# wonheeML/mtl-ssl

Hardware: AMD Instinct MI355X
Metric: images/sec training, Faster R-CNN ResNet-101 + aux heads (higher is better)
Workload: dtype f32; 1 GPU; Faster R-CNN ResNet-101 + window/closeness/edgemask heads + refine, synthetic 1024x600 COCO-shaped (90 classes), per-GPU batch 2 (BASELINE.json configs[1]); global_batch=2, parallelism=dp1, pipeline_config=configs/frcnn_resnet101_coco_mtl.config

## Files before the change

mtl_ssl_amd/csrc/conv.hip:

```cpp
#include <stdlib.h>

#include <atomic>
#include <mutex>
#include <unordered_map>

#include "conv_mfma.h"
#include "conv_split.h"

namespace mtlssl {

__global__ void __launch_bounds__(256) k_row_group_flags(const float* __restrict__ scale, int n, uint8_t* __restrict__ flags) {
  const int i = blockIdx.x * blockDim.x + threadIdx.x;
  if (i < n) flags[i] = scale[i] != 0.f;
}
__global__ void __launch_bounds__(256) k_active_ksteps(const uint8_t* __restrict__ flags, int rpg, int P, int pps, int stride,
                                                       int* __restrict__ out) {
  const int z = blockIdx.x, pix0 = z * pps, pix1 = min(P, pix0 + pps);
  const int ksteps = (max(pix1 - pix0, 0) + BK - 1) / BK;
  const int lane = threadIdx.x & 63, w = threadIdx.x >> 6;
  int* list = out + KSTEP_HDR + (int64_t)z * stride;
  __shared__ int wave_cnt[4];
  int base = 0;
  for (int s0 = 0; s0 < ksteps; s0 += 256) {
    const int s = s0 + threadIdx.x;
    bool act = false;
    if (s < ksteps) {
      const int r0 = pix0 + s * BK, r1 = min(r0 + BK, pix1) - 1;
      for (int g = r0 / rpg; g <= r1 / rpg; ++g) act |= flags[g] != 0;
    }
    const unsigned long long m = __ballot(act);
    if (lane == 0) wave_cnt[w] = __popcll(m);
    __syncthreads();
    int off = base;
    for (int i = 0; i < w; ++i) off += wave_cnt[i];
    if (act) list[off + __popcll(m & ((1ull << lane) - 1ull))] = s;
    base += wave_cnt[0] + wave_cnt[1] + wave_cnt[2] + wave_cnt[3];
    __syncthreads();
  }
  if (threadIdx.x == 0) out[z] = base;
}
static inline int64_t kstep_list_bytes(int64_t P) { return align_up((KSTEP_HDR + 2 * cdiv(P, BK) + 128) * 4, 256); }
static std::atomic<int>& row_skip_ref() { static std::atomic<int> v{1}; return v; }

__global__ void __launch_bounds__(256) k_wgrad_reduce(const float* ws, int nsplit, int64_t total4, int K,
                                                      const float* scale, float* dw, float beta, int main_blocks,
                                                      const float* cs_part, int cs_chunks, float* dbias,
                                                      const float* dbias_scale) {
  if ((int)blockIdx.x >= main_blocks) {
    const int lane = threadIdx.x & 63;
    const int k = ((int)blockIdx.x - main_blocks) * 4 + (threadIdx.x >> 6);
    if (k >= K) return;
    float s = 0.f;
    for (int c = lane; c < cs_chunks; c += 64) s += cs_part[(int64_t)c * K + k];
    s = wave_sum(s);
    if (dbias_scale) s *= dbias_scale[k];
    if (lane == 0) dbias[k] = beta != 0.f ? beta * dbias[k] + s : s;
    return;
  }
  const int64_t t = blockIdx.x * (int64_t)blockDim.x + threadIdx.x;
  const int64_t i = t >> 2;
  const int sl = (int)(t & 3);
  const bool live = i < total4;
  floatx4 s = {0.f, 0.f, 0.f, 0.f};
  if (live)
    for (int k = sl; k < nsplit; k += 4) s += reinterpret_cast<const floatx4*>(ws)[(int64_t)k * total4 + i];
#pragma unroll
  for (int e = 0; e < 4; ++e) {
    s[e] += __shfl_xor(s[e], 1, 64);
    s[e] += __shfl_xor(s[e], 2, 64);
  }
  if (!live || sl) return;
  if (scale) s *= *reinterpret_cast<const floatx4*>(scale + (i * 4) % K);
  floatx4* d = reinterpret_cast<floatx4*>(dw) + i;
  *d = beta != 0.f ? beta * *d + s : s;
}

__global__ void __launch_bounds__(256) k_wgrad_reduce_grouped(const float* ws, int nsplit, int64_t total4, int K,
                                                              const float* const* scale_tab, float* const* dw_tab,
                                                              float beta) {
  const int g = blockIdx.y;
  const int64_t t = blockIdx.x * (int64_t)blockDim.x + threadIdx.x;
  const int64_t i = t >> 2;
  const int sl = (int)(t & 3);
  const bool live = i < total4;
  const floatx4* w4 = reinterpret_cast<const floatx4*>(ws) + (int64_t)g * nsplit * total4;
  floatx4 s = {0.f, 0.f, 0.f, 0.f};
  if (live)
    for (int k = sl; k < nsplit; k += 4) s += w4[(int64_t)k * total4 + i];
#pragma unroll
  for (int e = 0; e < 4; ++e) {
    s[e] += __shfl_xor(s[e], 1, 64);
    s[e] += __shfl_xor(s[e], 2, 64);
  }
  if (!live || sl) return;
  const float* scale = scale_tab ? scale_tab[g] : nullptr;
  if (scale) s *= *reinterpret_cast<const floatx4*>(scale + (i * 4) % K);
  floatx4* d = reinterpret_cast<floatx4*>(dw_tab[g]) + i;
  *d = beta != 0.f ? beta * *d + s : s;
}

__global__ void k_conv_direct_fwd(ConvArgs p) {
  int64_t i = blockIdx.x * (int64_t)blockDim.x + threadIdx.x;
  int64_t total = (int64_t)p.M * p.K;
  if (i >= total) return;
  int k = i % p.K;
  int m = i / p.K;
  int ow = m % p.OW, t = m / p.OW, oh = t % p.OH, n = t / p.OH;
  float acc = 0.f;
  for (int r = 0; r < p.R; ++r) {
    int ih = oh * p.stride - p.pt + r * p.dil;
    if (ih < 0 || ih >= p.H) continue;
    for (int s = 0; s < p.S; ++s) {
      int iw = ow * p.stride - p.pl + s * p.dil;
      if (iw < 0 || iw >= p.W) continue;
      const float* xp = p.a + (((int64_t)n * p.H + ih) * p.W + iw) * p.C;
      const float* wp = p.b + ((int64_t)(r * p.S + s) * p.C) * p.K + k;
      for (int c = 0; c < p.C; ++c) acc = fmaf(xp[c], wp[(int64_t)c * p.K], acc);
    }
  }
  if (p.epi & MTLSSL_EPI_BIAS) acc += p.bias[k];
  if (p.epi & MTLSSL_EPI_RESIDUAL) acc += p.residual[i];
  if (p.epi & MTLSSL_EPI_RELU) acc = fmaxf(acc, 0.f);
  if (p.epi & MTLSSL_EPI_RELU6) acc = fminf(fmaxf(acc, 0.f), 6.f);
  if (p.epi & MTLSSL_EPI_TANH) acc = tanhf(acc);
  p.out[i] = acc;
}
__global__ void k_conv_direct_dgrad(ConvArgs p) {
  int64_t i = blockIdx.x * (int64_t)blockDim.x + threadIdx.x;
  int64_t total = (int64_t)p.M * p.C;
  if (i >= total) return;
  int c = i % p.C;
  int m = i / p.C;
  int iw = m % p.W, t = m / p.W, ih = t % p.H, n = t / p.H;
  float acc = 0.f;
  for (int r = 0; r < p.R; ++r) {
    int ny = ih + p.pt - r * p.dil;
    if (ny < 0 || ny % p.stride) continue;
    int oh = ny / p.stride;
    if (oh >= p.OH) continue;
    for (int s = 0; s < p.S; ++s) {
      int nx = iw + p.pl - s * p.dil;
      if (nx < 0 || nx % p.stride) continue;
      int ow = nx / p.stride;
      if (ow >= p.OW) continue;
      const float* gp = p.a + (((int64_t)n * p.OH + oh) * p.OW + ow) * p.K;
      const float* wp = p.b + ((int64_t)(r * p.S + s) * p.C + c) * p.K;
      for (int k = 0; k < p.K; ++k) acc = fmaf(gp[k], wp[k], acc);
    }
  }
  if (p.epi & MTLSSL_EPI_RESIDUAL) acc += p.residual[i];
  if (p.epi & MTLSSL_EPI_ACCUM) acc += p.out[i];
  if (p.epi & MASK_ANY) acc = act_mask(acc, p.mask[i], p.epi);
  p.out[i] = acc;
}
__global__ void k_conv_direct_wgrad(ConvArgs p, const float* scale, float* dw, float beta) {
  int rs = blockIdx.y, c = blockIdx.x;
  int r = rs / p.S, s = rs % p.S;
  int P = p.N * p.OH * p.OW;
  for (int k = threadIdx.x; k < p.K; k += blockDim.x) {
    float acc = 0.f;
    for (int pix = 0; pix < P; ++pix) {
      int ow = pix % p.OW, t = pix / p.OW, oh = t % p.OH, n = t / p.OH;
      int ih = oh * p.stride - p.pt + r * p.dil, iw = ow * p.stride - p.pl + s * p.dil;
      if (ih < 0 || ih >= p.H || iw < 0 || iw >= p.W) continue;
      acc = fmaf(p.a[(((int64_t)n * p.H + ih) * p.W + iw) * p.C + c], p.b[(int64_t)pix * p.K + k], acc);
    }
    if (scale) acc *= scale[k];
    int64_t o = ((int64_t)rs * p.C + c) * p.K + k;
    dw[o] = beta != 0.f ? beta * dw[o] + acc : acc;
  }
}

constexpr int STEM_MAX_CHUNKS = 512;
template <int R_, int S_, int C_>
__global__ void __launch_bounds__(256) k_conv_stem_wgrad(ConvArgs p, int pix_per_chunk, float* part) {
  constexpr int T = R_ * S_ * C_;
  const int KL = p.K <= 32 ? 32 : 64;
  const int k = threadIdx.x % KL, grp = threadIdx.x / KL, ngrp = 256 / KL;
  const int64_t P = (int64_t)p.N * p.OH * p.OW;
  int64_t p0 = (int64_t)blockIdx.x * pix_per_chunk;
  int64_t p1 = p0 + pix_per_chunk < P ? p0 + pix_per_chunk : P;
  float acc[T];
#pragma unroll
  for (int t = 0; t < T; ++t) acc[t] = 0.f;
  if (k < p.K) {
    for (int64_t pix = p0 + grp; pix < p1; pix += ngrp) {
      int ow = pix % p.OW;
      int64_t t2 = pix / p.OW;
      int oh = t2 % p.OH, n = t2 / p.OH;
      float g = p.b[pix * p.K + k];
#pragma unroll
      for (int r = 0; r < R_; ++r) {
        int ih = oh * p.stride - p.pt + r * p.dil;
#pragma unroll
        for (int s = 0; s < S_; ++s) {
          int iw = ow * p.stride - p.pl + s * p.dil;
          bool ok = ih >= 0 && ih < p.H && iw >= 0 && iw < p.W;
          const float* xp = p.a + (((int64_t)n * p.H + (ok ? ih : 0)) * p.W + (ok ? iw : 0)) * C_;
#pragma unroll
          for (int c = 0; c < C_; ++c) acc[(r * S_ + s) * C_ + c] += ok ? xp[c] * g : 0.f;
        }
      }
    }
  }
  __shared__ float red[8][64];
#pragma unroll
  for (int t = 0; t < T; ++t) {
    red[grp][k] = acc[t];
    __syncthreads();
    if (grp == 0 && k < p.K) {
      float v = 0.f;
      for (int g2 = 0; g2 < ngrp; ++g2) v += red[g2][k];
      part[((int64_t)blockIdx.x * T + t) * p.K + k] = v;
    }
    __syncthreads();
  }
}
static inline bool is_stem3(const mtlssl_conv_desc* d) {
  return d->R == 3 && d->S == 3 && d->C == 3 && d->K <= 64;
}
static inline void stem_plan(const mtlssl_conv_desc* d, int* chunks, int* ppc) {
  int64_t P = (int64_t)d->N * d->OH * d->OW;
  int c = (int)(cdiv(P, 128) < STEM_MAX_CHUNKS ? cdiv(P, 128) : STEM_MAX_CHUNKS);
  *ppc = (int)cdiv(P, c);
  *chunks = (int)cdiv(P, *ppc);
}

enum { GM_FWD = 0, GM_DGRAD = 1, GM_WGRAD = 2 };
struct GemmArgs {
  const float* a; const float* b; float* out;
  const float* bias; const float* residual; const float* mask;
  int M, N, K, epi, k_per_split;
};
template <int MODE>
__global__ void __launch_bounds__(256) k_gemm_small(GemmArgs p) {
  __shared__ float sA[16][64 + 1];
  __shared__ float sB[16][64 + 1];
  const int tid = threadIdx.x, tx = tid & 15, ty = tid >> 4;
  const int m0 = blockIdx.y * 64, n0 = blockIdx.x * 64;
  int k_lo = 0, k_hi = p.K;
  if constexpr (MODE == GM_WGRAD) {
    k_lo = blockIdx.z * p.k_per_split;
    k_hi = min(p.K, k_lo + p.k_per_split);
  }
  float acc[4][4] = {};
  for (int k0 = k_lo; k0 < k_hi; k0 += 16) {
#pragma unroll
    for (int e = 0; e < 4; ++e) {
      int u = tid + 256 * e;
      if constexpr (MODE == GM_WGRAD) {
        int k = u >> 6, m = u & 63;
        sA[k][m] = (k0 + k < k_hi && m0 + m < p.M) ? p.a[(int64_t)(k0 + k) * p.M + m0 + m] : 0.f;
      } else {
        int m = u >> 4, k = u & 15;
        sA[k][m] = (k0 + k < k_hi && m0 + m < p.M) ? p.a[(int64_t)(m0 + m) * p.K + k0 + k] : 0.f;
      }
      if constexpr (MODE == GM_DGRAD) {
        int n = u >> 4, k = u & 15;
        sB[k][n] = (k0 + k < k_hi && n0 + n < p.N) ? p.b[(int64_t)(n0 + n) * p.K + k0 + k] : 0.f;
      } else {
        int k = u >> 6, n = u & 63;
        sB[k][n] = (k0 + k < k_hi && n0 + n < p.N) ? p.b[(int64_t)(k0 + k) * p.N + n0 + n] : 0.f;
      }
    }
    __syncthreads();
#pragma unroll
    for (int k = 0; k < 16; ++k) {
      float av[4], bv[4];
#pragma unroll
      for (int i = 0; i < 4; ++i) av[i] = sA[k][ty + 16 * i];
#pragma unroll
      for (int j = 0; j < 4; ++j) bv[j] = sB[k][tx + 16 * j];
#pragma unroll
      for (int i = 0; i < 4; ++i)
#pragma unroll
        for (int j = 0; j < 4; ++j) acc[i][j] = fmaf(av[i], bv[j], acc[i][j]);
    }
    __syncthreads();
  }
  float* outp = p.out;
  if constexpr (MODE == GM_WGRAD) outp += (int64_t)blockIdx.z * p.M * p.N;
#pragma unroll
  for (int i = 0; i < 4; ++i) {
    int m = m0 + ty + 16 * i;
    if (m >= p.M) continue;
#pragma unroll
    for (int j = 0; j < 4; ++j) {
      int n = n0 + tx + 16 * j;
      if (n >= p.N) continue;
      int64_t o = (int64_t)m * p.N + n;
      float v = acc[i][j];
      if constexpr (MODE == GM_FWD) {
        if (p.epi & MTLSSL_EPI_BIAS) v += p.bias[n];
        if (p.epi & MTLSSL_EPI_RESIDUAL) v += p.residual[o];
        if (p.epi & MTLSSL_EPI_RELU) v = fmaxf(v, 0.f);
        if (p.epi & MTLSSL_EPI_RELU6) v = fminf(fmaxf(v, 0.f), 6.f);
        if (p.epi & MTLSSL_EPI_TANH) v = tanhf(v);
      } else if constexpr (MODE == GM_DGRAD) {
        if (p.epi & MTLSSL_EPI_RESIDUAL) v += p.residual[o];
        if (p.epi & MTLSSL_EPI_ACCUM) v += outp[o];
        if (p.epi & MASK_ANY) v = act_mask(v, p.mask[o], p.epi);
      }
      outp[o] = v;
    }
  }
}
__global__ void k_small_reduce(const float* ws, int nsplit, int64_t total, int K, const float* scale,
                               float* dw, float beta) {
  int64_t i = blockIdx.x * (int64_t)blockDim.x + threadIdx.x;
  if (i >= total) return;
  float s = 0.f;
  for (int k = 0; k < nsplit; ++k) s += ws[(int64_t)k * total + i];
  if (scale) s *= scale[i % K];
  dw[i] = beta != 0.f ? beta * dw[i] + s : s;
}
template <typename VT>
__global__ void __launch_bounds__(256) k_colsum_partial(const float* dy, int rows, int K, int ld, int rows_per_chunk,
                                                        int CQ, float* part) {
  constexpr int VW = sizeof(VT) / 4;
  const int KG = (K + VW - 1) / VW, PL = 256 / CQ;
  const int cq = threadIdx.x % CQ, sub = threadIdx.x / CQ;
  const int g = blockIdx.x * CQ + cq;
  const int r0 = blockIdx.y * rows_per_chunk, r1 = min(r0 + rows_per_chunk, rows);
  VT acc{};
  if (g < KG) {
    const float* b = dy + g * VW;
    for (int r = r0 + sub; r < r1; r += 2 * PL) {
      VT v0 = *reinterpret_cast<const VT*>(b + (int64_t)r * ld);
      VT v1 = r + PL < r1 ? *reinterpret_cast<const VT*>(b + (int64_t)(r + PL) * ld) : VT{};
      acc += v0;
      acc += v1;
    }
  }
  __shared__ floatx4 red_[256];
  VT* red = reinterpret_cast<VT*>(red_);
  red[threadIdx.x] = acc;
  __syncthreads();
  if (sub == 0 && g < KG) {
    VT v = red[cq];
    for (int l = 1; l < PL; ++l) v += red[l * CQ + cq];
    *reinterpret_cast<VT*>(part + (int64_t)blockIdx.y * K + g * VW) = v;
  }
}
// ... 182 lines not shown
  } else {
    if (p.epi & MTLSSL_EPI_RESIDUAL) v += p.residual[i];
    if (p.epi & MTLSSL_EPI_ACCUM) v += p.out[i];
    if (p.epi & MASK_ANY) v = act_mask(v, p.mask[i], p.epi);
  }
  p.out[i] = v;
}

struct Plan { int cfg, nsplit, ks_per_split, tail_rows, tail_nsplit, tail_ks; };
struct TunedKey {
  int mode; int64_t M, NG; int taps, kc, hw;
  bool operator==(const TunedKey& o) const {
    return mode == o.mode && M == o.M && NG == o.NG && taps == o.taps && kc == o.kc && hw == o.hw;
  }
};
struct TunedHash {
  size_t operator()(const TunedKey& k) const {
    uint64_t h = 1469598103934665603ull;
    for (uint64_t v : {(uint64_t)k.mode, (uint64_t)k.M, (uint64_t)k.NG, (uint64_t)k.taps, (uint64_t)k.kc, (uint64_t)k.hw}) { h ^= v; h *= 1099511628211ull; }
    return (size_t)h;
  }
};
static std::unordered_map<TunedKey, int, TunedHash>& tuned_map() { static std::unordered_map<TunedKey, int, TunedHash> m; return m; }
static std::mutex& tuned_mutex() { static std::mutex m; return m; }
static TunedKey make_key(const mtlssl_conv_desc* d, int mode) {
  const int hw = (d->H << 16) | (d->W & 0xffff);
  if (mode == MODE_FWD) return TunedKey{mode, (int64_t)d->N * d->OH * d->OW, d->K, d->R * d->S, d->C, hw};
  if (mode == MODE_DGRAD) return TunedKey{mode, (int64_t)d->N * d->H * d->W, d->C, d->R * d->S, d->K, hw};
  int64_t P = (int64_t)d->N * d->OH * d->OW;
  return TunedKey{mode, d->C, d->K, d->R * d->S, (int)(P > 0x7fffffff ? 0x7fffffff : P), hw};
}
static int tuned_cfg(const mtlssl_conv_desc* d, int mode) {
  std::lock_guard<std::mutex> g(tuned_mutex());
  auto it = tuned_map().find(make_key(d, mode));
  return it == tuned_map().end() ? -1 : it->second;
}
constexpr int CODE_ENGINE1 = 12, CODE_END = 24;
static inline int code_alg(int code) { return code < 0 ? -1 : (code % CODE_ENGINE1) / 4; }
static inline int code_tile(int code) { return code < 0 ? -1 : (code % 4) + (code >= CODE_ENGINE1 ? 4 : 0); }
static inline int make_code(int alg, int tile) { return 4 * alg + (tile & 3) + (tile >= 4 ? CODE_ENGINE1 : 0); }
static int tuned_direct_tile(const mtlssl_conv_desc* d, int mode) {
  const int code = tuned_cfg(d, mode);
  return code_alg(code) == 0 ? code_tile(code) : -1;
}
static inline bool glds_ok(int64_t NG) { return (NG & 3) == 0; }
static inline bool desc_is_pointwise(const mtlssl_conv_desc* d) {
  return d->R == 1 && d->S == 1 && d->stride == 1 && d->dilation == 1 && d->pad_t == 0 && d->pad_l == 0 && d->OH == d->H && d->OW == d->W;
}

static inline double fold_time_us(double bytes) { return 3.0 + bytes / (bytes < 48.0e6 ? 7.0e6 : 3.0e6); }
static Plan plan_gemm(int64_t M, int64_t NG, int taps, int kc, int tuned, double* t_out = nullptr, bool pw = false) {
  const int* resident = CFG_RESIDENT;
  Plan best{2, 1, taps * (kc / 16), 0, 1, 0};
  double best_t = 1e30;
  static int env_force = -2;
  if (env_force == -2) { const char* e = getenv("MTLSSL_FORCE_CFG"); env_force = e ? atoi(e) : -1; }
  int force = env_force >= 0 ? env_force : tuned;
  if (force >= NTILE || (force >= 0 && !cfg_allowed(force, kc))) force = -1;
  if (force >= NCFG && !glds_ok(NG)) force -= NCFG;
  for (int c = 0; c < NTILE; ++c) {
    if (!cfg_allowed(c, kc)) continue;
    if (force >= 0 ? c != force : c >= NCFG) continue;
    int ksteps = taps * (kc / CFG_BK[c]);
    const int64_t tiles_m = cdiv(M, CFG_BM[c]), tiles_n = cdiv(NG, CFG_BN[c]);
    int64_t tiles = tiles_m * tiles_n;
    for (int s = 1; s <= 8; ++s) {
      if (s > 1 && ksteps * CFG_BK[c] / s < 192) break;
      int per = (int)cdiv(ksteps, s);
      int ns = (int)cdiv(ksteps, per);
      if (ns != s) continue;
      double t = tile_time_us(c, tiles * ns, per, pw);
      if (ns > 1) t += fold_time_us((double)M * NG * 4.0 * (ns + 2));
      if (t < best_t) { best_t = t; best = Plan{c, ns, per, 0, 1, 0}; }
    }
    const int64_t slots = 256 * resident[c];
    const int64_t R = tiles % slots;
    if (!(NG & 3) && tiles >= slots && R > 0 && ksteps >= 32) {
      int64_t rows = cdiv(R, tiles_n);
      int64_t tail_tiles = rows * tiles_n;
      int ns = (int)(slots / tail_tiles);
      if (ns > 8) ns = 8;
      if (ns > ksteps / 16) ns = ksteps / 16;
      if (ns >= 2 && rows < tiles_m) {
        int per = (int)cdiv(ksteps, ns);
        ns = (int)cdiv(ksteps, per);
        double t = tile_time_us(c, tiles - tail_tiles, ksteps, pw) + tile_time_us(c, tail_tiles * ns, per, pw) +
                   5.0 + fold_time_us((double)rows * CFG_BM[c] * NG * 4.0 * (ns + 2));
        if (t < best_t) { best_t = t; best = Plan{c, 1, ksteps, (int)rows, ns, per}; }
      }
    }
  }
  if (t_out) *t_out = best_t;
  return best;
}
static Plan plan_dir(const mtlssl_conv_desc* d, int mode, double* t_out = nullptr) {
  const int64_t M = mode == MODE_FWD ? (int64_t)d->N * d->OH * d->OW : (int64_t)d->N * d->H * d->W;
  return plan_gemm(M, mode == MODE_FWD ? d->K : d->C, d->R * d->S, mode == MODE_FWD ? d->C : d->K,
                   tuned_direct_tile(d, mode), t_out, desc_is_pointwise(d));
}
static int64_t split_bytes(const Plan& pl, int64_t M, int64_t NG) {
  if (pl.tail_rows > 0) {
    const int64_t m_tail0 = (cdiv(M, CFG_BM[pl.cfg]) - pl.tail_rows) * CFG_BM[pl.cfg];
    return align_up((M - m_tail0) * NG * 4 * pl.tail_nsplit, 256);
  }
  return pl.nsplit > 1 ? align_up(M * NG * 4 * pl.nsplit, 256) : 0;
}

static bool is_pointwise(const mtlssl_conv_desc* d) {
  return d->R == 1 && d->S == 1 && d->stride == 1 && d->pad_t == 0 && d->pad_l == 0 && d->OH == d->H &&
         d->OW == d->W;
}
static bool padded_dgrad_ok(const mtlssl_conv_desc* d) {
  return is_pointwise(d) && d->K % BK != 0 && d->K >= 8 && d->C % 4 == 0 && d->C >= 16;
}
static mtlssl_conv_desc padded_desc(const mtlssl_conv_desc* d) {
  mtlssl_conv_desc q = *d;
  q.K = (int)align_up(d->K, BK);
  return q;
}
static bool padded_fwd_ok(const mtlssl_conv_desc* d) {
  return is_pointwise(d) && d->C % BK != 0 && d->C >= 32 && d->K >= 16;
}
static bool padded_wgrad_ok(const mtlssl_conv_desc* d) {
  return is_pointwise(d) && (d->K & 3) != 0 && d->K >= 13 && d->C % 4 == 0 && d->C >= 16 && desc_dense(d);
}
static mtlssl_conv_desc padded_wgrad_desc(const mtlssl_conv_desc* d) {
  mtlssl_conv_desc q = *d;
  q.K = (int)align_up(d->K, 4);
  q.ldy = 0;
  return q;
}
__global__ void __launch_bounds__(256) k_wgrad_reduce_unpad(const float* ws, int nsplit, int C, int Kp, int K,
                                                            const float* scale, float* dw, float beta, int main_blocks,
                                                            const float* cs_part, float* dbias, const float* dbias_scale) {
  if ((int)blockIdx.x >= main_blocks) {
    const int k = ((int)blockIdx.x - main_blocks) * 256 + threadIdx.x;
    if (k >= K) return;
    float s = 0.f;
    for (int z = 0; z < nsplit; ++z) s += cs_part[(int64_t)z * Kp + k];
    if (dbias_scale) s *= dbias_scale[k];
    dbias[k] = beta != 0.f ? beta * dbias[k] + s : s;
    return;
  }
  const int64_t i = blockIdx.x * (int64_t)blockDim.x + threadIdx.x;
  if (i >= (int64_t)C * K) return;
  const int c = (int)(i / K), k = (int)(i - (int64_t)c * K);
  const int64_t plane = (int64_t)C * Kp;
  float s = 0.f;
  for (int z = 0; z < nsplit; ++z) s += ws[(int64_t)z * plane + (int64_t)c * Kp + k];
  if (scale) s *= scale[k];
  dw[i] = beta != 0.f ? beta * dw[i] + s : s;
}
__global__ void __launch_bounds__(256) k_pw_thin_fwd(const float* __restrict__ x, const float* __restrict__ w,
                                                     const float* __restrict__ bias, const float* __restrict__ residual,
                                                     float* __restrict__ y, int M, int C, int K, int epi) {
  const int lane = threadIdx.x & 63;
  const int m = blockIdx.x * 4 + (threadIdx.x >> 6);
  if (m >= M) return;
  float acc[8] = {0.f, 0.f, 0.f, 0.f, 0.f, 0.f, 0.f, 0.f};
  const float* xr = x + (int64_t)m * C;
  for (int c = lane * 4; c < C; c += 256) {
    const floatx4 xv = *reinterpret_cast<const floatx4*>(xr + c);
#pragma unroll
    for (int j = 0; j < 4; ++j) {
      const float* wr = w + (int64_t)(c + j) * K;
#pragma unroll
      for (int k = 0; k < 8; ++k)
        if (k < K) acc[k] = fmaf(xv[j], wr[k], acc[k]);
    }
  }
#pragma unroll
  for (int k = 0; k < 8; ++k) acc[k] = wave_sum(acc[k]);
  if (lane < K) {
    float v = acc[0];
#pragma unroll
    for (int k = 1; k < 8; ++k) v = lane == k ? acc[k] : v;
    const int64_t o = (int64_t)m * K + lane;
    if (epi & MTLSSL_EPI_BIAS) v += bias[lane];
    if (epi & MTLSSL_EPI_RESIDUAL) v += residual[o];
    if (epi & MTLSSL_EPI_RELU) v = fmaxf(v, 0.f);
    if (epi & MTLSSL_EPI_RELU6) v = fminf(fmaxf(v, 0.f), 6.f);
    if (epi & MTLSSL_EPI_TANH) v = tanhf(v);
    y[o] = v;
  }
}
static bool thin_fwd_ok(const mtlssl_conv_desc* d) {
  return is_pointwise(d) && d->K <= 8 && d->C % 4 == 0 && desc_dense(d);
}
__global__ void __launch_bounds__(256) k_pad_rows(const float* src, int64_t rows, int K, int Kp, float* dst) {
  const int64_t i = (int64_t)blockIdx.x * blockDim.x + threadIdx.x;
  if (i >= rows * Kp) return;
  const int64_t r = i / Kp;
  const int k = (int)(i - r * Kp);
  dst[i] = k < K ? src[r * K + k] : 0.f;
}
static bool s2d_fwd_ok(const mtlssl_conv_desc* d) {
  return d->stride == 2 && d->dilation == 1 && d->C * 4 <= BK && d->K >= 16 && d->K % 4 == 0 && d->R <= 8 && d->S <= 8;
}
static mtlssl_conv_desc s2d_desc(const mtlssl_conv_desc* d) {
  mtlssl_conv_desc q = *d;
  q.R = (d->R + 1) / 2; q.S = (d->S + 1) / 2;
  q.H = d->OH + q.R - 1; q.W = d->OW + q.S - 1;
  q.C = BK; q.stride = 1; q.dilation = 1; q.pad_t = 0; q.pad_l = 0;
  return q;
}
__global__ void __launch_bounds__(256) k_s2d_pack(const float* __restrict__ x, int N, int H, int W, int C, int pt, int pl,
                                                   int H2, int W2, float* __restrict__ xs) {
  const int64_t i = (int64_t)blockIdx.x * blockDim.x + threadIdx.x;
  if (i >= (int64_t)N * H2 * W2 * 4) return;
  const int ph = (int)(i & 3);
  int64_t t = i >> 2;
  const int x2 = (int)(t % W2); t /= W2;
  const int y2 = (int)(t % H2);
  const int n = (int)(t / H2);
  const int ih = 2 * y2 + (ph >> 1) - pt, iw = 2 * x2 + (ph & 1) - pl;
  const bool ok = (unsigned)ih < (unsigned)H && (unsigned)iw < (unsigned)W;
  const float* src = x + (((int64_t)n * H + ih) * W + iw) * C;
  float* dst = xs + (((int64_t)n * H2 + y2) * W2 + x2) * BK;
  for (int c = 0; c < C; ++c) dst[ph * C + c] = ok ? src[c] : 0.f;
  if (ph == 0)
    for (int c = 4 * C; c < BK; ++c) dst[c] = 0.f;
}
__global__ void __launch_bounds__(256) k_s2d_filter(const float* __restrict__ w, int R, int S, int C, int K, int R2, int S2,
                                                     float* __restrict__ ws) {
  const int i = blockIdx.x * blockDim.x + threadIdx.x;
  if (i >= R2 * S2 * BK * K) return;
  const int k = i % K;
  int t = i / K;
  const int ch = t % BK; t /= BK;
  const int s2 = t % S2, r2 = t / S2;
  float v = 0.f;
  if (ch < 4 * C) {
    const int ph = ch / C, c = ch - ph * C;
    const int r = 2 * r2 + (ph >> 1), sx = 2 * s2 + (ph & 1);
    if (r < R && sx < S) v = w[((r * S + sx) * C + c) * K + k];
  }
  ws[i] = v;
}
static size_t stem_lds_bytes(const mtlssl_conv_desc* d) {
  int PH = (STEM_T - 1) * d->stride + (d->R - 1) * d->dilation + 1;
  int PW = (STEM_T - 1) * d->stride + (d->S - 1) * d->dilation + 1;
  return sizeof(float) * ((size_t)d->R * d->S * d->C * 64 + (size_t)PH * PW * d->C);
}
static void small_wgrad_plan(const mtlssl_conv_desc* d, int* nsplit, int* k_per_split) {
  int64_t P = (int64_t)d->N * d->OH * d->OW;
  int64_t tiles = cdiv(d->C, 64) * cdiv(d->K, 64);
  int64_t s = cdiv(512, tiles);
  int64_t maxs = cdiv(P, 128);
  if (s > maxs) s = maxs;
  if (s < 1) s = 1;
  if (s > 64) s = 64;
  int64_t per = align_up(cdiv(P, s), 16);
  *nsplit = (int)cdiv(P, per);
  *k_per_split = (int)per;
}

static std::atomic<int>& pointwise_ref() { static std::atomic<int> v{1}; return v; }

static std::atomic<int64_t>* engine_launch_counts() {
  static std::atomic<int64_t> v[4];
  return v;
}
void count_engine_launch(int slot) { engine_launch_counts()[slot].fetch_add(1, std::memory_order_relaxed); }

template <int MODE>
static void launch_mfma(int cfg, ConvArgs& p, dim3 extra, hipStream_t st, int tile_rows = -1) {
  count_engine_launch(0);
  p.tiles_m = tile_rows >= 0 ? tile_rows : (int)cdiv(p.M, CFG_BM[cfg]);
  p.tiles_n = (int)cdiv(p.NG, CFG_BN[cfg]);
  dim3 grid(p.tiles_m * p.tiles_n, extra.y, extra.z);
  if (cfg >= NCFG && (p.a_tab || !glds_ok(p.NG) || (MODE == MODE_WGRAD && !glds_ok(p.M)))) cfg -= NCFG;
  const bool pw = conv_is_pointwise(p) && pointwise_ref().load() != 0;
  if constexpr (MODE == MODE_WGRAD) {
    if (p.cs_part) {
      if (cfg < NCFG && pw) {
        switch (cfg) {
          case 0: hipLaunchKernelGGL((k_conv_mfma_pw_cs<128, 128>), grid, dim3(256), 0, st, p); break;
          case 1: hipLaunchKernelGGL((k_conv_mfma_pw_cs<128, 64>), grid, dim3(256), 0, st, p); break;
          case 2: hipLaunchKernelGGL((k_conv_mfma_pw_cs<64, 64>), grid, dim3(256), 0, st, p); break;
          default: hipLaunchKernelGGL((k_conv_mfma_pw_cs<256, 128>), grid, dim3(512), 0, st, p); break;
        }
      } else if (pw) {
        switch (cfg) {
          case 4: hipLaunchKernelGGL((k_conv_glds_pw_cs<128, 128, 16, GLDS_STAGES>), grid, dim3(256), 0, st, p); break;
          case 5: hipLaunchKernelGGL((k_conv_glds_pw_cs<128, 64, 16, GLDS_STAGES>), grid, dim3(256), 0, st, p); break;
          case 6: hipLaunchKernelGGL((k_conv_glds_pw_cs<64, 64, 16, GLDS_STAGES>), grid, dim3(256), 0, st, p); break;
          default: hipLaunchKernelGGL((k_conv_glds_pw_cs<256, 128, 16, GLDS_STAGES>), grid, dim3(512), 0, st, p); break;
        }
      } else {
        switch (cfg) {
          case 0: hipLaunchKernelGGL((k_conv_mfma_cs<128, 128, 16>), grid, dim3(256), 0, st, p); break;
          case 1: hipLaunchKernelGGL((k_conv_mfma_cs<128, 64, 16>), grid, dim3(256), 0, st, p); break;
          case 2: hipLaunchKernelGGL((k_conv_mfma_cs<64, 64, 16>), grid, dim3(256), 0, st, p); break;
          case 3: hipLaunchKernelGGL((k_conv_mfma_cs<256, 128, 16>), grid, dim3(512), 0, st, p); break;
          case 4: hipLaunchKernelGGL((k_conv_glds_cs<128, 128, 16, GLDS_STAGES>), grid, dim3(256), 0, st, p); break;
          case 5: hipLaunchKernelGGL((k_conv_glds_cs<128, 64, 16, GLDS_STAGES>), grid, dim3(256), 0, st, p); break;
          case 6: hipLaunchKernelGGL((k_conv_glds_cs<64, 64, 16, GLDS_STAGES>), grid, dim3(256), 0, st, p); break;
          default: hipLaunchKernelGGL((k_conv_glds_cs<256, 128, 16, GLDS_STAGES>), grid, dim3(512), 0, st, p); break;
        }
      }
      return;
    }
  }
  if (cfg < NCFG && pw) {
    switch (cfg) {
      case 0: hipLaunchKernelGGL((k_conv_mfma_pw<128, 128, MODE>), grid, dim3(256), 0, st, p); break;
      case 1: hipLaunchKernelGGL((k_conv_mfma_pw<128, 64, MODE>), grid, dim3(256), 0, st, p); break;
      case 2: hipLaunchKernelGGL((k_conv_mfma_pw<64, 64, MODE>), grid, dim3(256), 0, st, p); break;
      default: hipLaunchKernelGGL((k_conv_mfma_pw<256, 128, MODE>), grid, dim3(512), 0, st, p); break;
    }
    return;
  }
  if (pw) {
    switch (cfg) {
      case 4: hipLaunchKernelGGL((k_conv_glds_pw<128, 128, MODE, 16, GLDS_STAGES>), grid, dim3(256), 0, st, p); break;
      case 5: hipLaunchKernelGGL((k_conv_glds_pw<128, 64, MODE, 16, GLDS_STAGES>), grid, dim3(256), 0, st, p); break;
      case 6: hipLaunchKernelGGL((k_conv_glds_pw<64, 64, MODE, 16, GLDS_STAGES>), grid, dim3(256), 0, st, p); break;
      default: hipLaunchKernelGGL((k_conv_glds_pw<256, 128, MODE, 16, GLDS_STAGES>), grid, dim3(512), 0, st, p); break;
    }
    return;
  }
  switch (cfg) {
    case 0: hipLaunchKernelGGL((k_conv_mfma<128, 128, MODE, 16>), grid, dim3(256), 0, st, p); break;
    case 1: hipLaunchKernelGGL((k_conv_mfma<128, 64, MODE, 16>), grid, dim3(256), 0, st, p); break;
    case 2: hipLaunchKernelGGL((k_conv_mfma<64, 64, MODE, 16>), grid, dim3(256), 0, st, p); break;
    case 3: hipLaunchKernelGGL((k_conv_mfma<256, 128, MODE, 16>), grid, dim3(512), 0, st, p); break;
    case 4: hipLaunchKernelGGL((k_conv_glds<128, 128, MODE, 16, GLDS_STAGES>), grid, dim3(256), 0, st, p); break;
    case 5: hipLaunchKernelGGL((k_conv_glds<128, 64, MODE, 16, GLDS_STAGES>), grid, dim3(256), 0, st, p); break;
    case 6: hipLaunchKernelGGL((k_conv_glds<64, 64, MODE, 16, GLDS_STAGES>), grid, dim3(256), 0, st, p); break;
    default: hipLaunchKernelGGL((k_conv_glds<256, 128, MODE, 16, GLDS_STAGES>), grid, dim3(512), 0, st, p); break;
  }
}

template <int MODE>
static void launch_planned(const Plan& pl, ConvArgs& p, float* ws, hipStream_t st) {
  p.splitk_ws = ws;
  if (pl.nsplit == 1 && args_ldy(p) == p.K &&
      split_engine_takes(pl.cfg, p.M, p.NG, (int64_t)p.R * p.S * (MODE == MODE_FWD ? p.C : p.K))) {
    p.nsplit = 1; p.ks_per_split = 0; p.tile_m0 = 0; p.ws_m0 = 0;
    launch_split_direct<MODE>(p, dim3(1, 1, 1), st);
    return;
  }
  if (pl.tail_rows == 0) {
    p.nsplit = pl.nsplit; p.ks_per_split = pl.ks_per_split;
    launch_mfma<MODE>(pl.cfg, p, dim3(1, 1, pl.nsplit), st);
    if (pl.nsplit > 1) {
      if (p.NG & 3)
        hipLaunchKernelGGL(k_splitk_epilogue_scalar<MODE>, dim3(cdiv((int64_t)p.M * p.NG, 256)), dim3(256), 0, st, p);
      else
        hipLaunchKernelGGL(k_splitk_epilogue<MODE>, dim3(cdiv((int64_t)p.M * p.NG / 4, 256)), dim3(256), 0, st, p);
    }
    return;
  }
  const int rows_total = (int)cdiv(p.M, CFG_BM[pl.cfg]);
  const int rows_main = rows_total - pl.tail_rows;
  p.nsplit = 1; p.ks_per_split = 0; p.tile_m0 = 0; p.ws_m0 = 0;
  launch_mfma<MODE>(pl.cfg, p, dim3(1, 1, 1), st, rows_main);
  ConvArgs q = p;
  q.tile_m0 = rows_main;
  q.ws_m0 = rows_main * CFG_BM[pl.cfg];
  q.nsplit = pl.tail_nsplit; q.ks_per_split = pl.tail_ks;
  launch_mfma<MODE>(pl.cfg, q, dim3(1, 1, pl.tail_nsplit), st, pl.tail_rows);
  ConvArgs f = q;
  const int64_t off = (int64_t)q.ws_m0 * p.NG;
  f.M = p.M - q.ws_m0;
  f.out = p.out + (MODE == MODE_FWD ? (int64_t)q.ws_m0 * args_ldy(p) : off);
  if (p.residual) f.residual = p.residual + off;
  if (p.mask) f.mask = p.mask + off;
  hipLaunchKernelGGL(k_splitk_epilogue<MODE>, dim3(cdiv((int64_t)f.M * f.NG / 4, 256)), dim3(256), 0, st, f);
}

struct WgradPlan { int cfg, nsplit, pps; };
static WgradPlan wgrad_plan(const mtlssl_conv_desc* d, double* t_out = nullptr) {
  int64_t P = (int64_t)d->N * d->OH * d->OW;
  int RS = d->R * d->S;
  double best_t = 1e30;
  WgradPlan best{2, 1, (int)align_up(P, 16)};
  const int force = tuned_direct_tile(d, MODE_WGRAD);
  for (int c = 0; c < NTILE; ++c) {
    if (force >= 0 ? c != force : c >= NCFG) continue;
    int bk = CFG_BK[c];
    int ksteps = (int)cdiv(P, bk);
    int64_t tiles = cdiv(d->C, CFG_BM[c]) * cdiv(d->K, CFG_BN[c]) * RS;
    for (int s = 1; s <= 64; ++s) {
      if (s > 1 && ksteps * bk / s < 128) break;
      int per = (int)cdiv(ksteps, s);
      int ns = (int)cdiv(ksteps, per);
      if (ns != s) continue;
      double t = tile_time_us(c, tiles * ns, per, desc_is_pointwise(d)) +
                 2.0 + (double)RS * d->C * d->K * 4.0 * (ns + 1) / 3.0e6;
      if (t < best_t) { best_t = t; best = WgradPlan{c, ns, per * bk}; }
    }
  }
  if (t_out) *t_out = best_t;
  return best;
}

constexpr int WINO_CFG0 = 4;
struct WinoChoice { int variant, tile; };
static std::atomic<int>& fp32_engine_ref() {
  static std::atomic<int> v{-1};
  return v;
}
int fp32_engine() {
  int v = fp32_engine_ref().load();
  if (v < 0) {
    const char* e = getenv("MTLSSL_FP32_ENGINE");
    v = (e && (!strcmp(e, "split") || !strcmp(e, "1"))) ? 1 : 0;
    fp32_engine_ref().store(v);
  }
  return v;
}
static std::atomic<int>& wino_mode_ref() {
  static std::atomic<int> v{-1};
  return v;
}
static int wino_env() {
  int v = wino_mode_ref().load();
  if (v < 0) {
    const char* e = getenv("MTLSSL_WINOGRAD");
    v = e ? atoi(e) : 1;
    if (v < 0 || v > 2) v = 1;
    wino_mode_ref().store(v);
  }
  return v;
}
static bool choose_wino(const mtlssl_conv_desc* d, int mode, double t_direct, WinoChoice* wc) {
  const int env = wino_env();
  if (env == 0 || !wino_eligible(d, WINO_F43)) return false;
  const int force = tuned_cfg(d, mode);
  if (code_alg(force) >= 1) {
    const int variant = code_alg(force) - 1, tile = code_tile(force);
    if (variant < WINO_VARIANTS && wino_eligible(d, variant)) { *wc = WinoChoice{variant, tile}; return true; }
  }
  double tw = 1e30;
  for (int v = 0; v < WINO_VARIANTS; ++v) {
    if (!wino_eligible(d, v)) continue;
    int tile;
    double t = wino_time_us(d, v, mode, &tile);
    if (t < tw) { tw = t; *wc = WinoChoice{v, tile}; }
  }
  if (env == 2) return true;
  if (code_alg(force) == 0) return false;
  return tw < t_direct;
}

struct ParityProblem { int py, px, Hs, Ws, r0, s0, Rs, Ss, a, b; };
static bool parity_ok(const mtlssl_conv_desc* d) {
  return d->stride == 2 && d->dilation == 1 && mfma_dgrad_ok(d) && d->R * d->S > 1 &&
         d->H >= 2 && d->W >= 2;
}
static ParityProblem parity_problem(const mtlssl_conv_desc* d, int py, int px) {
  ParityProblem q;
  q.py = py; q.px = px;
  q.Hs = (d->H - py + 1) / 2; q.Ws = (d->W - px + 1) / 2;
  q.r0 = (py + d->pad_t) & 1; q.s0 = (px + d->pad_l) & 1;
  q.Rs = d->R > q.r0 ? (d->R - q.r0 + 1) / 2 : 0;
  q.Ss = d->S > q.s0 ? (d->S - q.s0 + 1) / 2 : 0;
  q.a = (py + d->pad_t - q.r0) / 2; q.b = (px + d->pad_l - q.s0) / 2;
  return q;
}
__global__ void k_parity_filter(const float* w, float* ws, int S, int r0, int s0, int Ss, int64_t CK4) {
  int64_t i = blockIdx.x * (int64_t)blockDim.x + threadIdx.x;
  if (i >= CK4) return;
  int jl = blockIdx.y, j = jl / Ss, l = jl - j * Ss;
  reinterpret_cast<floatx4*>(ws)[(int64_t)jl * CK4 + i] =
      reinterpret_cast<const floatx4*>(w)[(int64_t)((r0 + 2 * j) * S + s0 + 2 * l) * CK4 + i];
}
__global__ void k_parity_scatter(const float* tmp, float* dx, const float* residual, const float* mask, int epi,
                                 int H, int W, int C4, int Hs, int Ws, int py, int px, int64_t total4) {
  int64_t i = blockIdx.x * (int64_t)blockDim.x + threadIdx.x;
  if (i >= total4) return;
  int c4 = (int)(i % C4);
  int64_t t = i / C4;
  int v = (int)(t % Ws);
  t /= Ws;
  int u = (int)(t % Hs), n = (int)(t / Hs);
  floatx4 val = tmp ? reinterpret_cast<const floatx4*>(tmp)[i] : floatx4{0.f, 0.f, 0.f, 0.f};
  const int64_t o = ((((int64_t)n * H + 2 * u + py) * W + 2 * v + px) * C4 + c4);
  if (epi & MTLSSL_EPI_RESIDUAL) val += reinterpret_cast<const floatx4*>(residual)[o];
  if (epi & MTLSSL_EPI_ACCUM) val += reinterpret_cast<const floatx4*>(dx)[o];
  if (epi & MASK_ANY) {
    floatx4 mk = reinterpret_cast<const floatx4*>(mask)[o];
#pragma unroll
    for (int e = 0; e < 4; ++e) val[e] = act_mask(val[e], mk[e], epi);
  }
  reinterpret_cast<floatx4*>(dx)[o] = val;
}

enum Family {
  FAM_WINO,
  FAM_DIRECT,
  FAM_PARITY,
  FAM_PADDED,
  FAM_S2D,
  FAM_THIN,
  FAM_GEMM_SMALL,
  FAM_STEM_FWD,
  FAM_STEM3_WGRAD,
  FAM_SCALAR,
};
struct Route {
  int family;
  WinoChoice wc;
  mtlssl_conv_desc q;
  Plan plan;
  WgradPlan wg;
  int split_ns, split_pps;
  Plan parity[4];
  int64_t front_a, front_bytes;
  int64_t bytes;
};
static inline int64_t colsum_bytes(const mtlssl_conv_desc* d) { return align_up((int64_t)COLSUM_MAX_PARTS * d->K * 4, 256); }
static int64_t wgrad_partial_bytes(const mtlssl_conv_desc* d, int ns, int* split_ns, int* split_pps) {
  if (!split_wgrad_plan((int64_t)d->N * d->OH * d->OW, d->C, d->K, d->R * d->S, split_ns, split_pps)) *split_ns = *split_pps = 0;
  if (*split_ns > ns) ns = *split_ns;
  return align_up((int64_t)ns * d->R * d->S * d->C * d->K * 4, 256);
}
static bool wgrad_on_split_engine(const Route& r, const mtlssl_conv_desc* d) {
  return fp32_engine() >= 1 && (r.wg.cfg == 0 || r.wg.cfg == 3) && desc_dense(d) && r.split_ns > 0;
}
static inline int stem_fwd_family(int epi) { return (epi & ~(MTLSSL_EPI_BIAS | MTLSSL_EPI_RELU)) ? FAM_SCALAR : FAM_STEM_FWD; }

static void resolve_wgrad(const mtlssl_conv_desc* d, Route* r) {
  const int64_t P = (int64_t)d->N * d->OH * d->OW;
  int ns, pps;
  if (mfma_wgrad_ok(d)) {
    double t;
    r->wg = wgrad_plan(d, &t);
    if (choose_wino(d, MODE_WGRAD, t, &r->wc)) {
      r->family = FAM_WINO;
      r->bytes = wino_workspace_bytes(d, r->wc.variant, MODE_WGRAD);
    } else {
      r->family = FAM_DIRECT;
      r->bytes = wgrad_partial_bytes(d, r->wg.nsplit, &r->split_ns, &r->split_pps);
    }
  } else if (padded_wgrad_ok(d)) {
    r->family = FAM_PADDED;
    r->q = padded_wgrad_desc(d);
    r->wg = wgrad_plan(&r->q);
    r->front_a = r->front_bytes = align_up(P * r->q.K * 4, 256);
    r->bytes = r->front_bytes + wgrad_partial_bytes(&r->q, r->wg.nsplit, &ns, &pps);
  } else if (is_pointwise(d)) {
    r->family = FAM_GEMM_SMALL;
    small_wgrad_plan(d, &r->wg.nsplit, &r->wg.pps);
    r->bytes = align_up((int64_t)r->wg.nsplit * d->C * d->K * 4, 256);
  } else if (is_stem3(d)) {
    r->family = FAM_STEM3_WGRAD;
    stem_plan(d, &r->wg.nsplit, &r->wg.pps);
    r->bytes = align_up((int64_t)STEM_MAX_CHUNKS * 27 * d->K * 4, 256);
  } else {
    r->family = FAM_SCALAR;
  }
}
static Route resolve(const mtlssl_conv_desc* d, int mode, bool ws) {
  Route r;
  memset(&r, 0, sizeof(r));
  r.q = *d;
  if (mode == MODE_WGRAD) { resolve_wgrad(d, &r); return r; }
  const bool fwd = mode == MODE_FWD;
  const int64_t M = fwd ? (int64_t)d->N * d->OH * d->OW : (int64_t)d->N * d->H * d->W, NG = fwd ? d->K : d->C;
  if (fwd ? mfma_fwd_ok(d) : mfma_dgrad_ok(d)) {
    double t;
    r.plan = plan_dir(d, mode, &t);
    if (ws && choose_wino(d, mode, t, &r.wc)) {
      r.family = FAM_WINO;
      r.bytes = wino_workspace_bytes(d, r.wc.variant, mode);
    } else if (ws && !fwd && parity_ok(d)) {
      r.family = FAM_PARITY;
      r.front_a = align_up((int64_t)d->R * d->S * d->C * d->K * 4, 256);
      r.front_bytes = r.front_a + align_up((int64_t)d->N * ((d->H + 1) / 2) * ((d->W + 1) / 2) * d->C * 4, 256);
      int64_t split = 0;
      for (int c = 0; c < 4; ++c) {
        const ParityProblem q = parity_problem(d, c >> 1, c & 1);
        if (q.Rs == 0 || q.Ss == 0) continue;
        r.parity[c] = plan_gemm((int64_t)d->N * q.Hs * q.Ws, d->C, q.Rs * q.Ss, d->K, tuned_direct_tile(d, MODE_DGRAD));
        const int64_t b = split_bytes(r.parity[c], (int64_t)d->N * q.Hs * q.Ws, d->C);
        if (b > split) split = b;
      }
      r.bytes = r.front_bytes + split;
    } else {
      r.family = FAM_DIRECT;
      if (!ws && (r.plan.nsplit > 1 || r.plan.tail_rows > 0)) r.plan = Plan{pick_tile(M, NG, 1), 1, 0, 0, 1, 0};
      r.bytes = split_bytes(r.plan, M, NG);
    }
    return r;
  }
  if (ws && (fwd ? padded_fwd_ok(d) : padded_dgrad_ok(d))) {
    r.family = FAM_PADDED;
    if (fwd) r.q.C = (int)align_up(d->C, BK); else r.q = padded_desc(d);
    r.front_a = align_up(M * (fwd ? r.q.C : r.q.K) * 4, 256);
    r.front_bytes = r.front_a + align_up((int64_t)r.q.C * r.q.K * 4, 256);
  } else if (fwd && thin_fwd_ok(d)) {
    r.family = FAM_THIN;
  } else if (is_pointwise(d)) {
    r.family = FAM_GEMM_SMALL;
  } else if (ws && fwd && s2d_fwd_ok(d)) {
    r.family = FAM_S2D;
    r.q = s2d_desc(d);
    r.front_a = align_up((int64_t)r.q.N * r.q.H * r.q.W * r.q.C * 4, 256);
    r.front_bytes = r.front_a + align_up((int64_t)r.q.R * r.q.S * r.q.C * r.q.K * 4, 256);
  } else if (fwd && d->K == 64 && d->C <= 4 && stem_lds_bytes(d) <= 160 * 1024) {
    r.family = FAM_STEM_FWD;
  } else {
    r.family = FAM_SCALAR;
  }
  if (r.family == FAM_PADDED || r.family == FAM_S2D) {
    r.plan = plan_dir(&r.q, mode);
    r.bytes = r.front_bytes + split_bytes(r.plan, M, NG);
  }
  return r;
}

struct DescKey {
  mtlssl_conv_desc d; int mode;
  bool operator==(const DescKey& o) const { return mode == o.mode && memcmp(&d, &o.d, sizeof(d)) == 0; }
};
struct DescHash {
  size_t operator()(const DescKey& k) const {
    uint64_t h = 1469598103934665603ull ^ (uint64_t)k.mode;
    const int32_t* p = reinterpret_cast<const int32_t*>(&k.d);
    for (size_t i = 0; i < sizeof(k.d) / 4; ++i) { h ^= (uint32_t)p[i]; h *= 1099511628211ull; }
    return (size_t)h;
  }
};
static std::unordered_map<DescKey, Route, DescHash>& route_map() {
  static std::unordered_map<DescKey, Route, DescHash> m;
  return m;
}
static std::mutex& memo_mutex() { static std::mutex m; return m; }
static void routes_clear() {
  std::lock_guard<std::mutex> g(memo_mutex());
  route_map().clear();
}
static Route route(const mtlssl_conv_desc* d, int mode, bool have_workspace = true) {
  DescKey k;
  memset(&k, 0, sizeof(k));
  k.d = *d; k.mode = have_workspace ? mode : mode + 4;
  {
    std::lock_guard<std::mutex> g(memo_mutex());
    auto it = route_map().find(k);
    if (it != route_map().end()) return it->second;
  }
  const Route r = resolve(d, mode, have_workspace);
  std::lock_guard<std::mutex> g(memo_mutex());
  route_map()[k] = r;
  return r;
}

static void parity_dgrad(const Route& r, const mtlssl_conv_desc* d, const float* dy, const float* w, const float* residual,
                         const float* mask_ref, float* dx, int epi, void* workspace, hipStream_t st) {
  const int64_t CK = (int64_t)d->C * d->K;
  float* wsub = (float*)workspace;
  float* tmp = (float*)((char*)workspace + r.front_a);
  float* split = (float*)((char*)workspace + r.front_bytes);
  for (int c = 0; c < 4; ++c) {
    ParityProblem q = parity_problem(d, c >> 1, c & 1);
    if (q.Hs == 0 || q.Ws == 0) continue;
    const int64_t M = (int64_t)d->N * q.Hs * q.Ws;
    const bool taps = q.Rs > 0 && q.Ss > 0;
    if (taps) {
      hipLaunchKernelGGL(k_parity_filter, dim3(cdiv(CK / 4, 256), q.Rs * q.Ss), dim3(256), 0, st, w, wsub, d->S, q.r0,
                         q.s0, q.Ss, CK / 4);
      ConvArgs p;
      memset(&p, 0, sizeof(p));
      p.N = d->N; p.H = q.Hs; p.W = q.Ws; p.C = d->C; p.K = d->K; p.R = q.Rs; p.S = q.Ss;
      p.OH = d->OH; p.OW = d->OW; p.stride = 1; p.dil = 1; p.pt = q.a; p.pl = q.b;
      p.a = dy; p.b = wsub; p.out = tmp; p.epi = 0;
      p.ldy = desc_ldy(d);
      p.a_bytes = ydy_bytes(d);
      p.b_bytes = (unsigned)((int64_t)q.Rs * q.Ss * CK * 4);
      p.M = (int)M; p.NG = d->C;
      launch_planned<MODE_DGRAD>(r.parity[c], p, split, st);
    }
    const int64_t total4 = M * d->C / 4;
    hipLaunchKernelGGL(k_parity_scatter, dim3(cdiv(total4, 256)), dim3(256), 0, st, taps ? (const float*)tmp : nullptr,
                       dx, residual, mask_ref, epi, d->H, d->W, d->C / 4, q.Hs, q.Ws, q.py, q.px, total4);
  }
}
template <int MODE>
static void launch_packed(const Route& r, const ConvArgs& p, const float* a, const float* b, void* workspace, hipStream_t st) {
  const mtlssl_conv_desc& q = r.q;
  ConvArgs pq = make_args(&q);
  pq.a = a; pq.b = b; pq.out = p.out; pq.bias = p.bias; pq.residual = p.residual; pq.mask = p.mask; pq.epi = p.epi;
  pq.a_bytes = (unsigned)((MODE == MODE_FWD ? (int64_t)q.N * q.H * q.W * q.C : (int64_t)q.N * q.OH * q.OW * q.K) * 4);
  pq.b_bytes = (unsigned)((int64_t)q.R * q.S * q.C * q.K * 4);
  pq.M = p.M; pq.NG = p.NG;
  launch_planned<MODE>(r.plan, pq, (float*)((char*)workspace + r.front_bytes), st);
}

}

using namespace mtlssl;

extern "C" {

int64_t mtlssl_conv2d_workspace_bytes(const mtlssl_conv_desc* d, int mode) {
  if (!d || mode < MODE_FWD || mode > MODE_WGRAD) return 0;
  if (mode == MODE_WGRAD) return mtlssl_conv2d_wgrad_workspace_bytes(d);
  return route(d, mode).bytes;
}

int64_t mtlssl_conv2d_filter_xf_bytes(const mtlssl_conv_desc* d, int mode) {
  if (!d || (mode != MODE_FWD && mode != MODE_DGRAD) || check_desc(d)) return 0;
  const Route r = route(d, mode);
  return r.family == FAM_WINO ? wino_filter_bytes(d, r.wc.variant) : 0;
}
int mtlssl_conv2d_filter_xf_variant(const mtlssl_conv_desc* d, int mode) {
  if (!d || mode < MODE_FWD || mode > MODE_WGRAD || check_desc(d)) return -1;
  const Route r = route(d, mode);
  return r.family == FAM_WINO ? r.wc.variant : -1;
}
int64_t mtlssl_conv2d_input_xf_bytes(const mtlssl_conv_desc* d, int variant) {
  if (!d || check_desc(d) || variant < 0 || variant >= WINO_VARIANTS || !wino_eligible(d, variant)) return 0;
  return wino_input_bytes(d, variant);
}
int mtlssl_conv2d_transform_filter(const mtlssl_conv_desc* d, int mode, int variant, const float* w, float* filter_xf,
                                   mtlssl_stream_t stream) {
  if (int rc = check_desc(d)) return rc;
  MTLSSL_REQUIRE(mode == MODE_FWD || mode == MODE_DGRAD, "transform_filter: mode %d", mode);
  MTLSSL_REQUIRE(variant >= 0 && variant < WINO_VARIANTS && wino_eligible(d, variant),
                 "transform_filter: variant %d is not applicable to this problem", variant);
  MTLSSL_REQUIRE(w && filter_xf, "transform_filter: null pointer");
  wino_filter(d, variant, mode == MODE_DGRAD, w, filter_xf, S(stream));
  return check_launch("conv2d_transform_filter");
}

int mtlssl_conv2d_transform_filters(int variant, int n, const void* w_ptrs, const void* xf_ptrs, const int64_t* ck,
                                    const int32_t* flip, int64_t max_ck, mtlssl_stream_t stream) {
  if (n <= 0) return MTLSSL_OK;
  MTLSSL_REQUIRE(variant >= 0 && variant < WINO_VARIANTS, "transform_filters: variant %d", variant);
  MTLSSL_REQUIRE(w_ptrs && xf_ptrs && ck && flip && max_ck > 0 && n <= 65535, "transform_filters: bad table");
  wino_filters_batched(variant, n, w_ptrs, xf_ptrs, ck, flip, max_ck, S(stream));
  return check_launch("conv2d_transform_filters");
}

int mtlssl_conv2d_fwd(const mtlssl_conv_desc* d, const float* x, const float* w, const float* bias,
                      const float* residual, float* y, int epi, void* workspace,
                      mtlssl_stream_t stream) {
  return mtlssl_conv2d_fwd_xf(d, x, w, bias, residual, y, epi, workspace, nullptr, -1, stream);
}

int mtlssl_conv2d_fwd_xf(const mtlssl_conv_desc* d, const float* x, const float* w, const float* bias,
                         const float* residual, float* y, int epi, void* workspace, const float* filter_xf,
                         int xf_variant, mtlssl_stream_t stream) {
  return mtlssl_conv2d_fwd_keep(d, x, w, bias, residual, y, epi, workspace, filter_xf, xf_variant, nullptr, -1, stream);
}

int mtlssl_conv2d_fwd_keep(const mtlssl_conv_desc* d, const float* x, const float* w, const float* bias,
                           const float* residual, float* y, int epi, void* workspace, const float* filter_xf,
                           int xf_variant, float* input_xf, int input_variant, mtlssl_stream_t stream) {
  if (int rc = check_desc(d)) return rc;
  MTLSSL_REQUIRE(!(epi & MTLSSL_EPI_BIAS) || bias, "conv_fwd: bias pointer required");
  MTLSSL_REQUIRE(!(epi & MTLSSL_EPI_RESIDUAL) || residual, "conv_fwd: residual pointer required");
  ConvArgs p = make_args(d);
  p.a = x; p.b = w; p.out = y; p.bias = bias; p.residual = residual; p.epi = epi;
  p.a_bytes = (unsigned)((int64_t)d->N * d->H * d->W * d->C * 4);
  p.b_bytes = (unsigned)((int64_t)d->R * d->S * d->C * d->K * 4);
  p.M = d->N * d->OH * d->OW;
  p.NG = d->K;
  MTLSSL_REQUIRE(desc_dense(d) || mfma_fwd_ok(d), "conv_fwd: a strided output (ldy = %d) needs C %% 16 == 0 and K >= 16", d->ldy);
  const Route r = route(d, MODE_FWD, workspace != nullptr);
  const mtlssl_conv_desc& q = r.q;
  switch (r.family == FAM_STEM_FWD ? stem_fwd_family(epi) : r.family) {
    case FAM_WINO:
      wino_fwd(d, r.wc.variant, r.wc.tile, x, w, bias, residual, y, epi, workspace, S(stream),
               (filter_xf && xf_variant == r.wc.variant) ? filter_xf : nullptr,
               (input_xf && input_variant == r.wc.variant) ? input_xf : nullptr);
      break;
    case FAM_DIRECT:
      launch_planned<MODE_FWD>(r.plan, p, (float*)workspace, S(stream));
      break;
    case FAM_PADDED: {
      float* x_pad = (float*)workspace;
      float* w_pad = (float*)((char*)workspace + r.front_a);
      hipLaunchKernelGGL(k_pad_rows, dim3(cdiv((int64_t)p.M * q.C, 256)), dim3(256), 0, S(stream), x, (int64_t)p.M, d->C, q.C, x_pad);
      (void)hipMemcpyAsync(w_pad, w, (size_t)d->C * d->K * 4, hipMemcpyDeviceToDevice, S(stream));
      (void)hipMemsetAsync(w_pad + (int64_t)d->C * d->K, 0, (size_t)(q.C - d->C) * d->K * 4, S(stream));
      launch_packed<MODE_FWD>(r, p, x_pad, w_pad, workspace, S(stream));
      break;
    }
    case FAM_THIN:
      hipLaunchKernelGGL(k_pw_thin_fwd, dim3(cdiv(p.M, 4)), dim3(256), 0, S(stream), x, w, bias, residual, y, p.M, d->C, d->K, epi);
      break;
    case FAM_GEMM_SMALL: {
      GemmArgs g{x, w, y, bias, residual, nullptr, p.M, d->K, d->C, epi, 0};
      hipLaunchKernelGGL(k_gemm_small<GM_FWD>, dim3(cdiv(g.N, 64), cdiv(g.M, 64)), dim3(256), 0, S(stream), g);
      break;
    }
    case FAM_S2D: {
      float* xs = (float*)workspace;
      float* wsf = (float*)((char*)workspace + r.front_a);
      hipLaunchKernelGGL(k_s2d_pack, dim3(cdiv((int64_t)q.N * q.H * q.W * 4, 256)), dim3(256), 0, S(stream), x, d->N, d->H, d->W,
                         d->C, d->pad_t, d->pad_l, q.H, q.W, xs);
      hipLaunchKernelGGL(k_s2d_filter, dim3(cdiv((int64_t)q.R * q.S * q.C * q.K, 256)), dim3(256), 0, S(stream), w, d->R, d->S,
                         d->C, d->K, q.R, q.S, wsf);
      launch_packed<MODE_FWD>(r, p, xs, wsf, workspace, S(stream));
      break;
    }
    case FAM_STEM_FWD: {
      dim3 grid(cdiv(d->OW, STEM_T), cdiv(d->OH, STEM_T), d->N);
      hipLaunchKernelGGL(k_conv_smallc_fwd, grid, dim3(256), stem_lds_bytes(d), S(stream), p);
      break;
    }
    default:
      hipLaunchKernelGGL(k_conv_direct_fwd, dim3(cdiv((int64_t)p.M * p.K, 256)), dim3(256), 0, S(stream), p);
  }
  return check_launch("conv2d_fwd");
}

int mtlssl_conv2d_fwd_grouped(const mtlssl_conv_desc* d, const float* x, int n, const mtlssl_conv_group_entry* entries,
                              int max_k, int sum_k, mtlssl_stream_t stream) {
  if (n <= 0) return MTLSSL_OK;
  if (int rc = check_desc(d)) return rc;
  MTLSSL_REQUIRE(is_pointwise(d) && d->dilation == 1, "fwd_grouped: pointwise problems only (1x1, stride 1, no padding)");
  MTLSSL_REQUIRE(d->C % BK == 0, "fwd_grouped: C = %d must be a multiple of %d", d->C, BK);
  MTLSSL_REQUIRE(x && entries && n <= MTLSSL_CONV_GROUP_MAX && max_k >= 16 && sum_k >= max_k, "fwd_grouped: bad arguments");
  ConvArgs p = make_args(d);
  GroupArgs ga;
  memset(&ga, 0, sizeof(ga));
  p.a = x;
  for (int i = 0; i < n; ++i) {
    const mtlssl_conv_group_entry& e = entries[i];
    MTLSSL_REQUIRE(e.w && e.y && e.K >= 16 && e.K % 4 == 0 && e.K <= max_k && (e.ldy == 0 || (e.ldy >= e.K && e.ldy % 4 == 0)) &&
                       !(e.epilogue & (MTLSSL_EPI_RESIDUAL | MASK_ANY | MTLSSL_EPI_ACCUM)) && (!(e.epilogue & MTLSSL_EPI_BIAS) || e.bias),
                   "fwd_grouped: problem %d: K = %d, ldy = %d, epilogue = %d", i, e.K, e.ldy, e.epilogue);
    ga.e[i] = e;
  }
  p.a_bytes = (unsigned)((int64_t)d->N * d->H * d->W * d->C * 4);
  p.M = d->N * d->H * d->W;
  p.NG = max_k; p.K = max_k; p.ldy = 0;
  p.nsplit = 1; p.ks_per_split = 0; p.tile_m0 = 0; p.ws_m0 = 0;
  int cfg = 2;
  double best = 1e30;
  for (int c = 0; c < NCFG; ++c) {
    const int64_t tiles = cdiv(p.M, CFG_BM[c]) * cdiv(sum_k, CFG_BN[c]);
    const double t = tile_time_us(c, tiles, d->C / CFG_BK[c], true);
    if (t < best) { best = t; cfg = c; }
  }
  p.tiles_m = (int)cdiv(p.M, CFG_BM[cfg]);
  p.tiles_n = (int)cdiv(max_k, CFG_BN[cfg]);
  dim3 grid(p.tiles_m * p.tiles_n, n, 1);
  count_engine_launch(0);
  switch (cfg) {
    case 0: hipLaunchKernelGGL((k_conv_mfma_pw_grp<128, 128>), grid, dim3(256), 0, S(stream), p, ga); break;
    case 1: hipLaunchKernelGGL((k_conv_mfma_pw_grp<128, 64>), grid, dim3(256), 0, S(stream), p, ga); break;
    case 2: hipLaunchKernelGGL((k_conv_mfma_pw_grp<64, 64>), grid, dim3(256), 0, S(stream), p, ga); break;
    default: hipLaunchKernelGGL((k_conv_mfma_pw_grp<256, 128>), grid, dim3(512), 0, S(stream), p, ga); break;
  }
  return check_launch("conv2d_fwd_grouped");
}

static int seg_dgrad_cfg_env() {
  static const int v = [] { const char* e = getenv("MTLSSL_SEG_DGRAD_CFG"); return e ? atoi(e) : -1; }();
  return v;
}
int mtlssl_conv2d_dgrad_segmented(const mtlssl_conv_desc* d, int n, const mtlssl_conv_seg_entry* entries,
                                  const float* residual, const float* mask_ref, float* dx, int epi,
                                  mtlssl_stream_t stream) {
  if (int rc = check_desc(d)) return rc;
  MTLSSL_REQUIRE(is_pointwise(d) && d->dilation == 1, "dgrad_segmented: pointwise problems only (1x1, stride 1, no padding)");
  MTLSSL_REQUIRE(entries && dx && n >= 1 && n <= MTLSSL_CONV_GROUP_MAX, "dgrad_segmented: bad arguments (n = %d)", n);
  MTLSSL_REQUIRE(d->C % 4 == 0 && d->C >= 16, "dgrad_segmented: C = %d must be a multiple of 4 and >= 16", d->C);
  MTLSSL_REQUIRE(!(epi & MASK_ANY) || mask_ref, "dgrad_segmented: mask_ref pointer required");
  MTLSSL_REQUIRE(!(epi & MTLSSL_EPI_RESIDUAL) || residual, "dgrad_segmented: residual pointer required");
  MTLSSL_REQUIRE(!(epi & ~(MTLSSL_EPI_RESIDUAL | MASK_ANY)), "dgrad_segmented: epilogue = %d (RESIDUAL / MASK / MASK6 only)", epi);
  const int64_t M = (int64_t)d->N * d->H * d->W;
  SegArgs sa;
  memset(&sa, 0, sizeof(sa));
  int sum_k = 0;
  for (int i = 0; i < n; ++i) {
    const mtlssl_conv_seg_entry& e = entries[i];
    MTLSSL_REQUIRE(e.dy && e.w && e.K >= BK && e.K % BK == 0 && (e.ldy == 0 || (e.ldy >= e.K && e.ldy % 4 == 0)),
                   "dgrad_segmented: segment %d: K = %d, ldy = %d", i, e.K, e.ldy);
    MTLSSL_REQUIRE(((M - 1) * (e.ldy ? e.ldy : e.K) + e.K) * 4 < (int64_t)1 << 32, "dgrad_segmented: segment %d exceeds 4 GiB", i);
    sa.e[i] = e;
    sum_k += e.K;
  }
  mtlssl_conv_desc q = *d;
  q.K = sum_k; q.ldy = 0;
  ConvArgs p = make_args(&q);
  p.a = entries[0].dy; p.b = entries[0].w; p.out = dx; p.residual = residual; p.mask = mask_ref; p.epi = epi;
  p.a_bytes = 0; p.b_bytes = 0;
  p.M = (int)M;
  p.NG = d->C;
  p.nsplit = 1; p.ks_per_split = 0; p.tile_m0 = 0; p.ws_m0 = 0;
  int cfg = seg_dgrad_cfg_env();
  if (cfg < 0 || cfg >= NCFG) {
    cfg = cdiv(p.M, CFG_BM[1]) * cdiv(p.NG, CFG_BN[1]) >= 512 ? 1 : 2;
  }
  p.tiles_m = (int)cdiv(p.M, CFG_BM[cfg]);
  p.tiles_n = (int)cdiv(p.NG, CFG_BN[cfg]);
  dim3 grid(p.tiles_m * p.tiles_n, 1, 1);
  count_engine_launch(0);
  switch (cfg) {
    case 0: hipLaunchKernelGGL((k_conv_mfma_pw_seg<128, 128>), grid, dim3(256), 0, S(stream), p, sa); break;
    case 1: hipLaunchKernelGGL((k_conv_mfma_pw_seg<128, 64>), grid, dim3(256), 0, S(stream), p, sa); break;
    case 2: hipLaunchKernelGGL((k_conv_mfma_pw_seg<64, 64>), grid, dim3(256), 0, S(stream), p, sa); break;
    default: hipLaunchKernelGGL((k_conv_mfma_pw_seg<256, 128>), grid, dim3(512), 0, S(stream), p, sa); break;
  }
  return check_launch("conv2d_dgrad_segmented");
}

int mtlssl_conv2d_dgrad(const mtlssl_conv_desc* d, const float* dy, const float* w,
                        const float* residual, const float* mask_ref, float* dx, int epi,
                        void* workspace, mtlssl_stream_t stream) {
  return mtlssl_conv2d_dgrad_xf(d, dy, w, residual, mask_ref, dx, epi, workspace, nullptr, -1, stream);
}

int mtlssl_conv2d_dgrad_xf(const mtlssl_conv_desc* d, const float* dy, const float* w,
                           const float* residual, const float* mask_ref, float* dx, int epi,
                           void* workspace, const float* filter_xf, int xf_variant, mtlssl_stream_t stream) {
  return mtlssl_conv2d_dgrad_rs(d, dy, w, residual, mask_ref, dx, epi, workspace, filter_xf, xf_variant, nullptr, 0, stream);
}

int mtlssl_conv2d_dgrad_rs(const mtlssl_conv_desc* d, const float* dy, const float* w,
                           const float* residual, const float* mask_ref, float* dx, int epi,
                           void* workspace, const float* filter_xf, int xf_variant, const uint8_t* group_active,
                           int rows_per_group, mtlssl_stream_t stream) {
  if (int rc = check_desc(d)) return rc;
  MTLSSL_REQUIRE(!group_active || rows_per_group > 0, "conv_dgrad: group_active needs rows_per_group > 0");
  MTLSSL_REQUIRE(!(epi & MASK_ANY) || mask_ref, "conv_dgrad: mask_ref pointer required");
  MTLSSL_REQUIRE(!(epi & MTLSSL_EPI_RESIDUAL) || residual, "conv_dgrad: residual pointer required");
  ConvArgs p = make_args(d);
  p.a = dy; p.b = w; p.out = dx; p.residual = residual; p.mask = mask_ref; p.epi = epi;
  p.a_bytes = ydy_bytes(d);
  p.b_bytes = (unsigned)((int64_t)d->R * d->S * d->C * d->K * 4);
  p.M = d->N * d->H * d->W;
  p.NG = d->C;
  MTLSSL_REQUIRE(desc_dense(d) || mfma_dgrad_ok(d),
                 "conv_dgrad: a strided dy (ldy = %d) needs K %% 16 == 0, C %% 4 == 0 and C >= 16", d->ldy);
  const Route r = route(d, MODE_DGRAD, workspace != nullptr);
  switch (r.family) {
    case FAM_WINO:
      wino_dgrad(d, r.wc.variant, r.wc.tile, dy, w, residual, mask_ref, dx, epi, workspace, S(stream),
                 (filter_xf && xf_variant == r.wc.variant) ? filter_xf : nullptr,
                 (group_active && row_skip_ref().load() != 0 && rows_per_group == d->H * d->W) ? group_active : nullptr);
      break;
    case FAM_PARITY:
      parity_dgrad(r, d, dy, w, residual, mask_ref, dx, epi, workspace, S(stream));
      break;
    case FAM_DIRECT:
      if (group_active && row_skip_ref().load() != 0 && desc_is_pointwise(d)) {
        p.group_active = group_active;
        p.rows_per_group = rows_per_group;
      }
      launch_planned<MODE_DGRAD>(r.plan, p, (float*)workspace, S(stream));
      break;
    case FAM_PADDED: {
      float* dy_pad = (float*)workspace;
      float* w_pad = (float*)((char*)workspace + r.front_a);
      hipLaunchKernelGGL(k_pad_rows, dim3(cdiv((int64_t)p.M * r.q.K, 256)), dim3(256), 0, S(stream), dy, (int64_t)p.M, d->K, r.q.K, dy_pad);
      hipLaunchKernelGGL(k_pad_rows, dim3(cdiv((int64_t)d->C * r.q.K, 256)), dim3(256), 0, S(stream), w, (int64_t)d->C, d->K, r.q.K, w_pad);
      launch_packed<MODE_DGRAD>(r, p, dy_pad, w_pad, workspace, S(stream));
      break;
    }
    case FAM_GEMM_SMALL: {
      GemmArgs g{dy, w, dx, nullptr, residual, mask_ref, p.M, d->C, d->K, epi, 0};
      hipLaunchKernelGGL(k_gemm_small<GM_DGRAD>, dim3(cdiv(g.N, 64), cdiv(g.M, 64)), dim3(256), 0, S(stream), g);
      break;
    }
    default:
      hipLaunchKernelGGL(k_conv_direct_dgrad, dim3(cdiv((int64_t)p.M * p.C, 256)), dim3(256), 0, S(stream), p);
  }
  return check_launch("conv2d_dgrad");
}

int mtlssl_conv2d_tile_config(const mtlssl_conv_desc* d, int mode) {
  if (!d || mode < MODE_FWD || mode > MODE_WGRAD) return -1;
  const Route r = route(d, mode);
  if (r.family == FAM_WINO) return make_code(1 + r.wc.variant, r.wc.tile);
  if (r.family != FAM_DIRECT && r.family != FAM_PARITY) return -1;
  return make_code(0, mode == MODE_WGRAD ? r.wg.cfg : r.plan.cfg);
}

int64_t mtlssl_conv2d_executed_macs(const mtlssl_conv_desc* d, int mode, int on_mfma) {
  if (!d || mode < MODE_FWD || mode > MODE_WGRAD || check_desc(d)) return 0;
  const int64_t P_out = (int64_t)d->N * d->OH * d->OW, P_in = (int64_t)d->N * d->H * d->W;
  const int64_t taps = (int64_t)d->R * d->S;
  const int64_t direct = (mode == MODE_DGRAD && d->stride == 1 ? P_in : P_out) * taps * d->C * d->K;
  const int64_t gathered = P_in * taps * d->C * d->K;
  const Route r = route(d, mode);
  const mtlssl_conv_desc& q = r.q;
  int64_t mfma = 0;
  switch (r.family) {
    case FAM_WINO: mfma = wino_input_bytes(d, r.wc.variant) / 4 * d->K; break;
    case FAM_DIRECT: mfma = mode == MODE_DGRAD ? gathered : direct; break;
    case FAM_PARITY: mfma = gathered / ((int64_t)d->stride * d->stride); break;
    case FAM_PADDED: mfma = (mode == MODE_DGRAD ? P_in : P_out) * q.C * q.K; break;
    case FAM_S2D: mfma = P_out * q.R * q.S * q.C * q.K; break;
    default: return on_mfma ? 0 : direct;
  }
  return on_mfma ? mfma : 0;
}

int mtlssl_conv2d_force_config(const mtlssl_conv_desc* d, int mode, int cfg) {
  MTLSSL_REQUIRE(d != nullptr && mode >= MODE_FWD && mode <= MODE_WGRAD, "force_config: bad arguments");
  MTLSSL_REQUIRE(cfg < CODE_END, "force_config: plan code out of range (0..%d)", CODE_END - 1);
  TunedKey k = make_key(d, mode);
  {
    std::lock_guard<std::mutex> g(tuned_mutex());
    if (cfg < 0) tuned_map().erase(k); else tuned_map()[k] = cfg;
  }
  routes_clear();
  return MTLSSL_OK;
}

int mtlssl_conv2d_set_fp32_engine(int mode) {
  const int prev = fp32_engine();
  if (mode >= 0 && mode <= 3) fp32_engine_ref().store(mode);
  return prev;
}

int mtlssl_conv2d_engine_launches(int64_t out[4], int reset) {
  MTLSSL_REQUIRE(out != nullptr, "engine_launches: out required");
  for (int i = 0; i < 4; ++i)
    out[i] = reset ? engine_launch_counts()[i].exchange(0, std::memory_order_relaxed)
                   : engine_launch_counts()[i].load(std::memory_order_relaxed);
  return MTLSSL_OK;
}

int mtlssl_conv2d_set_winograd(int mode) {
  const int prev = wino_env();
  if (mode >= 0 && mode <= 2) { wino_mode_ref().store(mode); routes_clear(); }
  return prev;
}

int mtlssl_conv2d_set_row_skip(int on) {
  const int prev = row_skip_ref().load();
  if (on == 0 || on == 1) row_skip_ref().store(on);
  return prev;
}

int mtlssl_row_group_flags(const float* scale, int n, uint8_t* flags, mtlssl_stream_t stream) {
  if (n <= 0) return MTLSSL_OK;
  MTLSSL_REQUIRE(scale && flags, "row_group_flags: null pointer");
  hipLaunchKernelGGL(k_row_group_flags, dim3(cdiv(n, 256)), dim3(256), 0, S(stream), scale, n, flags);
  return check_launch("row_group_flags");
}

int mtlssl_conv2d_set_pointwise(int on) {
  const int prev = pointwise_ref().load();
  if (on == 0 || on == 1) pointwise_ref().store(on);
  return prev;
}

int mtlssl_conv2d_num_dispatches(const mtlssl_conv_desc* d, int mode) {
  if (!d) return 0;
  if (mode != MODE_FWD && mode != MODE_DGRAD) return 1;
  const Route r = route(d, mode);
  return (r.family == FAM_DIRECT || r.family == FAM_PARITY) && r.plan.tail_rows > 0 ? 2 : 1;
}

static void plan_info_gemm(const Plan& pl, int64_t M, int64_t NG, int ksteps, int32_t* out) {
  out[2] = pl.cfg; out[3] = pl.nsplit; out[4] = pl.ks_per_split;
  out[5] = pl.tail_rows; out[6] = pl.tail_rows > 0 ? pl.tail_nsplit : 0; out[7] = pl.tail_rows > 0 ? pl.tail_ks : 0;
  out[8] = ksteps; out[9] = (int32_t)M; out[10] = (int32_t)NG; out[11] = CFG_BM[pl.cfg]; out[12] = CFG_BN[pl.cfg];
}
int mtlssl_conv2d_plan_info(const mtlssl_conv_desc* d, int mode, int parity_class, int32_t* out) {
  MTLSSL_REQUIRE(d != nullptr && out != nullptr && mode >= MODE_FWD && mode <= MODE_WGRAD, "plan_info: bad arguments");
  if (int rc = check_desc(d)) return rc;
  static const int32_t PUBLIC[] = {MTLSSL_PLAN_WINO_F43, MTLSSL_PLAN_DIRECT, MTLSSL_PLAN_PARITY, MTLSSL_PLAN_PADDED, MTLSSL_PLAN_S2D,
                                   MTLSSL_PLAN_THIN,     MTLSSL_PLAN_VALU,   MTLSSL_PLAN_VALU,   MTLSSL_PLAN_VALU,   MTLSSL_PLAN_VALU};
  const Route r = route(d, mode);
  const mtlssl_conv_desc& q = r.q;
  for (int i = 0; i < MTLSSL_PLAN_INFO_LEN; ++i) out[i] = 0;
  out[0] = PUBLIC[r.family];
  out[1] = mtlssl_conv2d_tile_config(d, mode);
  out[2] = -1;
  out[14] = mtlssl_conv2d_num_dispatches(d, mode);
  const int64_t P = (int64_t)d->N * d->OH * d->OW, M = mode == MODE_FWD ? P : (int64_t)d->N * d->H * d->W;
  switch (r.family) {
    case FAM_WINO:
      if (r.wc.variant != 0) out[0] = MTLSSL_PLAN_WINO_M7;
      out[2] = r.wc.tile; out[3] = 1;
      if (mode == MODE_WGRAD) {
        int ns, pps;
        wino_wgrad_split(d, r.wc.variant, r.wc.tile, &ns, &pps);
        const int64_t T = wino_input_bytes(d, r.wc.variant) / ((r.wc.variant != 0 ? 121 : 36) * 4 * (int64_t)d->C);
        out[3] = ns; out[4] = pps / BK; out[8] = (int32_t)cdiv(T, BK); out[13] = pps;
      }
      out[9] = (int32_t)(mode == MODE_WGRAD ? d->C : M);
      out[10] = mode == MODE_DGRAD ? d->C : d->K;
      out[11] = CFG_BM[r.wc.tile]; out[12] = CFG_BN[r.wc.tile];
      break;
    case FAM_PARITY: {
      MTLSSL_REQUIRE(parity_class >= 0 && parity_class < 4, "plan_info: parity class %d of an input-parity dgrad", parity_class);
      const ParityProblem c = parity_problem(d, parity_class >> 1, parity_class & 1);
      if (c.Hs == 0 || c.Ws == 0 || c.Rs == 0 || c.Ss == 0) break;
      const Plan& pl = r.parity[parity_class];
      plan_info_gemm(pl, (int64_t)d->N * c.Hs * c.Ws, d->C, c.Rs * c.Ss * (d->K / CFG_BK[pl.cfg]), out);
      break;
    }
    case FAM_DIRECT: case FAM_PADDED: case FAM_S2D:
      if (mode == MODE_WGRAD) {
        const int cfg = r.wg.cfg;
        out[2] = cfg; out[3] = r.wg.nsplit; out[4] = r.wg.pps / CFG_BK[cfg]; out[8] = (int32_t)cdiv(P, CFG_BK[cfg]);
        out[9] = q.C; out[10] = q.K; out[11] = CFG_BM[cfg]; out[12] = CFG_BN[cfg]; out[13] = r.wg.pps;
      } else {
        plan_info_gemm(r.plan, M, mode == MODE_FWD ? q.K : q.C, q.R * q.S * ((mode == MODE_FWD ? q.C : q.K) / CFG_BK[r.plan.cfg]), out);
      }
      break;
    default: break;
  }
  return MTLSSL_OK;
}

int64_t mtlssl_conv2d_wgrad_workspace_bytes(const mtlssl_conv_desc* d) {
  if (!d) return 256;
  return colsum_bytes(d) + route(d, MODE_WGRAD).bytes +
         (desc_is_pointwise(d) ? kstep_list_bytes((int64_t)d->N * d->OH * d->OW) : 0);
}

static void wgrad_group_plan(const mtlssl_conv_desc* d, int n, int* cfg, int* nsplit, int* pps) {
  const int64_t P = (int64_t)d->N * d->OH * d->OW;
  const int RS = d->R * d->S;
  double best_t = 1e30;
  *cfg = 2; *nsplit = 1; *pps = (int)align_up(P, 16);
  for (int c = 0; c < NCFG; ++c) {
    const int ksteps = (int)cdiv(P, CFG_BK[c]);
    const int64_t tiles = cdiv(d->C, CFG_BM[c]) * cdiv(d->K, CFG_BN[c]) * RS * n;
    for (int s = 1; s <= 16; ++s) {
      if (s > 1 && ksteps * CFG_BK[c] / s < 128) break;
      const int per = (int)cdiv(ksteps, s), ns = (int)cdiv(ksteps, per);
      if (ns != s) continue;
      const double t = tile_time_us(c, tiles * ns, per, desc_is_pointwise(d)) + 2.0 + (double)n * RS * d->C * d->K * 4.0 * (ns + 1) / 3.0e6;
      if (t < best_t) { best_t = t; *cfg = c; *nsplit = ns; *pps = per * CFG_BK[c]; }
    }
  }
}
int64_t mtlssl_conv2d_wgrad_grouped_workspace_bytes(const mtlssl_conv_desc* d, int n) {
  if (!d || n <= 0 || check_desc(d) || !mfma_wgrad_ok(d)) return 0;
  int cfg, ns, pps;
  wgrad_group_plan(d, n, &cfg, &ns, &pps);
  return align_up((int64_t)n * ns * d->R * d->S * d->C * d->K * 4, 256);
}
int mtlssl_conv2d_wgrad_grouped(const mtlssl_conv_desc* d, int n, const void* x_ptrs, const void* dy_ptrs,
                                const void* scale_ptrs, const void* dw_ptrs, float beta, void* workspace,
                                mtlssl_stream_t stream) {
  if (n <= 0) return MTLSSL_OK;
  if (int rc = check_desc(d)) return rc;
  MTLSSL_REQUIRE(mfma_wgrad_ok(d), "wgrad_grouped: the problem is not on the MFMA path (C, K multiples of 4 and >= 16)");
  MTLSSL_REQUIRE(x_ptrs && dy_ptrs && dw_ptrs && workspace, "wgrad_grouped: null table / workspace");
  MTLSSL_REQUIRE(n <= 1024, "wgrad_grouped: at most 1024 problems per launch");
  hipStream_t st = S(stream);
  ConvArgs p = make_args(d);
  p.a_bytes = (unsigned)((int64_t)d->N * d->H * d->W * d->C * 4);
  p.b_bytes = ydy_bytes(d);
  p.a_tab = (const float* const*)x_ptrs;
  p.b_tab = (const float* const*)dy_ptrs;
  int cfg, ns, pps;
  wgrad_group_plan(d, n, &cfg, &ns, &pps);
  MTLSSL_REQUIRE((int64_t)n * ns <= 65535, "wgrad_grouped: grid too large");
  p.out = (float*)workspace;
  p.M = d->C; p.NG = d->K; p.nsplit = ns; p.pix_per_split = pps;
  launch_mfma<MODE_WGRAD>(cfg, p, dim3(1, d->R * d->S, n * ns), st);
  const int64_t total4 = (int64_t)d->R * d->S * d->C * d->K / 4;
  hipLaunchKernelGGL(k_wgrad_reduce_grouped, dim3(cdiv(total4 * 4, 256), n), dim3(256), 0, st, (const float*)workspace, ns,
                     total4, d->K, (const float* const*)scale_ptrs, (float* const*)dw_ptrs, beta);
  return check_launch("conv2d_wgrad_grouped");
}

int mtlssl_conv2d_wgrad(const mtlssl_conv_desc* d, const float* x, const float* dy,
                        const float* out_scale, float* dw, float* dbias, float beta,
                        void* workspace, mtlssl_stream_t stream) {
  return mtlssl_conv2d_wgrad_xf(d, x, dy, out_scale, dw, dbias, beta, workspace, nullptr, -1, stream);
}

int mtlssl_conv2d_wgrad_xf(const mtlssl_conv_desc* d, const float* x, const float* dy,
                           const float* out_scale, float* dw, float* dbias, float beta,
                           void* workspace, const float* input_xf, int input_variant, mtlssl_stream_t stream) {
  return mtlssl_conv2d_wgrad_ex(d, x, dy, out_scale, dw, dbias, nullptr, beta, workspace, input_xf, input_variant, stream);
}

int mtlssl_conv2d_wgrad_ex(const mtlssl_conv_desc* d, const float* x, const float* dy,
                           const float* out_scale, float* dw, float* dbias, const float* dbias_scale, float beta,
                           void* workspace, const float* input_xf, int input_variant, mtlssl_stream_t stream) {
  return mtlssl_conv2d_wgrad_rs(d, x, dy, out_scale, dw, dbias, dbias_scale, beta, workspace, input_xf, input_variant,
                                nullptr, 0, stream);
}

int mtlssl_conv2d_wgrad_rs(const mtlssl_conv_desc* d, const float* x, const float* dy,
                           const float* out_scale, float* dw, float* dbias, const float* dbias_scale, float beta,
                           void* workspace, const float* input_xf, int input_variant, const uint8_t* group_active,
                           int rows_per_group, mtlssl_stream_t stream) {
  if (int rc = check_desc(d)) return rc;
  MTLSSL_REQUIRE(!group_active || rows_per_group > 0, "conv_wgrad: group_active needs rows_per_group > 0");
  hipStream_t st = S(stream);
  ConvArgs p = make_args(d);
  p.a = x; p.b = dy;
  p.a_bytes = (unsigned)((int64_t)d->N * d->H * d->W * d->C * 4);
  p.b_bytes = ydy_bytes(d);
  const int ldy = desc_ldy(d);
  MTLSSL_REQUIRE(desc_dense(d) || mfma_wgrad_ok(d),
                 "conv_wgrad: a strided dy (ldy = %d) needs C, K %% 4 == 0 and C, K >= 16", d->ldy);
  int64_t P = (int64_t)d->N * d->OH * d->OW;
  MTLSSL_REQUIRE(workspace != nullptr, "conv_wgrad: workspace required");
  float* ws_main = (float*)((char*)workspace + colsum_bytes(d));
  ColsumPlan cp = colsum_plan(P, d->K);
  bool colsum_folded = false;
  auto colsum_partial = [&]() {
    const int kg = (int)cdiv(d->K, (d->K & 3) ? 1 : 4);
    dim3 grid(cdiv(kg, cp.CQ), cp.chunks);
    if (d->K & 3)
      hipLaunchKernelGGL(k_colsum_partial<float>, grid, dim3(256), 0, st, dy, (int)P, d->K, ldy, cp.per_chunk, cp.CQ,
                         (float*)workspace);
    else
      hipLaunchKernelGGL(k_colsum_partial<floatx4>, grid, dim3(256), 0, st, dy, (int)P, d->K, ldy, cp.per_chunk, cp.CQ,
                         (float*)workspace);
  };
  const Route r = route(d, MODE_WGRAD);
  switch (r.family) {
    case FAM_WINO:
      wino_wgrad(d, r.wc.variant, r.wc.tile, x, dy, out_scale, dw, beta, ws_main, st,
                 (input_xf && input_variant == r.wc.variant) ? input_xf : nullptr,
                 (group_active && row_skip_ref().load() != 0 && rows_per_group == d->OH * d->OW) ? group_active : nullptr);
      break;
    case FAM_DIRECT: {
      const bool split = wgrad_on_split_engine(r, d);
      const int ns = split ? r.split_ns : r.wg.nsplit, pps = split ? r.split_pps : r.wg.pps;
      const bool ride = dbias && !split && ns <= COLSUM_MAX_PARTS;
      if (dbias && !ride) colsum_partial();
      p.out = ws_main;
      p.M = d->C; p.NG = d->K; p.nsplit = ns; p.pix_per_split = pps;
      p.cs_part = ride ? (float*)workspace : nullptr;
      if (group_active && row_skip_ref().load() != 0 && !split && desc_is_pointwise(d) && pointwise_ref().load() != 0 &&
          ns <= KSTEP_HDR) {
        int* list = (int*)((char*)ws_main + r.bytes);
        const int stride = (int)cdiv(pps, BK);
        hipLaunchKernelGGL(k_active_ksteps, dim3(ns), dim3(256), 0, st, group_active, rows_per_group, (int)P, pps, stride, list);
        p.k_steps = list;
        p.k_stride = stride;
      }
      if (split) launch_split_direct<MODE_WGRAD>(p, dim3(1, d->R * d->S, ns), st);
      else launch_mfma<MODE_WGRAD>(r.wg.cfg, p, dim3(1, d->R * d->S, ns), st);
      int64_t total4 = (int64_t)d->R * d->S * d->C * d->K / 4;
      const int main_blocks = (int)cdiv(total4 * 4, 256);
      hipLaunchKernelGGL(k_wgrad_reduce, dim3(main_blocks + (dbias ? (int)cdiv(d->K, 4) : 0)), dim3(256), 0, st,
                         (const float*)ws_main, ns, total4, d->K, out_scale, dw, beta, main_blocks,
                         (const float*)workspace, ride ? ns : cp.chunks, dbias, dbias_scale);
      colsum_folded = dbias != nullptr;
      break;
    }
    case FAM_PADDED: {
      const mtlssl_conv_desc& q = r.q;
      const int ns = r.wg.nsplit;
      float* dy_pad = ws_main;
      float* ws_q = (float*)((char*)ws_main + r.front_bytes);
// ... 43 lines not shown
```

mtl_ssl_amd/csrc/conv_mfma.h:

```cpp
#pragma once
#include <type_traits>

#include "common.h"

namespace mtlssl {

typedef float floatx16 __attribute__((ext_vector_type(16)));
typedef float floatx4 __attribute__((ext_vector_type(4)));

enum { MODE_FWD = 0, MODE_DGRAD = 1, MODE_WGRAD = 2 };
__device__ __forceinline__ float act_mask(float g, float y, int epi) {
  bool on = y > 0.f && (!(epi & MTLSSL_EPI_MASK6) || y < 6.f);
  return on ? g : 0.f;
}
constexpr int MASK_ANY = MTLSSL_EPI_MASK | MTLSSL_EPI_MASK6;
constexpr int BK = 16;
#ifndef MTLSSL_LAB_FLAGS
#define MTLSSL_LAB_FLAGS 0
#endif
constexpr int LAB = MTLSSL_LAB_FLAGS;

struct ConvArgs {
  const float* a;
  const float* b;
  float* out;
  const float* bias;
  const float* residual;
  const float* mask;
  float* splitk_ws;
  int N, H, W, C, K, R, S, OH, OW, stride, dil, pt, pl;
  int M;
  int NG;
  int epi;
  int tiles_m, tiles_n;
  unsigned a_bytes, b_bytes;
  int nsplit;
  int ks_per_split;
  int pix_per_split;
  int tile_m0;
  int ws_m0;
  int ldy;
  float* cs_part;
  int64_t a_bs, b_bs, o_bs;
  const float* const* a_tab;
  const float* const* b_tab;
  const uint8_t* group_active;
  int rows_per_group;
  const int* k_steps;
  int k_stride;
};
constexpr int KSTEP_HDR = 64;

__device__ __forceinline__ bool tile_rows_active(const ConvArgs& p, int m0, int bm) {
  const int g1 = (min(m0 + bm, p.M) - 1) / p.rows_per_group;
  bool any = false;
  for (int g = m0 / p.rows_per_group; g <= g1; ++g) any |= p.group_active[g] != 0;
  return any;
}

typedef unsigned uintx4 __attribute__((ext_vector_type(4)));
__host__ __device__ __forceinline__ int args_ldy(const ConvArgs& p) { return p.ldy ? p.ldy : p.K; }

__device__ __forceinline__ floatx4 bufload4(__amdgpu_buffer_rsrc_t rsrc, unsigned voffset,
                                            unsigned soffset) {
  return __builtin_bit_cast(floatx4, __builtin_amdgcn_raw_buffer_load_b128(rsrc, voffset, soffset, 0));
}

template <int BM, int BN, int MODE, int NW, bool PREFETCH_RES = false>
__device__ __forceinline__ void conv_epilogue(const ConvArgs& p, floatx16 (&acc)[BM / (16 * NW)][BN / 64], float* smem,
                                              int m0, int n0) {
  constexpr int WR = NW / 2, TM = BM / (32 * WR), TN = BN / 64, LDT = 36;
  const int tid = threadIdx.x, lane = tid & 63, wid = tid >> 6;
  const int wr = wid >> 1, wc = wid & 1;
  const int lo = lane & 31, hi = lane >> 5;
  if constexpr (LAB & 16)
    if (p.epi != 0x7fffffff) {
      float t = 0.f;
#pragma unroll
      for (int i = 0; i < TM; ++i)
#pragma unroll
        for (int j = 0; j < TN; ++j)
#pragma unroll
          for (int e = 0; e < 16; ++e) t += acc[i][j][e];
      if (t == 1.2345e-30f) p.out[0] = t;
      return;
    }
  const int ldo = p.NG;
  const int ldf = MODE == MODE_FWD ? args_ldy(p) : p.NG;
  float* outp = p.out;
  if constexpr (MODE == MODE_WGRAD)
    outp += ((int64_t)blockIdx.z * gridDim.y + blockIdx.y) * (int64_t)p.M * p.NG;
  const bool raw = (MODE != MODE_WGRAD) && p.nsplit > 1;
  if (raw) outp = p.splitk_ws + (int64_t)blockIdx.z * (int64_t)(p.M - p.ws_m0) * p.NG;
  if (!(p.NG & 3)) {
    float* tile = smem + wid * (32 * LDT);
    const int r_in = lane >> 3, c4 = (lane & 7) * 4;
    const bool use_res = PREFETCH_RES && !raw && (MODE == MODE_FWD || MODE == MODE_DGRAD) && (p.epi & MTLSSL_EPI_RESIDUAL);
    floatx4 res_cur[4], res_nxt[4];
    auto fetch_res = [&](int t, floatx4 (&dst)[4]) {
      const int i = t / TN, j = t % TN;
      const int col = n0 + wc * (BN / 2) + j * 32 + c4;
#pragma unroll
      for (int k = 0; k < 4; ++k) {
        const int row = m0 + wr * (BM / WR) + i * 32 + r_in + 8 * k;
        dst[k] = floatx4{0.f, 0.f, 0.f, 0.f};
        if (use_res && row < p.M && col < p.NG) dst[k] = *reinterpret_cast<const floatx4*>(p.residual + (int64_t)row * ldo + col);
      }
    };
    if constexpr (PREFETCH_RES) fetch_res(0, res_cur);
#pragma unroll
    for (int i = 0; i < TM; ++i) {
#pragma unroll
      for (int j = 0; j < TN; ++j) {
        if constexpr (PREFETCH_RES)
          if (i * TN + j + 1 < TM * TN) fetch_res(i * TN + j + 1, res_nxt);
#pragma unroll
        for (int e = 0; e < 16; ++e) tile[((e & 3) + 8 * (e >> 2) + 4 * hi) * LDT + lo] = acc[i][j][e];
        const int col = n0 + wc * (BN / 2) + j * 32 + c4;
        floatx4 bv = {0.f, 0.f, 0.f, 0.f};
        if constexpr (MODE == MODE_FWD)
          if ((p.epi & MTLSSL_EPI_BIAS) && col < p.NG && !raw) bv = *reinterpret_cast<const floatx4*>(p.bias + col);
#pragma unroll
        for (int k = 0; k < 4; ++k) {
          const int rt = r_in + 8 * k;
          floatx4 v = *reinterpret_cast<const floatx4*>(tile + rt * LDT + c4);
          const int row = m0 + wr * (BM / WR) + i * 32 + rt;
          if (row >= p.M || col >= p.NG) continue;
          if (raw) {
            *reinterpret_cast<floatx4*>(outp + (int64_t)(row - p.ws_m0) * ldo + col) = v;
            continue;
          }
          const int64_t o = (int64_t)row * ldo + col;
          const int64_t of = MODE == MODE_FWD ? (int64_t)row * ldf + col : o;
          if constexpr (MODE == MODE_FWD) {
            v += bv;
            if (p.epi & MTLSSL_EPI_RESIDUAL) v += PREFETCH_RES ? res_cur[k] : *reinterpret_cast<const floatx4*>(p.residual + o);
#pragma unroll
            for (int q = 0; q < 4; ++q) {
              if (p.epi & MTLSSL_EPI_RELU) v[q] = fmaxf(v[q], 0.f);
              if (p.epi & MTLSSL_EPI_RELU6) v[q] = fminf(fmaxf(v[q], 0.f), 6.f);
              if (p.epi & MTLSSL_EPI_TANH) v[q] = tanhf(v[q]);
            }
          } else if constexpr (MODE == MODE_DGRAD) {
            if (p.epi & MTLSSL_EPI_RESIDUAL) v += PREFETCH_RES ? res_cur[k] : *reinterpret_cast<const floatx4*>(p.residual + o);
            if (p.epi & MTLSSL_EPI_ACCUM) v += *reinterpret_cast<const floatx4*>(outp + o);
            if (p.epi & MASK_ANY) {
              floatx4 mk = *reinterpret_cast<const floatx4*>(p.mask + o);
#pragma unroll
              for (int q = 0; q < 4; ++q) v[q] = act_mask(v[q], mk[q], p.epi);
            }
          }
          *reinterpret_cast<floatx4*>(outp + of) = v;
        }
        if constexpr (PREFETCH_RES) {
#pragma unroll
          for (int k = 0; k < 4; ++k) res_cur[k] = res_nxt[k];
        }
      }
    }
    return;
  }
#pragma unroll
  for (int i = 0; i < TM; ++i) {
#pragma unroll
    for (int j = 0; j < TN; ++j) {
      const int col = n0 + wc * (BN / 2) + j * 32 + lo;
      const bool col_ok = col < p.NG;
      float bv = 0.f;
      if constexpr (MODE == MODE_FWD)
        if ((p.epi & MTLSSL_EPI_BIAS) && col_ok) bv = p.bias[col];
#pragma unroll
      for (int e = 0; e < 16; ++e) {
        const int row = m0 + wr * (BM / WR) + i * 32 + (e & 3) + 8 * (e >> 2) + 4 * hi;
        if (row >= p.M || !col_ok) continue;
        const int64_t o = (int64_t)row * ldo + col;
        const int64_t of = MODE == MODE_FWD ? (int64_t)row * ldf + col : o;
        float v = acc[i][j][e];
        if (raw) {
          outp[(int64_t)(row - p.ws_m0) * ldo + col] = v;
          continue;
        }
        if constexpr (MODE == MODE_FWD) {
          v += bv;
          if (p.epi & MTLSSL_EPI_RESIDUAL) v += p.residual[o];
          if (p.epi & MTLSSL_EPI_RELU) v = fmaxf(v, 0.f);
          if (p.epi & MTLSSL_EPI_RELU6) v = fminf(fmaxf(v, 0.f), 6.f);
          if (p.epi & MTLSSL_EPI_TANH) v = tanhf(v);
        } else if constexpr (MODE == MODE_DGRAD) {
          if (p.epi & MTLSSL_EPI_RESIDUAL) v += p.residual[o];
          if (p.epi & MTLSSL_EPI_ACCUM) v += outp[o];
          if (p.epi & MASK_ANY) v = act_mask(v, p.mask[o], p.epi);
        }
        outp[of] = v;
      }
    }
  }
}

struct SegArgs { mtlssl_conv_seg_entry e[MTLSSL_CONV_GROUP_MAX]; };
template <int BM, int BN, int MODE, int BKT, bool BATCH, bool PW = false, bool CS = false, bool SEG = false>
__device__ __forceinline__ void conv_mfma_body(ConvArgs p, const SegArgs sg = SegArgs{}) {
  static_assert(!SEG || (PW && MODE == MODE_DGRAD && !BATCH), "segments: pointwise dgrad only");
  constexpr int NW = BM > 128 ? 8 : 4, NT = 64 * NW, WR = NW / 2;
  constexpr int LDA = BM + 4, LDB = BN + 4;
  constexpr int KQ = BKT / 4;
  constexpr int RP = NT / KQ;
  constexpr int TM = BM / (32 * WR), TN = BN / 64;
  constexpr bool A_KC = (MODE != MODE_WGRAD);
  constexpr bool B_KC = (MODE == MODE_DGRAD);
  constexpr int A_LD = BM / RP, B_LD = BN / RP;
  constexpr unsigned OOB = 0xFFFFFFF0u;
  constexpr int LDT = 36;
  constexpr int SMEM_OPS = 2 * BKT * (LDA + LDB), SMEM_EPI = NW * 32 * LDT;
  __shared__ __attribute__((aligned(16))) float smem[SMEM_OPS > SMEM_EPI ? SMEM_OPS : SMEM_EPI];
  float* const sA = smem;
  float* const sB = smem + 2 * BKT * LDA;

  int nwg = p.tiles_m * p.tiles_n;
  int bid = blockIdx.x;
  {
    int q = nwg / 8, r = nwg % 8, xcd = bid % 8, loc = bid / 8;
    bid = (xcd < r ? xcd * (q + 1) : r * (q + 1) + (xcd - r) * q) + loc;
  }
  if constexpr (BATCH && MODE == MODE_DGRAD)
    if (p.group_active) bid = (int)((bid + (unsigned)blockIdx.y * ((nwg + 7) / 8)) % (unsigned)nwg);
  const int tile_m = bid / p.tiles_n + p.tile_m0, tile_n = bid % p.tiles_n;
  const int m0 = tile_m * BM, n0 = tile_n * BN;
  const int tid = threadIdx.x, lane = tid & 63, wid = tid >> 6;
  const int wr = wid >> 1, wc = wid & 1;
  const int lo = lane & 31, hi = lane >> 5;
  const int kq4 = (tid % KQ) * 4;

  if constexpr (BATCH) {
    p.a += (int64_t)blockIdx.y * p.a_bs;
    p.b += (int64_t)blockIdx.y * p.b_bs;
    if constexpr (MODE != MODE_WGRAD) p.out += (int64_t)blockIdx.y * p.o_bs;
  }
  if constexpr (MODE == MODE_WGRAD && !BATCH) {
    if (p.a_tab) {
      const int grp = blockIdx.z / p.nsplit;
      p.a = p.a_tab[grp];
      p.b = p.b_tab[grp];
    }
  }
  const int ldy = args_ldy(p);
  int rs_fixed = 0, pix0 = 0, pix1 = 0, ksteps, ks_begin = 0;
  const int* steps = nullptr;
  if constexpr (MODE == MODE_FWD) {
    ksteps = p.R * p.S * (p.C / BKT);
  } else if constexpr (MODE == MODE_DGRAD) {
    ksteps = p.R * p.S * (p.K / BKT);
  } else {
    rs_fixed = BATCH ? 0 : blockIdx.y;
    int split = (!BATCH && p.a_tab) ? blockIdx.z % p.nsplit : blockIdx.z;
    int P = p.N * p.OH * p.OW;
    pix0 = split * p.pix_per_split;
    pix1 = min(P, pix0 + p.pix_per_split);
    ksteps = (max(pix1 - pix0, 0) + BKT - 1) / BKT;
    if constexpr (PW)
      if (p.k_steps) {
        steps = p.k_steps + KSTEP_HDR + split * p.k_stride;
        ksteps = p.k_steps[split];
      }
  }
  unsigned a_rec = p.a_bytes, b_rec = p.b_bytes;
  if constexpr (PW && MODE == MODE_WGRAD) {
    a_rec = min(a_rec, (unsigned)(max(pix1, 0) * p.C) * 4u);
    b_rec = min(b_rec, (unsigned)(max(pix1, 0) * ldy) * 4u);
  }
  __amdgpu_buffer_rsrc_t rsrc_a = __builtin_amdgcn_make_buffer_rsrc(const_cast<float*>(p.a), 0, a_rec, 0x00020000);
  __amdgpu_buffer_rsrc_t rsrc_b = __builtin_amdgcn_make_buffer_rsrc(const_cast<float*>(p.b), 0, b_rec, 0x00020000);
  if constexpr (MODE != MODE_WGRAD) {
    if (p.nsplit > 1) {
      ks_begin = blockIdx.z * p.ks_per_split;
      ksteps = min(ksteps, ks_begin + p.ks_per_split);
    }
  }
  if constexpr (PW && MODE == MODE_DGRAD && !SEG)
    if (p.group_active && !tile_rows_active(p, m0, BM)) {
      if constexpr (BATCH) return;
      ksteps = ks_begin;
    }

  int a_base[A_LD], a_y[A_LD], a_x[A_LD], a_n[A_LD];
  bool a_ok[A_LD];
  unsigned a_voff[A_LD];
  unsigned b_base[B_LD];
  if constexpr (PW && MODE == MODE_WGRAD) {
#pragma unroll
    for (int i = 0; i < A_LD; ++i) {
      const int u = tid + NT * i;
      const int col = m0 + (u % (BM / 4)) * 4;
      a_voff[i] = col < p.M ? (unsigned)((pix0 + u / (BM / 4)) * p.C + col) * 4u : OOB;
    }
  } else if constexpr (PW) {
#pragma unroll
    for (int i = 0; i < A_LD; ++i) {
      const int m = m0 + (tid / KQ) + RP * i;
      const int ld = MODE == MODE_FWD ? p.C : ldy;
      a_voff[i] = m < p.M ? (unsigned)(m * ld + kq4) * 4u : OOB;
    }
  } else if constexpr (A_KC) {
#pragma unroll
    for (int i = 0; i < A_LD; ++i) {
      int m = m0 + (tid / KQ) + RP * i;
      a_ok[i] = m < p.M;
      int mm = a_ok[i] ? m : 0;
      if constexpr (MODE == MODE_FWD) {
        int ow = mm % p.OW, t = mm / p.OW;
        a_x[i] = ow * p.stride - p.pl;
        a_y[i] = (t % p.OH) * p.stride - p.pt;
        a_n[i] = t / p.OH;
        a_base[i] = ((a_n[i] * p.H + a_y[i]) * p.W + a_x[i]) * p.C + kq4;
      } else {
        int iw = mm % p.W, t = mm / p.W;
        a_x[i] = iw + p.pl;
        a_y[i] = (t % p.H) + p.pt;
        a_n[i] = t / p.H;
        a_base[i] = ((a_n[i] * p.OH + a_y[i]) * p.OW + a_x[i]) * ldy + kq4;
      }
    }
  }
#pragma unroll
  for (int i = 0; i < B_LD; ++i) {
    if constexpr (MODE == MODE_FWD) {
      int u = tid + NT * i;
      int col = n0 + (u % (BN / 4)) * 4;
      b_base[i] = col < p.NG ? (unsigned)((u / (BN / 4)) * p.K + col) * 4u : OOB;
    } else if constexpr (MODE == MODE_DGRAD) {
      int row = n0 + (tid / KQ) + RP * i;
      b_base[i] = row < p.NG ? (unsigned)(row * p.K + kq4) * 4u : OOB;
    } else {
      int u = tid + NT * i;
      int col = n0 + (u % (BN / 4)) * 4;
      if constexpr (PW)
        b_base[i] = col < p.NG ? (unsigned)((pix0 + u / (BN / 4)) * ldy + col) * 4u : OOB;
      else
        b_base[i] = col < p.NG ? (unsigned)col * 4u : OOB;
    }
  }

  int seg_ks0 = 0;
  int seg_b[MTLSSL_CONV_GROUP_MAX] = {0, 0, 0, 0};
  auto seg_setup = [&](auto SI) {
    constexpr int s = decltype(SI)::value;
    const int e_K = sg.e[s].K;
    const int ld = sg.e[s].ldy ? sg.e[s].ldy : e_K;
    rsrc_a = __builtin_amdgcn_make_buffer_rsrc(const_cast<float*>(sg.e[s].dy), 0, (unsigned)((p.M - 1) * ld + e_K) * 4u, 0x00020000);
    rsrc_b = __builtin_amdgcn_make_buffer_rsrc(const_cast<float*>(sg.e[s].w), 0, (unsigned)(p.NG * e_K) * 4u, 0x00020000);
#pragma unroll
    for (int i = 0; i < A_LD; ++i) {
      const int m = m0 + (tid / KQ) + RP * i;
      a_voff[i] = m < p.M ? (unsigned)(m * ld + kq4) * 4u : OOB;
    }
#pragma unroll
    for (int i = 0; i < B_LD; ++i) {
      const int row = n0 + (tid / KQ) + RP * i;
      b_base[i] = row < p.NG ? (unsigned)(row * e_K + kq4) * 4u : OOB;
    }
    seg_ks0 = seg_b[s];
  };
  if constexpr (SEG) {
    static_assert(MTLSSL_CONV_GROUP_MAX == 4, "the boundary ladder in load_tile covers four segments");
    int at = 0;
#pragma unroll
    for (int s = 0; s < MTLSSL_CONV_GROUP_MAX; ++s) {
      seg_b[s] = sg.e[s].K > 0 ? at : 0x7fffffff;
      at += sg.e[s].K / BKT;
    }
    seg_setup(std::integral_constant<int, 0>{});
  }

  int t_r = 0, t_s = 0, t_c = 0;
  if constexpr (!PW && MODE != MODE_WGRAD) {
    const int cpk = (MODE == MODE_FWD ? p.C : p.K) / BKT;
    const int rs = ks_begin / cpk;
    t_c = (ks_begin - rs * cpk) * BKT;
    t_r = rs / p.S;
    t_s = rs - t_r * p.S;
  }
  auto next_tap = [&]() {
    t_c += BKT;
    if (t_c >= (MODE == MODE_FWD ? p.C : p.K)) {
      t_c = 0;
      if (++t_s == p.S) { t_s = 0; ++t_r; }
    }
  };
  int w_n[A_LD], w_oh[A_LD], w_ow[A_LD];
  if constexpr (!PW && MODE == MODE_WGRAD) {
#pragma unroll
    for (int i = 0; i < A_LD; ++i) {
      const int pix = pix0 + (tid + NT * i) / (BM / 4);
      w_ow[i] = pix % p.OW;
      const int t = pix / p.OW;
      w_oh[i] = t % p.OH;
      w_n[i] = t / p.OH;
    }
  }

  floatx4 rA[2][A_LD], rB[2][B_LD];
  using Set0 = std::integral_constant<int, 0>;
  using Set1 = std::integral_constant<int, 1>;

  auto load_tile = [&](int ks, auto SET) {
    floatx4 (&ra)[A_LD] = rA[decltype(SET)::value];
    floatx4 (&rb)[B_LD] = rB[decltype(SET)::value];
    if constexpr (PW && MODE == MODE_WGRAD) {
      const unsigned sa = (unsigned)(ks * BKT * p.C) * 4u, sb = (unsigned)(ks * BKT * ldy) * 4u;
#pragma unroll
      for (int i = 0; i < A_LD; ++i) ra[i] = bufload4(rsrc_a, __builtin_elementwise_add_sat(a_voff[i], sa), 0);
#pragma unroll
      for (int i = 0; i < B_LD; ++i) rb[i] = bufload4(rsrc_b, __builtin_elementwise_add_sat(b_base[i], sb), 0);
    } else if constexpr (PW) {
      if constexpr (SEG) {
        if (ks == seg_b[1]) seg_setup(std::integral_constant<int, 1>{});
        else if (ks == seg_b[2]) seg_setup(std::integral_constant<int, 2>{});
        else if (ks == seg_b[3]) seg_setup(std::integral_constant<int, 3>{});
      }
      const unsigned ka = (unsigned)((SEG ? ks - seg_ks0 : ks) * BKT) * 4u;
#pragma unroll
      for (int i = 0; i < A_LD; ++i) ra[i] = bufload4(rsrc_a, a_voff[i], ka);
      const unsigned so = MODE == MODE_FWD ? (unsigned)(ks * BKT * p.K) * 4u : ka;
#pragma unroll
      for (int i = 0; i < B_LD; ++i) rb[i] = bufload4(rsrc_b, b_base[i], so);
      if constexpr (MODE == MODE_FWD)
        if (p.NG & 3) {
#pragma unroll
          for (int i = 0; i < B_LD; ++i) {
            int left = p.NG - (n0 + ((tid + NT * i) % (BN / 4)) * 4);
#pragma unroll
            for (int e = 1; e < 4; ++e) rb[i][e] = e < left ? rb[i][e] : 0.f;
          }
        }
    } else if constexpr (MODE == MODE_FWD) {
      const int dy = t_r * p.dil, dx = t_s * p.dil;
      const int tapoff = (dy * p.W + dx) * p.C + t_c;
      next_tap();
#pragma unroll
      for (int i = 0; i < A_LD; ++i) {
        int ih = a_y[i] + dy, iw = a_x[i] + dx;
        bool ok = a_ok[i] && (unsigned)ih < (unsigned)p.H && (unsigned)iw < (unsigned)p.W;
        ra[i] = bufload4(rsrc_a, ok ? (unsigned)(a_base[i] + tapoff) * 4u : OOB, 0);
      }
      unsigned so = (unsigned)(ks * BKT * p.K) * 4u;
#pragma unroll
      for (int i = 0; i < B_LD; ++i) rb[i] = bufload4(rsrc_b, b_base[i], so);
      if (p.NG & 3) {
#pragma unroll
        for (int i = 0; i < B_LD; ++i) {
          int left = p.NG - (n0 + ((tid + NT * i) % (BN / 4)) * 4);
#pragma unroll
          for (int e = 1; e < 4; ++e) rb[i][e] = e < left ? rb[i][e] : 0.f;
        }
      }
    } else if constexpr (MODE == MODE_DGRAD) {
      const int rs = t_r * p.S + t_s, k0 = t_c;
      const int dy = t_r * p.dil, dx = t_s * p.dil;
      next_tap();
      if (p.stride == 1) {
        int tapoff = k0 - (dy * p.OW + dx) * ldy;
#pragma unroll
        for (int i = 0; i < A_LD; ++i) {
          int oh = a_y[i] - dy, ow = a_x[i] - dx;
          bool ok = a_ok[i] && (unsigned)oh < (unsigned)p.OH && (unsigned)ow < (unsigned)p.OW;
          ra[i] = bufload4(rsrc_a, ok ? (unsigned)(a_base[i] + tapoff) * 4u : OOB, 0);
        }
      } else {
#pragma unroll
        for (int i = 0; i < A_LD; ++i) {
          int ny = a_y[i] - dy, nx = a_x[i] - dx;
          bool ok = a_ok[i] && ny >= 0 && nx >= 0 && (ny % p.stride == 0) && (nx % p.stride == 0);
          int oh = ny / p.stride, ow = nx / p.stride;
          ok = ok && oh < p.OH && ow < p.OW;
          int off = ((a_n[i] * p.OH + oh) * p.OW + ow) * ldy + k0 + kq4;
          ra[i] = bufload4(rsrc_a, ok ? (unsigned)off * 4u : OOB, 0);
        }
      }
      unsigned so = (unsigned)(rs * p.C * p.K + k0) * 4u;
#pragma unroll
      for (int i = 0; i < B_LD; ++i) rb[i] = bufload4(rsrc_b, b_base[i], so);
    } else {
      int r = rs_fixed / p.S, s = rs_fixed - r * p.S;
#pragma unroll
      for (int i = 0; i < A_LD; ++i) {
        int u = tid + NT * i;
        int kr = u / (BM / 4), m4 = u % (BM / 4);
        int pix = pix0 + ks * BKT + kr;
        bool ok = pix < pix1;
        const int ih = w_oh[i] * p.stride - p.pt + r * p.dil, iw = w_ow[i] * p.stride - p.pl + s * p.dil;
        ok = ok && (unsigned)ih < (unsigned)p.H && (unsigned)iw < (unsigned)p.W && (m0 + m4 * 4) < p.M;
        const int off = ((w_n[i] * p.H + ih) * p.W + iw) * p.C;
        ra[i] = bufload4(rsrc_a, ok ? (unsigned)(off + m0 + m4 * 4) * 4u : OOB, 0);
        w_ow[i] += BKT;
        while (w_ow[i] >= p.OW) {
          w_ow[i] -= p.OW;
          if (++w_oh[i] == p.OH) { w_oh[i] = 0; ++w_n[i]; }
        }
      }
#pragma unroll
      for (int i = 0; i < B_LD; ++i) {
        int u = tid + NT * i;
        int pix = pix0 + ks * BKT + u / (BN / 4);
        rb[i] = bufload4(rsrc_b, (pix < pix1 && b_base[i] != OOB) ? b_base[i] + (unsigned)(pix * ldy) * 4u : OOB, 0);
      }
    }
  };

  static_assert(!CS || (MODE == MODE_WGRAD && !BATCH), "column sums ride on the plain wgrad launch only");
  bool do_cs = false;
  floatx4 cs[CS ? B_LD : 1];
  if constexpr (CS) {
    do_cs = p.cs_part != nullptr && tile_m == 0 && rs_fixed == 0 && p.a_tab == nullptr;
#pragma unroll
    for (int i = 0; i < B_LD; ++i) cs[i] = floatx4{0.f, 0.f, 0.f, 0.f};
  }
  auto store_tile = [&](int buf, auto SET) {
    floatx4 (&ra)[A_LD] = rA[decltype(SET)::value];
    floatx4 (&rb)[B_LD] = rB[decltype(SET)::value];
    float* a = sA + buf * (BKT * LDA);
    float* b = sB + buf * (BKT * LDB);
    if constexpr (CS)
      if (do_cs) {
#pragma unroll
        for (int i = 0; i < B_LD; ++i) cs[i] += rb[i];
      }
#pragma unroll
    for (int i = 0; i < A_LD; ++i) {
      if constexpr (A_KC) {
        int row = (tid / KQ) + RP * i;
        a[(kq4 + 0) * LDA + row] = ra[i].x; a[(kq4 + 1) * LDA + row] = ra[i].y;
        a[(kq4 + 2) * LDA + row] = ra[i].z; a[(kq4 + 3) * LDA + row] = ra[i].w;
      } else {
        int u = tid + NT * i;
        *reinterpret_cast<floatx4*>(a + (u / (BM / 4)) * LDA + (u % (BM / 4)) * 4) = ra[i];
      }
    }
#pragma unroll
    for (int i = 0; i < B_LD; ++i) {
      if constexpr (B_KC) {
        int row = (tid / KQ) + RP * i;
        b[(kq4 + 0) * LDB + row] = rb[i].x; b[(kq4 + 1) * LDB + row] = rb[i].y;
        b[(kq4 + 2) * LDB + row] = rb[i].z; b[(kq4 + 3) * LDB + row] = rb[i].w;
      } else {
        int u = tid + NT * i;
        *reinterpret_cast<floatx4*>(b + (u / (BN / 4)) * LDB + (u % (BN / 4)) * 4) = rb[i];
      }
    }
  };

  floatx16 acc[TM][TN];
#pragma unroll
  for (int i = 0; i < TM; ++i)
#pragma unroll
    for (int j = 0; j < TN; ++j)
#pragma unroll
      for (int e = 0; e < 16; ++e) acc[i][j][e] = 0.f;

  const int nk = ksteps - ks_begin;
  auto kmap = [&](int it) { return steps ? steps[it] : ks_begin + it; };
  int step_pf = 0;
  if (nk > 0) {
    load_tile(kmap(0), Set0{});
    store_tile(0, Set0{});
  }
  if (nk > 1) load_tile(kmap(1), Set1{});
  if (steps && nk > 2) step_pf = steps[2];
  __syncthreads();
  auto kstep = [&](int it, auto next, auto spare) {
    const int cur = it & 1;
    if constexpr (!(LAB & 1))
      if (it + 2 < nk) {
        load_tile(steps ? step_pf : ks_begin + it + 2, spare);
        if (steps && it + 3 < nk) step_pf = steps[it + 3];
      }
    const float* a = sA + cur * (BKT * LDA) + wr * (BM / WR) + lo;
    const float* b = sB + cur * (BKT * LDB) + wc * (BN / 2) + lo;
    float fa[2][TM], fb[2][TN];
#pragma unroll
    for (int i = 0; i < TM; ++i) fa[0][i] = a[hi * LDA + i * 32];
#pragma unroll
    for (int j = 0; j < TN; ++j) fb[0][j] = b[hi * LDB + j * 32];
#pragma unroll
    for (int kk = 0; kk < BKT / 2; ++kk) {
      const int cs = kk & 1, ns = cs ^ 1;
      if (kk + 1 < BKT / 2) {
        const int kr = 2 * (kk + 1) + hi;
        if constexpr (LAB & 8) {
#pragma unroll
          for (int i = 0; i < TM; ++i) fa[ns][i] = fa[cs][i] * 1.0001f;
#pragma unroll
          for (int j = 0; j < TN; ++j) fb[ns][j] = fb[cs][j] * 0.9999f;
        } else {
#pragma unroll
          for (int i = 0; i < TM; ++i) fa[ns][i] = a[kr * LDA + i * 32];
#pragma unroll
          for (int j = 0; j < TN; ++j) fb[ns][j] = b[kr * LDB + j * 32];
        }
      }
      __builtin_amdgcn_sched_barrier(0);
#pragma unroll
      for (int i = 0; i < TM; ++i)
#pragma unroll
        for (int j = 0; j < TN; ++j)
          acc[i][j] = __builtin_amdgcn_mfma_f32_32x32x2f32(fa[cs][i], fb[cs][j], acc[i][j], 0, 0, 0);
      __builtin_amdgcn_sched_barrier(0);
    }
    if constexpr (!(LAB & 2))
      if (it + 1 < nk) store_tile(cur ^ 1, next);
    if constexpr (!(LAB & 4)) __syncthreads();
  };
  for (int it = 0; it < nk; it += 2) {
    kstep(it, Set1{}, Set0{});
    if (it + 1 < nk) kstep(it + 1, Set0{}, Set1{});
  }

  if constexpr (CS) {
    if (do_cs) {
      floatx4* red = reinterpret_cast<floatx4*>(smem);
#pragma unroll
      for (int i = 0; i < B_LD; ++i) red[tid + NT * i] = cs[i];
      __syncthreads();
      if (tid < BN / 4) {
        floatx4 t = red[tid];
#pragma unroll
        for (int r = 1; r < BKT; ++r) t += red[r * (BN / 4) + tid];
        const int col = n0 + tid * 4;
        if (col < p.NG) *reinterpret_cast<floatx4*>(p.cs_part + (int64_t)blockIdx.z * p.NG + col) = t;
      }
      __syncthreads();
    }
  }
  conv_epilogue<BM, BN, MODE, NW>(p, acc, smem, m0, n0);
}


template <int BM, int BN, int MODE, int BKT, int NSTAGE, bool BATCH, bool PWISE = false, bool CS = false>
__device__ __forceinline__ void conv_glds_body(ConvArgs p) {
  constexpr int NW = BM > 128 ? 8 : 4, WR = NW / 2;
  constexpr int TM = BM / (32 * WR), TN = BN / 64;
  constexpr bool A_KC = (MODE != MODE_WGRAD);
  constexpr bool B_KC = (MODE == MODE_DGRAD);
  constexpr int QPR = BKT / 4;
  constexpr int RPP = 64 / QPR;
  constexpr int RSH = QPR == 4 ? 2 : 1;
  constexpr int A_FL = BM * BKT, B_FL = BN * BKT;
  constexpr int STAGE = A_FL + B_FL;
  constexpr int PA = BM * BKT / 256 / NW, PB = BN * BKT / 256 / NW;
  constexpr int G = BKT / 8;
  constexpr unsigned OOB = 0xFFFFFFF0u;
  constexpr int LDT = 36;
  constexpr int SMEM_OPS = NSTAGE * STAGE, SMEM_EPI = NW * 32 * LDT;
  __shared__ __attribute__((aligned(16))) float smem[SMEM_OPS > SMEM_EPI ? SMEM_OPS : SMEM_EPI];
  typedef __attribute__((address_space(3))) void* lds_ptr_t;

  int nwg = p.tiles_m * p.tiles_n;
  int bid = blockIdx.x;
  {
    int q = nwg / 8, r = nwg % 8, xcd = bid % 8, loc = bid / 8;
    bid = (xcd < r ? xcd * (q + 1) : r * (q + 1) + (xcd - r) * q) + loc;
  }
  if constexpr (BATCH && MODE == MODE_DGRAD)
    if (p.group_active) bid = (int)((bid + (unsigned)blockIdx.y * ((nwg + 7) / 8)) % (unsigned)nwg);
  const int tile_m = bid / p.tiles_n + p.tile_m0, tile_n = bid % p.tiles_n;
  const int m0 = tile_m * BM, n0 = tile_n * BN;
  const int tid = threadIdx.x, lane = tid & 63, wid = tid >> 6;
  const int wr = wid >> 1, wc = wid & 1;
  const int lo = lane & 31, hi = lane >> 5;
  auto kc_row = [&](int piece) { return piece * RPP + lane / QPR; };
  auto kc_quad4 = [&](int row) { return (((lane % QPR) ^ ((row >> RSH) & (QPR - 1)))) * 4; };

  if constexpr (BATCH) {
    p.a += (int64_t)blockIdx.y * p.a_bs;
    p.b += (int64_t)blockIdx.y * p.b_bs;
    if constexpr (MODE != MODE_WGRAD) p.out += (int64_t)blockIdx.y * p.o_bs;
  }
  int rs_fixed = 0, pix0 = 0, pix1 = 0, ksteps, ks_begin = 0;
  const int* steps = nullptr;
  if constexpr (MODE == MODE_FWD) {
    ksteps = p.R * p.S * (p.C / BKT);
  } else if constexpr (MODE == MODE_DGRAD) {
    ksteps = p.R * p.S * (p.K / BKT);
  } else {
    rs_fixed = BATCH ? 0 : blockIdx.y;
    int split = blockIdx.z;
    int P = p.N * p.OH * p.OW;
    pix0 = split * p.pix_per_split;
    pix1 = min(P, pix0 + p.pix_per_split);
    ksteps = (max(pix1 - pix0, 0) + BKT - 1) / BKT;
    if constexpr (PWISE)
      if (p.k_steps) {
        steps = p.k_steps + KSTEP_HDR + split * p.k_stride;
        ksteps = p.k_steps[split];
      }
  }
  if constexpr (MODE != MODE_WGRAD) {
    if (p.nsplit > 1) {
      ks_begin = blockIdx.z * p.ks_per_split;
      ksteps = min(ksteps, ks_begin + p.ks_per_split);
    }
  }
  if constexpr (PWISE && MODE == MODE_DGRAD)
    if (p.group_active && !tile_rows_active(p, m0, BM)) {
      if constexpr (BATCH) return;
      ksteps = ks_begin;
    }

  const int ldy = args_ldy(p);
  unsigned a_rec = p.a_bytes, b_rec = p.b_bytes;
  if constexpr (PWISE && MODE == MODE_WGRAD) {
    a_rec = min(a_rec, (unsigned)(max(pix1, 0) * p.C) * 4u);
    b_rec = min(b_rec, (unsigned)(max(pix1, 0) * ldy) * 4u);
  }
  const __amdgpu_buffer_rsrc_t rsrc_a = __builtin_amdgcn_make_buffer_rsrc(const_cast<float*>(p.a), 0, a_rec, 0x00020000);
  const __amdgpu_buffer_rsrc_t rsrc_b = __builtin_amdgcn_make_buffer_rsrc(const_cast<float*>(p.b), 0, b_rec, 0x00020000);

  int a_base[PA], a_y[PA], a_x[PA], a_n[PA], a_q4[PA];
  bool a_ok[PA];
  unsigned a_voff[PA];
  unsigned b_base[PB];
  if constexpr (PWISE && MODE == MODE_WGRAD) {
#pragma unroll
    for (int i = 0; i < PA; ++i) {
      const int pos = (wid * PA + i) * 64 + lane;
      const int col = m0 + (pos % (BM / 4)) * 4;
      a_voff[i] = col < p.M ? (unsigned)((pix0 + pos / (BM / 4)) * p.C + col) * 4u : OOB;
    }
  } else if constexpr (PWISE) {
#pragma unroll
    for (int i = 0; i < PA; ++i) {
      const int row = kc_row(wid * PA + i);
      const int m = m0 + row;
      a_voff[i] = m < p.M ? (unsigned)(m * (MODE == MODE_FWD ? p.C : ldy) + kc_quad4(row)) * 4u : OOB;
    }
  } else if constexpr (A_KC) {
#pragma unroll
    for (int i = 0; i < PA; ++i) {
      const int row = kc_row(wid * PA + i);
      a_q4[i] = kc_quad4(row);
      int m = m0 + row;
      a_ok[i] = m < p.M;
      int mm = a_ok[i] ? m : 0;
      if constexpr (MODE == MODE_FWD) {
        int ow = mm % p.OW, t = mm / p.OW;
        a_x[i] = ow * p.stride - p.pl;
        a_y[i] = (t % p.OH) * p.stride - p.pt;
        a_n[i] = t / p.OH;
        a_base[i] = ((a_n[i] * p.H + a_y[i]) * p.W + a_x[i]) * p.C + a_q4[i];
      } else {
        int iw = mm % p.W, t = mm / p.W;
        a_x[i] = iw + p.pl;
        a_y[i] = (t % p.H) + p.pt;
        a_n[i] = t / p.H;
        a_base[i] = ((a_n[i] * p.OH + a_y[i]) * p.OW + a_x[i]) * ldy + a_q4[i];
      }
    }
  }
#pragma unroll
  for (int i = 0; i < PB; ++i) {
    const int pos = (wid * PB + i) * 64 + lane;
    if constexpr (MODE == MODE_FWD) {
      int col = n0 + (pos % (BN / 4)) * 4;
      b_base[i] = col < p.NG ? (unsigned)((pos / (BN / 4)) * p.K + col) * 4u : OOB;
    } else if constexpr (MODE == MODE_DGRAD) {
      const int row = kc_row(wid * PB + i);
      b_base[i] = n0 + row < p.NG ? (unsigned)((n0 + row) * p.K + kc_quad4(row)) * 4u : OOB;
    } else {
      int col = n0 + (pos % (BN / 4)) * 4;
      if constexpr (PWISE)
        b_base[i] = col < p.NG ? (unsigned)((pix0 + pos / (BN / 4)) * ldy + col) * 4u : OOB;
      else
        b_base[i] = col < p.NG ? (unsigned)col * 4u : OOB;
    }
  }

  auto issue_tile = [&](int ks, int st) {
    if constexpr (LAB & 32) ks = ks_begin;
    float* sa = smem + st * STAGE + wid * (PA * 256);
    float* sb = smem + st * STAGE + A_FL + wid * (PB * 256);
    if constexpr (PWISE && MODE == MODE_WGRAD) {
      const unsigned sa_off = (unsigned)(ks * BKT * p.C) * 4u, sb_off = (unsigned)(ks * BKT * ldy) * 4u;
#pragma unroll
      for (int i = 0; i < PA; ++i)
        __builtin_amdgcn_raw_ptr_buffer_load_lds(rsrc_a, (lds_ptr_t)(sa + i * 256), 16, __builtin_elementwise_add_sat(a_voff[i], sa_off), 0, 0, 0);
#pragma unroll
      for (int i = 0; i < PB; ++i)
        __builtin_amdgcn_raw_ptr_buffer_load_lds(rsrc_b, (lds_ptr_t)(sb + i * 256), 16, __builtin_elementwise_add_sat(b_base[i], sb_off), 0, 0, 0);
    } else if constexpr (PWISE) {
      const unsigned ka = (unsigned)(ks * BKT) * 4u;
      const unsigned so = MODE == MODE_FWD ? (unsigned)(ks * BKT * p.K) * 4u : ka;
#pragma unroll
      for (int i = 0; i < PA; ++i)
        __builtin_amdgcn_raw_ptr_buffer_load_lds(rsrc_a, (lds_ptr_t)(sa + i * 256), 16, a_voff[i], ka, 0, 0);
#pragma unroll
      for (int i = 0; i < PB; ++i)
        __builtin_amdgcn_raw_ptr_buffer_load_lds(rsrc_b, (lds_ptr_t)(sb + i * 256), 16, b_base[i], so, 0, 0);
    } else if constexpr (MODE == MODE_FWD) {
      int cpk = p.C / BKT;
      int rs = ks / cpk, c0 = (ks - rs * cpk) * BKT;
      int r = rs / p.S, s = rs - r * p.S;
      int dy = r * p.dil, dx = s * p.dil;
      int tapoff = (dy * p.W + dx) * p.C + c0;
      if constexpr (!(LAB & 64)) {
#pragma unroll
        for (int i = 0; i < PA; ++i) {
          int ih = a_y[i] + dy, iw = a_x[i] + dx;
          bool ok = a_ok[i] && (unsigned)ih < (unsigned)p.H && (unsigned)iw < (unsigned)p.W;
          __builtin_amdgcn_raw_ptr_buffer_load_lds(rsrc_a, (lds_ptr_t)(sa + i * 256), 16,
                                                   ok ? (unsigned)(a_base[i] + tapoff) * 4u : OOB, 0, 0, 0);
        }
      }
      unsigned so = (unsigned)(ks * BKT * p.K) * 4u;
      if constexpr (!(LAB & 128)) {
#pragma unroll
        for (int i = 0; i < PB; ++i)
          __builtin_amdgcn_raw_ptr_buffer_load_lds(rsrc_b, (lds_ptr_t)(sb + i * 256), 16, b_base[i], so, 0, 0);
      }
    } else if constexpr (MODE == MODE_DGRAD) {
      int kpk = p.K / BKT;
      int rs = ks / kpk, k0 = (ks - rs * kpk) * BKT;
      int r = rs / p.S, s = rs - r * p.S;
      int dy = r * p.dil, dx = s * p.dil;
      if (p.stride == 1) {
        int tapoff = k0 - (dy * p.OW + dx) * ldy;
#pragma unroll
        for (int i = 0; i < PA; ++i) {
          int oh = a_y[i] - dy, ow = a_x[i] - dx;
          bool ok = a_ok[i] && (unsigned)oh < (unsigned)p.OH && (unsigned)ow < (unsigned)p.OW;
          __builtin_amdgcn_raw_ptr_buffer_load_lds(rsrc_a, (lds_ptr_t)(sa + i * 256), 16,
                                                   ok ? (unsigned)(a_base[i] + tapoff) * 4u : OOB, 0, 0, 0);
        }
      } else {
#pragma unroll
        for (int i = 0; i < PA; ++i) {
          int ny = a_y[i] - dy, nx = a_x[i] - dx;
          bool ok = a_ok[i] && ny >= 0 && nx >= 0 && (ny % p.stride == 0) && (nx % p.stride == 0);
          int oh = ny / p.stride, ow = nx / p.stride;
          ok = ok && oh < p.OH && ow < p.OW;
          int off = ((a_n[i] * p.OH + oh) * p.OW + ow) * ldy + k0 + a_q4[i];
          __builtin_amdgcn_raw_ptr_buffer_load_lds(rsrc_a, (lds_ptr_t)(sa + i * 256), 16,
                                                   ok ? (unsigned)off * 4u : OOB, 0, 0, 0);
        }
      }
      unsigned so = (unsigned)(rs * p.C * p.K + k0) * 4u;
#pragma unroll
      for (int i = 0; i < PB; ++i)
        __builtin_amdgcn_raw_ptr_buffer_load_lds(rsrc_b, (lds_ptr_t)(sb + i * 256), 16, b_base[i], so, 0, 0);
    } else {
      int r = rs_fixed / p.S, s = rs_fixed - r * p.S;
#pragma unroll
      for (int i = 0; i < PA; ++i) {
        const int pos = (wid * PA + i) * 64 + lane;
        int kr = pos / (BM / 4), m4 = pos % (BM / 4);
        int pix = pix0 + ks * BKT + kr;
        bool ok = pix < pix1;
        int off = 0;
        if (p.R == 1 && p.S == 1 && p.stride == 1) {
          off = pix * p.C;
        } else {
          int ow = pix % p.OW, t = pix / p.OW;
          int oh = t % p.OH, n = t / p.OH;
          int ih = oh * p.stride - p.pt + r * p.dil, iw = ow * p.stride - p.pl + s * p.dil;
          ok = ok && (unsigned)ih < (unsigned)p.H && (unsigned)iw < (unsigned)p.W;
          off = ((n * p.H + ih) * p.W + iw) * p.C;
        }
        ok = ok && (m0 + m4 * 4) < p.M;
        __builtin_amdgcn_raw_ptr_buffer_load_lds(rsrc_a, (lds_ptr_t)(sa + i * 256), 16,
                                                 ok ? (unsigned)(off + m0 + m4 * 4) * 4u : OOB, 0, 0, 0);
      }
#pragma unroll
      for (int i = 0; i < PB; ++i) {
        const int pos = (wid * PB + i) * 64 + lane;
        int pix = pix0 + ks * BKT + pos / (BN / 4);
        __builtin_amdgcn_raw_ptr_buffer_load_lds(
            rsrc_b, (lds_ptr_t)(sb + i * 256), 16,
            (pix < pix1 && b_base[i] != OOB) ? b_base[i] + (unsigned)(pix * ldy) * 4u : OOB, 0, 0, 0);
      }
    }
  };

  floatx16 acc[TM][TN];
#pragma unroll
  for (int i = 0; i < TM; ++i)
#pragma unroll
    for (int j = 0; j < TN; ++j)
#pragma unroll
      for (int e = 0; e < 16; ++e) acc[i][j][e] = 0.f;

  int fa_off[TM], fb_off[TN];
#pragma unroll
  for (int i = 0; i < TM; ++i) {
    const int row = wr * (BM / WR) + i * 32 + lo;
    fa_off[i] = A_KC ? row * BKT + (((hi * (QPR / 2)) ^ ((row >> RSH) & (QPR - 1))) * 4) : hi * (BKT / 2) * BM + row;
  }
#pragma unroll
  for (int j = 0; j < TN; ++j) {
    const int col = wc * (BN / 2) + j * 32 + lo;
    fb_off[j] = B_KC ? col * BKT + (((hi * (QPR / 2)) ^ ((col >> RSH) & (QPR - 1))) * 4) : hi * (BKT / 2) * BN + col;
  }

  const int nk = ksteps - ks_begin;
  constexpr int NDMA = ((LAB & 64) ? 0 : PA) + ((LAB & 128) ? 0 : PB);
  int step_pf = 0;
#pragma unroll
  for (int s = 0; s < NSTAGE - 1; ++s)
    if (s < nk) issue_tile(steps ? steps[s] : ks_begin + s, s);
  if (steps && NSTAGE - 1 < nk) step_pf = steps[NSTAGE - 1];
  if (NSTAGE == 3 && nk > 1) asm volatile("s_waitcnt vmcnt(%0)" ::"n"(NDMA) : "memory");
  else asm volatile("s_waitcnt vmcnt(0)" ::: "memory");
  __builtin_amdgcn_s_barrier();
  asm volatile("" ::: "memory");

  bool do_cs = false;
  float csum = 0.f;
  static_assert(!CS || (MODE == MODE_WGRAD && !BATCH), "column sums ride on the plain wgrad launch only");
  if constexpr (CS) do_cs = p.cs_part != nullptr && tile_m == 0 && rs_fixed == 0;
  int cur = 0, nxt = NSTAGE - 1;
  for (int it = 0; it < nk; ++it) {
    const bool more = it + NSTAGE - 1 < nk;
    if constexpr (!(LAB & 1))
      if (more) {
        issue_tile(steps ? step_pf : ks_begin + it + NSTAGE - 1, nxt);
        if (steps && it + NSTAGE < nk) step_pf = steps[it + NSTAGE];
      }
    const float* a = smem + cur * STAGE;
    const float* b = a + A_FL;
    if constexpr (CS)
      if (do_cs && tid < BN) {
#pragma unroll
        for (int k = 0; k < BKT; ++k) csum += b[k * BN + tid];
      }
    float fa[TM][BKT / 2], fb[TN][BKT / 2];
    auto read_group = [&](auto GI) {
      constexpr int g = decltype(GI)::value;
#pragma unroll
      for (int i = 0; i < TM; ++i) {
        if constexpr (A_KC) {
          floatx4 v = *reinterpret_cast<const floatx4*>(a + (fa_off[i] ^ (g * 4)));
          fa[i][4 * g + 0] = v.x; fa[i][4 * g + 1] = v.y; fa[i][4 * g + 2] = v.z; fa[i][4 * g + 3] = v.w;
        } else {
#pragma unroll
          for (int t = 0; t < 4; ++t) fa[i][4 * g + t] = a[fa_off[i] + (4 * g + t) * BM];
        }
      }
#pragma unroll
      for (int j = 0; j < TN; ++j) {
        if constexpr (B_KC) {
          floatx4 v = *reinterpret_cast<const floatx4*>(b + (fb_off[j] ^ (g * 4)));
          fb[j][4 * g + 0] = v.x; fb[j][4 * g + 1] = v.y; fb[j][4 * g + 2] = v.z; fb[j][4 * g + 3] = v.w;
        } else {
#pragma unroll
          for (int t = 0; t < 4; ++t) fb[j][4 * g + t] = b[fb_off[j] + (4 * g + t) * BN];
        }
      }
    };
    auto mma = [&](int t) {
#pragma unroll
      for (int i = 0; i < TM; ++i)
#pragma unroll
        for (int j = 0; j < TN; ++j)
          acc[i][j] = __builtin_amdgcn_mfma_f32_32x32x2f32(fa[i][t], fb[j][t], acc[i][j], 0, 0, 0);
    };
    if constexpr (LAB & 8) {
#pragma unroll
      for (int t = 0; t < BKT / 2; ++t) {
#pragma unroll
        for (int i = 0; i < TM; ++i) fa[i][t] = (float)(lane + it + t) * 1e-3f;
#pragma unroll
        for (int j = 0; j < TN; ++j) fb[j][t] = (float)(lane - it - t) * 1e-3f;
      }
#pragma unroll
      for (int t = 0; t < BKT / 2; ++t) mma(t);
    } else {
      read_group(std::integral_constant<int, 0>{});
      auto group = [&](auto GI) {
        constexpr int g = decltype(GI)::value;
        __builtin_amdgcn_sched_barrier(0);
        mma(4 * g);
        __builtin_amdgcn_sched_barrier(0);
        if constexpr (g + 1 < G) read_group(std::integral_constant<int, g + 1>{});
        __builtin_amdgcn_sched_barrier(0);
        mma(4 * g + 1); mma(4 * g + 2); mma(4 * g + 3);
      };
      group(std::integral_constant<int, 0>{});
      group(std::integral_constant<int, 1>{});
      if constexpr (G > 2) {
        group(std::integral_constant<int, 2>{});
        group(std::integral_constant<int, 3>{});
      }
    }
    __builtin_amdgcn_sched_barrier(0);
    if constexpr (!(LAB & 4)) {
      if (NSTAGE == 3 && more) asm volatile("s_waitcnt vmcnt(%0)" ::"n"(NDMA) : "memory");
      else asm volatile("s_waitcnt vmcnt(0)" ::: "memory");
      __builtin_amdgcn_s_barrier();
    }
    asm volatile("" ::: "memory");
    cur = cur + 1 == NSTAGE ? 0 : cur + 1;
    nxt = nxt + 1 == NSTAGE ? 0 : nxt + 1;
  }
  if constexpr (CS)
    if (do_cs && tid < BN && n0 + tid < p.NG) p.cs_part[(int64_t)blockIdx.z * p.NG + n0 + tid] = csum;
  conv_epilogue<BM, BN, MODE, NW>(p, acc, smem, m0, n0);
}

template <int BM, int BN, int BKT, int NSTAGE>
constexpr int glds_waves() {
  constexpr int lds = NSTAGE * (BM + BN) * BKT * 4;
  constexpr int nw = BM > 128 ? 8 : 4;
  constexpr int blocks = 163840 / lds;
  constexpr int w = blocks * nw / 4;
  return w > 4 ? 4 : (w < 1 ? 1 : w);
}
template <int BM, int BN, int MODE, int BKT, int NSTAGE>
__global__ void __launch_bounds__(BM > 128 ? 512 : 256, (glds_waves<BM, BN, BKT, NSTAGE>()))
k_conv_glds(ConvArgs p) {
  conv_glds_body<BM, BN, MODE, BKT, NSTAGE, false>(p);
}
template <int BM, int BN, int MODE, int BKT, int NSTAGE>
__global__ void __launch_bounds__(BM > 128 ? 512 : 256, (glds_waves<BM, BN, BKT, NSTAGE>()))
k_conv_glds_pw(ConvArgs p) {
  conv_glds_body<BM, BN, MODE, BKT, NSTAGE, false, true>(p);
}
template <int BM, int BN, int BKT, int NSTAGE>
__global__ void __launch_bounds__(BM > 128 ? 512 : 256, (glds_waves<BM, BN, BKT, NSTAGE>()))
k_conv_glds_cs(ConvArgs p) {
  conv_glds_body<BM, BN, MODE_WGRAD, BKT, NSTAGE, false, false, true>(p);
}
template <int BM, int BN, int BKT, int NSTAGE>
__global__ void __launch_bounds__(BM > 128 ? 512 : 256, (glds_waves<BM, BN, BKT, NSTAGE>()))
k_conv_glds_pw_cs(ConvArgs p) {
  conv_glds_body<BM, BN, MODE_WGRAD, BKT, NSTAGE, false, true, true>(p);
}
template <int BM, int BN, int MODE, int BKT, int NSTAGE>
__global__ void __launch_bounds__(BM > 128 ? 512 : 256, (glds_waves<BM, BN, BKT, NSTAGE>()))
k_wino_glds(ConvArgs p) {
  conv_glds_body<BM, BN, MODE, BKT, NSTAGE, true, true>(p);
}

template <int BM, int BN, int MODE, int BKT>
__global__ void __launch_bounds__(BM > 128 ? 512 : 256, (BM > 128 ? 2 : BM * BN >= 128 * 128 ? (BKT > 16 ? 2 : 3) : 4))
k_conv_mfma(ConvArgs p) {
  conv_mfma_body<BM, BN, MODE, BKT, false>(p);
}
template <int BM, int BN, int MODE>
__global__ void __launch_bounds__(BM > 128 ? 512 : 256, (BM > 128 ? 2 : BM * BN >= 128 * 128 ? 3 : 4))
k_conv_mfma_pw(ConvArgs p) {
  conv_mfma_body<BM, BN, MODE, 16, false, true>(p);
}
template <int BM, int BN, int BKT>
__global__ void __launch_bounds__(BM > 128 ? 512 : 256, (BM > 128 ? 2 : BM * BN >= 128 * 128 ? (BKT > 16 ? 2 : 3) : 4))
k_conv_mfma_cs(ConvArgs p) {
  conv_mfma_body<BM, BN, MODE_WGRAD, BKT, false, false, true>(p);
}
template <int BM, int BN>
__global__ void __launch_bounds__(BM > 128 ? 512 : 256, (BM > 128 ? 2 : BM * BN >= 128 * 128 ? 3 : 4))
k_conv_mfma_pw_cs(ConvArgs p) {
  conv_mfma_body<BM, BN, MODE_WGRAD, 16, false, true, true>(p);
}
struct GroupArgs { mtlssl_conv_group_entry e[MTLSSL_CONV_GROUP_MAX]; };
template <int BM, int BN>
__global__ void __launch_bounds__(BM > 128 ? 512 : 256, (BM > 128 ? 2 : BM * BN >= 128 * 128 ? 3 : 4))
k_conv_mfma_pw_grp(ConvArgs p, GroupArgs g) {
  static_assert(MTLSSL_CONV_GROUP_MAX == 4, "the select chain below covers four problems");
  const int gy = blockIdx.y;
  const mtlssl_conv_group_entry e = gy == 0 ? g.e[0] : gy == 1 ? g.e[1] : gy == 2 ? g.e[2] : g.e[3];
  p.b = e.w; p.out = e.y; p.bias = e.bias;
  p.NG = e.K; p.K = e.K; p.ldy = e.ldy; p.epi = e.epilogue;
  p.b_bytes = (unsigned)(p.C * e.K) * 4u;
  p.tiles_n = (e.K + BN - 1) / BN;
  if ((int)blockIdx.x >= p.tiles_m * p.tiles_n) return;
  conv_mfma_body<BM, BN, MODE_FWD, 16, false, true>(p);
}
template <int BM, int BN>
__global__ void __launch_bounds__(BM > 128 ? 512 : 256, (BM > 128 ? 2 : BM * BN >= 128 * 128 ? 3 : 4))
k_conv_mfma_pw_seg(ConvArgs p, SegArgs g) {
  conv_mfma_body<BM, BN, MODE_DGRAD, 16, false, true, false, true>(p, g);
}
inline bool conv_is_pointwise(const ConvArgs& p) {
  return p.R == 1 && p.S == 1 && p.stride == 1 && p.dil == 1 && p.pt == 0 && p.pl == 0 && p.OH == p.H && p.OW == p.W;
}
template <int BM, int BN, int MODE>
__global__ void __launch_bounds__(BM > 128 ? 512 : 256, (BM > 128 ? 2 : BM * BN >= 128 * 128 ? 3 : 4))
k_wino_gemm(ConvArgs p) {
  conv_mfma_body<BM, BN, MODE, 16, true, true>(p);
}

constexpr int NCFG = 4;
constexpr int NTILE = 8;
static const int CFG_BM[NTILE] = {128, 128, 64, 256, 128, 128, 64, 256};
static const int CFG_BN[NTILE] = {128, 64, 64, 128, 128, 64, 64, 128};
static const int CFG_BK[NTILE] = {16, 16, 16, 16, 16, 16, 16, 16};
static const int CFG_THREADS[NTILE] = {256, 256, 256, 512, 256, 256, 256, 512};
static const int CFG_RESIDENT[NTILE] = {3, 6, 8, 2, 3, 6, 8, 2};
constexpr int GLDS_STAGES = 2;

static inline double tile_time_us(int cfg, int64_t nblocks, int ksteps_per_block, bool pointwise = false) {
  const double eff_general[NCFG] = {0.80, 0.76, 0.72, 0.78}, eff_pointwise[NCFG] = {0.90, 0.88, 0.87, 0.90};
  const double* base_eff = pointwise ? eff_pointwise : eff_general;
  int64_t per_cu = cdiv(nblocks, 256);
  int64_t occ = per_cu < CFG_RESIDENT[cfg] ? per_cu : CFG_RESIDENT[cfg];
  if ((cfg & 3) == 3) occ *= 2;
  double occ_eff = occ <= 1 ? 0.55 : (occ == 2 ? 0.80 : 1.0);
  double step_us = CFG_BM[cfg] * CFG_BN[cfg] * 2.0 * CFG_BK[cfg] / 614e9 * 1e6 / (base_eff[cfg & 3] * occ_eff);
  return (double)per_cu * (ksteps_per_block + 96 / CFG_BK[cfg]) * step_us;
}

enum { WINO_F43 = 0, WINO_M7 = 1, WINO_VARIANTS = 2 };
bool wino_eligible(const mtlssl_conv_desc* d, int variant);
double wino_time_us(const mtlssl_conv_desc* d, int variant, int mode, int* tile);
int64_t wino_workspace_bytes(const mtlssl_conv_desc* d, int variant, int mode);
void wino_fwd(const mtlssl_conv_desc* d, int variant, int tile, const float* x, const float* w, const float* bias,
              const float* residual, float* y, int epi, void* workspace, hipStream_t st, const float* filter_xf = nullptr,
              float* input_xf_keep = nullptr);
int64_t wino_input_bytes(const mtlssl_conv_desc* d, int variant);
void wino_dgrad(const mtlssl_conv_desc* d, int variant, int tile, const float* dy, const float* w,
                const float* residual, const float* mask_ref, float* dx, int epi, void* workspace, hipStream_t st,
                const float* filter_xf = nullptr, const uint8_t* batch_active = nullptr);
int64_t wino_filter_bytes(const mtlssl_conv_desc* d, int variant);
void wino_filter(const mtlssl_conv_desc* d, int variant, int flip, const float* w, float* U, hipStream_t st);
void wino_filters_batched(int variant, int n, const void* w_ptrs, const void* u_ptrs, const int64_t* ck,
                          const int32_t* flip, int64_t max_ck, hipStream_t st);
void wino_wgrad(const mtlssl_conv_desc* d, int variant, int tile, const float* x, const float* dy,
                const float* out_scale, float* dw, float beta, void* workspace, hipStream_t st,
                const float* input_xf = nullptr, const uint8_t* batch_active = nullptr);
void wino_wgrad_split(const mtlssl_conv_desc* d, int variant, int tile, int* ns, int* pps);

}
```

mtl_ssl_amd/csrc/winograd.hip:

```cpp
#include "conv_mfma.h"
#include "conv_split.h"

namespace mtlssl {

namespace {

struct F43 {
  static constexpr int P = 6, I = 6, O = 4;
  static constexpr float bt(int a, int i) {
    constexpr float t[6][6] = {{4, 0, -5, 0, 1, 0}, {0, -4, -4, 1, 1, 0}, {0, 4, -4, -1, 1, 0},
                               {0, -2, -1, 2, 1, 0}, {0, 2, -1, -2, 1, 0}, {0, 4, 0, -5, 0, 1}};
    return t[a][i];
  }
  static constexpr float at(int u, int a) {
    constexpr float t[4][6] = {{1, 1, 1, 1, 1, 0}, {0, 1, -1, 2, -2, 0}, {0, 1, 1, 4, 4, 0}, {0, 1, -1, 8, -8, 1}};
    return t[u][a];
  }
  static constexpr float g(int a, int r) {
    constexpr float t[6][3] = {{1.f / 4, 0, 0}, {-1.f / 6, -1.f / 6, -1.f / 6}, {-1.f / 6, 1.f / 6, -1.f / 6},
                               {1.f / 24, 1.f / 12, 1.f / 6}, {1.f / 24, -1.f / 12, 1.f / 6}, {0, 0, 1}};
    return t[a][r];
  }
};
struct F33 {
// ... 290 lines not shown
  for (int r = 0; r < 3; ++r) {
    VT o[3];
    xform<S, XF_GT, 3, P>(t[r], o);
#pragma unroll
    for (int s = 0; s < 3; ++s) {
      VT v = scale ? o[s] * sc : o[s];
      VT* p = reinterpret_cast<VT*>(dw + (int64_t)(r * 3 + s) * CK + i);
      *p = beta != 0.f ? beta * *p + v : v;
    }
  }
}

__global__ void __launch_bounds__(256) k_wino_active_tiles(const uint8_t* __restrict__ flags, int tpg, int T,
                                                           int* __restrict__ slot, int* __restrict__ row_src,
                                                           uint8_t* __restrict__ gflags) {
  const int lane = threadIdx.x & 63, w = threadIdx.x >> 6;
  __shared__ int wave_cnt[4];
  int base = 0;
  for (int t0 = 0; t0 < T; t0 += 256) {
    const int t = t0 + threadIdx.x;
    const bool act = t < T && flags[t / tpg] != 0;
    const unsigned long long m = __ballot(act);
    if (lane == 0) wave_cnt[w] = __popcll(m);
    __syncthreads();
    int off = base;
    for (int i = 0; i < w; ++i) off += wave_cnt[i];
    const int row = off + __popcll(m & ((1ull << lane) - 1ull));
    if (t < T) slot[t] = act ? row : -1;
    if (act) row_src[row] = t;
    base += wave_cnt[0] + wave_cnt[1] + wave_cnt[2] + wave_cnt[3];
    __syncthreads();
  }
  for (int r = base + threadIdx.x; r < T; r += 256) row_src[r] = ROW_SKIP;
  for (int i = threadIdx.x; i < (T + 63) / 64; i += 256) gflags[i] = i * 64 < base;
}
__global__ void __launch_bounds__(256) k_wino_active_pairs(const uint8_t* __restrict__ flags, int tpg, int T, int pps, int glds,
                                                           int stride, int* __restrict__ row_src, int* __restrict__ out) {
  const int z = blockIdx.x, pix0 = z * pps, pix1 = min(T, pix0 + pps);
  const int npairs = (max(pix1 - pix0, 0) + BK - 1) / BK * (BK / 2);
  const int lane = threadIdx.x & 63, w = threadIdx.x >> 6;
  auto row_of = [&](int q, int h) { return pix0 + BK * (q >> 3) + (glds ? (q & 7) + 8 * h : 2 * (q & 7) + h); };
  auto live = [&](int r) { return r < pix1 && flags[r / tpg] != 0; };
  __shared__ int wave_cnt[4];
  int base = 0;
  for (int q0 = 0; q0 < npairs; q0 += 256) {
    const int q = q0 + threadIdx.x;
    const bool act = q < npairs && (live(row_of(q, 0)) || live(row_of(q, 1)));
    const unsigned long long m = __ballot(act);
    if (lane == 0) wave_cnt[w] = __popcll(m);
    __syncthreads();
    int off = base;
    for (int i = 0; i < w; ++i) off += wave_cnt[i];
    if (act) {
      const int j = off + __popcll(m & ((1ull << lane) - 1ull));
      for (int h = 0; h < 2; ++h) {
        const int dst = row_of(j, h), src = row_of(q, h);
        if (dst < pix1) row_src[dst] = src < pix1 ? src : ROW_ZERO;
      }
    }
    base += wave_cnt[0] + wave_cnt[1] + wave_cnt[2] + wave_cnt[3];
    __syncthreads();
  }
  const int ksteps = (base + 7) / 8;
  for (int j = base + threadIdx.x; j < npairs; j += 256)
    for (int h = 0; h < 2; ++h) {
      const int dst = row_of(j, h);
      if (dst < pix1) row_src[dst] = j < ksteps * 8 ? ROW_ZERO : ROW_SKIP;
    }
  if (threadIdx.x == 0) out[z] = ksteps;
  for (int i = threadIdx.x; i < ksteps; i += 256) out[KSTEP_HDR + (int64_t)z * stride + i] = i;
}
__global__ void __launch_bounds__(256) k_wino_gather_rows(const float* __restrict__ src, float* __restrict__ dst,
                                                          const int* __restrict__ row_src, int64_t T, int C) {
  const int cq = C / 4;
  const int64_t idx = blockIdx.x * (int64_t)256 + threadIdx.x;
  if (idx >= T * cq) return;
  const int64_t r = idx / cq;
  const int c = (int)(idx % cq) * 4;
  const int m = row_src[r];
  if (m == ROW_SKIP) return;
  const int64_t plane = (int64_t)blockIdx.y * T * C;
  floatx4 v = {0.f, 0.f, 0.f, 0.f};
  if (m >= 0) v = *reinterpret_cast<const floatx4*>(src + plane + (int64_t)m * C + c);
  *reinterpret_cast<floatx4*>(dst + plane + r * C + c) = v;
}

typedef float floatx2 __attribute__((ext_vector_type(2)));

template <typename S>
WinoGeom geom(const mtlssl_conv_desc* d) {
  WinoGeom g;
  g.N = d->N; g.H = d->H; g.W = d->W;
  g.th = (int)cdiv(d->H, S::O); g.tw = (int)cdiv(d->W, S::O);
  g.T = (int64_t)d->N * g.th * g.tw;
  return g;
}

template <typename S> constexpr bool can_vec() { return S::P <= 6; }
inline bool wide(int64_t T, int C) { return T * C / 4 >= 131072; }

template <typename S>
void run_filter(const float* w, float* U, int64_t CK, int flip, hipStream_t st) {
  if constexpr (can_vec<S>()) {
    if (CK >= 262144) {
      hipLaunchKernelGGL((k_wino_filter<S, floatx4>), dim3(cdiv(CK / 4, 256)), dim3(256), 0, st, w, U, CK, flip);
      return;
    }
  }
  hipLaunchKernelGGL((k_wino_filter<S, float>), dim3(cdiv(CK, 256)), dim3(256), 0, st, w, U, CK, flip);
}
template <typename S>
void run_input(const float* in, float* V, const WinoGeom& g, int C, hipStream_t st, int ld = 0,
               const int* row_src = nullptr) {
  if (ld <= 0) ld = C;
  if constexpr (can_vec<S>()) {
    if (wide(g.T, C)) {
      hipLaunchKernelGGL((k_wino_input<S, floatx4>), dim3(cdiv(g.T * C / 4, 256)), dim3(256), 0, st, in, V, g, C, ld,
                         row_src);
      return;
    }
  }
  hipLaunchKernelGGL((k_wino_input<S, float>), dim3(cdiv(g.T * C, 256)), dim3(256), 0, st, in, V, g, C, ld, row_src);
}
template <typename S>
void run_dy(const float* dy, float* dM, const WinoGeom& g, int K, hipStream_t st, int ld = 0,
            const int* row_src = nullptr) {
  if (ld <= 0) ld = K;
  if constexpr (can_vec<S>()) {
    if (wide(g.T, K)) {
      hipLaunchKernelGGL((k_wino_dy<S, floatx4>), dim3(cdiv(g.T * K / 4, 256)), dim3(256), 0, st, dy, dM, g, K, ld,
                         row_src);
      return;
    }
  }
  hipLaunchKernelGGL((k_wino_dy<S, float>), dim3(cdiv(g.T * K, 256)), dim3(256), 0, st, dy, dM, g, K, ld, row_src);
}
template <typename S, int MODE>
void run_output(const float* Mb, float* out, const WinoGeom& g, int K, const float* bias, const float* residual,
                const float* mask, int epi, hipStream_t st, int ldo = 0, const int* slot = nullptr) {
  if (ldo <= 0) ldo = K;
  if constexpr (can_vec<S>()) {
    if (wide(g.T, K)) {
      hipLaunchKernelGGL((k_wino_output<S, MODE, floatx4>), dim3(cdiv(g.T * K / 4, 256)), dim3(256), 0, st, Mb, out,
                         g, K, ldo, bias, residual, mask, epi, slot);
      return;
    }
  }
  hipLaunchKernelGGL((k_wino_output<S, MODE, float>), dim3(cdiv(g.T * K, 256)), dim3(256), 0, st, Mb, out, g, K, ldo,
                     bias, residual, mask, epi, slot);
}
template <typename S>
void run_wgrad_out(const float* dU, int ns, int64_t CK, int K, const float* scale, float* dw, float beta,
                   hipStream_t st) {
  if constexpr (can_vec<S>()) {
    if (CK >= 262144) {
      hipLaunchKernelGGL((k_wino_wgrad_out<S, floatx2>), dim3(cdiv(CK / 2, 256)), dim3(256), 0, st, dU, ns, CK, K,
                         scale, dw, beta);
      return;
    }
  }
  hipLaunchKernelGGL((k_wino_wgrad_out<S, float>), dim3(cdiv(CK, 256)), dim3(256), 0, st, dU, ns, CK, K, scale, dw,
                     beta);
}

template <int MODE>
void launch_gemm(int cfg, ConvArgs& p, int planes, int nz, hipStream_t st) {
  if (MODE != MODE_WGRAD && split_engine_takes(cfg, p.M, p.NG, p.C, planes)) {
    launch_split<MODE, true>(p, dim3(1, planes, nz), st);
    return;
  }
  count_engine_launch(0);
  p.tiles_m = (int)cdiv(p.M, CFG_BM[cfg]);
  p.tiles_n = (int)cdiv(p.NG, CFG_BN[cfg]);
  dim3 grid(p.tiles_m * p.tiles_n, planes, nz);
  if (cfg >= NCFG && ((p.NG & 3) || (MODE == MODE_WGRAD && (p.M & 3)))) cfg -= NCFG;
  switch (cfg) {
    case 0: hipLaunchKernelGGL((k_wino_gemm<128, 128, MODE>), grid, dim3(256), 0, st, p); break;
    case 1: hipLaunchKernelGGL((k_wino_gemm<128, 64, MODE>), grid, dim3(256), 0, st, p); break;
    case 2: hipLaunchKernelGGL((k_wino_gemm<64, 64, MODE>), grid, dim3(256), 0, st, p); break;
    case 3: hipLaunchKernelGGL((k_wino_gemm<256, 128, MODE>), grid, dim3(512), 0, st, p); break;
    case 4: hipLaunchKernelGGL((k_wino_glds<128, 128, MODE, 16, GLDS_STAGES>), grid, dim3(256), 0, st, p); break;
    case 5: hipLaunchKernelGGL((k_wino_glds<128, 64, MODE, 16, GLDS_STAGES>), grid, dim3(256), 0, st, p); break;
    case 6: hipLaunchKernelGGL((k_wino_glds<64, 64, MODE, 16, GLDS_STAGES>), grid, dim3(256), 0, st, p); break;
    default: hipLaunchKernelGGL((k_wino_glds<256, 128, MODE, 16, GLDS_STAGES>), grid, dim3(512), 0, st, p); break;
  }
}

ConvArgs gemm_args(int64_t T, int C, int K) {
  ConvArgs p;
  memset(&p, 0, sizeof(p));
  p.N = 1; p.H = 1; p.W = (int)T; p.C = C; p.K = K; p.R = 1; p.S = 1; p.OH = 1; p.OW = (int)T;
  p.stride = 1; p.dil = 1;
  p.nsplit = 1;
  return p;
}

void wgrad_split(int64_t T, int planes, int C, int K, int cfg, int* nsplit, int* pps) {
  int64_t tiles = cdiv(C, CFG_BM[cfg]) * cdiv(K, CFG_BN[cfg]) * planes;
  int64_t ksteps = cdiv(T, 16);
  double best = 1e30;
  *nsplit = 1; *pps = (int)align_up(T, 16);
  for (int s = 1; s <= 16; ++s) {
    if (s > 1 && ksteps * 16 / s < 128) break;
    int64_t per = cdiv(ksteps, s);
    int64_t ns = cdiv(ksteps, per);
    if (ns != s) continue;
    double t = tile_time_us(cfg, tiles * ns, (int)per, true) + (double)planes * C * K * 4.0 * ns / 3.0e6;
    if (t < best) { best = t; *nsplit = (int)ns; *pps = (int)(per * 16); }
  }
}

int best_tile(int64_t rows, int64_t cols, int planes, int ksteps, double* t_out) {
  int best = 2;
  double bt = 1e30;
  for (int c = 0; c < NCFG; ++c) {
    double t = tile_time_us(c, cdiv(rows, CFG_BM[c]) * cdiv(cols, CFG_BN[c]) * planes, ksteps, true);
    if (t < bt) { bt = t; best = c; }
  }
  if (t_out) *t_out = bt;
  return best;
}

template <typename S>
bool eligible(const mtlssl_conv_desc* d) {
  if (!(d->R == 3 && d->S == 3 && d->stride == 1 && d->dilation == 1 && d->pad_t == 1 && d->pad_l == 1 &&
        d->OH == d->H && d->OW == d->W))
    return false;
  if (d->C % 16 || d->K % 16 || d->C < 32 || d->K < 32) return false;
  if (S::O == 7 && (d->H % 7 || d->W % 7)) return false;
  WinoGeom g = geom<S>(d);
  int64_t widest = d->C > d->K ? d->C : d->K;
  return g.T * widest < (1ll << 30);
}

template <typename S>
double time_us(const mtlssl_conv_desc* d, int mode, int* tile) {
  constexpr int PL = S::P * S::P;
  WinoGeom g = geom<S>(d);
  double tg;
  int cfg;
  const double px = (double)d->N * d->H * d->W;
  double bytes;
  if (mode == MODE_WGRAD) {
    cfg = best_tile(d->C, d->K, PL, (int)cdiv(g.T, 16), &tg);
    int ns, pps;
    wgrad_split(g.T, PL, d->C, d->K, cfg, &ns, &pps);
    tg = tile_time_us(cfg, cdiv(d->C, CFG_BM[cfg]) * cdiv(d->K, CFG_BN[cfg]) * PL * ns, pps / 16, true);
    bytes = 4.0 * (px * (d->C + d->K) + 2.0 * PL * g.T * (d->C + d->K) + (double)PL * d->C * d->K * (ns + 1));
  } else {
    int cin = mode == MODE_FWD ? d->C : d->K, cout = mode == MODE_FWD ? d->K : d->C;
    cfg = best_tile(g.T, cout, PL, cin / 16, &tg);
    bytes = 4.0 * (px * (cin + cout) + 2.0 * PL * g.T * (cin + cout) + 2.0 * PL * d->C * d->K);
  }
  if (tile) *tile = cfg;
  return tg + bytes / 4.0e6 + 12.0;
}

inline int64_t index_bytes(int64_t T) {
  const int64_t Tp = align_up(T, 64);
  return align_up((2 * Tp + KSTEP_HDR + Tp / 16 + 16) * 4 + Tp / 64, 256);
}
template <typename S>
int64_t workspace_bytes(const mtlssl_conv_desc* d, int mode) {
  constexpr int PL = S::P * S::P;
  WinoGeom g = geom<S>(d);
  int64_t planes = align_up((int64_t)PL * g.T * d->C * 4, 256) + align_up((int64_t)PL * g.T * d->K * 4, 256);
  if (mode != MODE_FWD) planes += index_bytes(g.T);
  if (mode == MODE_WGRAD) {
    int ns = 1, pps;
    int64_t mx = 1;
    for (int cfg = 0; cfg < NCFG; ++cfg) { wgrad_split(g.T, PL, d->C, d->K, cfg, &ns, &pps); if (ns > mx) mx = ns; }
    if (split_wgrad_plan(g.T, d->C, d->K, PL, &ns, &pps) && ns > mx) mx = ns;
    return planes + align_up(mx * PL * d->C * d->K * 4, 256);
  }
  return planes + align_up((int64_t)PL * d->C * d->K * 4, 256);
}

template <typename S>
void fwd(const mtlssl_conv_desc* d, int tile, const float* x, const float* w, const float* bias,
         const float* residual, float* y, int epi, void* workspace, hipStream_t st, const float* U_pre = nullptr,
         float* V_keep = nullptr) {
  constexpr int PL = S::P * S::P;
  WinoGeom g = geom<S>(d);
  const int64_t CK = (int64_t)d->C * d->K;
  float* U = (float*)workspace;
  float* V = (float*)((char*)U + align_up(PL * CK * 4, 256));
  float* Mb = (float*)((char*)V + align_up((int64_t)PL * g.T * d->C * 4, 256));
  if (U_pre) U = const_cast<float*>(U_pre);
  else run_filter<S>(w, U, CK, 0, st);
  if (V_keep) V = V_keep;
  run_input<S>(x, V, g, d->C, st);
  ConvArgs p = gemm_args(g.T, d->C, d->K);
  p.a = V; p.b = U; p.out = Mb;
  p.M = (int)g.T; p.NG = d->K;
  p.a_bytes = (unsigned)(g.T * d->C * 4); p.b_bytes = (unsigned)(CK * 4);
  p.a_bs = g.T * d->C; p.b_bs = CK; p.o_bs = g.T * d->K;
  launch_gemm<MODE_FWD>(tile, p, PL, 1, st);
  run_output<S, MODE_FWD>(Mb, y, g, d->K, bias, residual, nullptr, epi, st, d->ldy);
}

template <typename S>
void dgrad(const mtlssl_conv_desc* d, int tile, const float* dy, const float* w, const float* residual,
           const float* mask_ref, float* dx, int epi, void* workspace, hipStream_t st, const float* U_pre = nullptr,
           const uint8_t* active = nullptr) {
  constexpr int PL = S::P * S::P;
  WinoGeom g = geom<S>(d);
  const int64_t CK = (int64_t)d->C * d->K;
  float* U = (float*)workspace;
  float* V = (float*)((char*)U + align_up(PL * CK * 4, 256));
  float* Mb = (float*)((char*)V + align_up((int64_t)PL * g.T * d->K * 4, 256));
  if (U_pre) U = const_cast<float*>(U_pre);
  else run_filter<S>(w, U, CK, 1, st);
  ConvArgs p = gemm_args(g.T, d->C, d->K);
  p.a = V; p.b = U; p.out = Mb;
  p.M = (int)g.T; p.NG = d->C;
  p.a_bytes = (unsigned)(g.T * d->K * 4); p.b_bytes = (unsigned)(CK * 4);
  p.a_bs = g.T * d->K; p.b_bs = CK; p.o_bs = g.T * d->C;
  const int* slot = nullptr;
  const int* row_src = nullptr;
  if (active && !split_engine_takes(tile, p.M, p.NG, p.C, PL)) {
    const int64_t Tp = align_up(g.T, 64);
    int* maps = (int*)((char*)workspace + workspace_bytes<S>(d, MODE_DGRAD) - index_bytes(g.T));
    uint8_t* gflags = (uint8_t*)(maps + 2 * Tp);
    hipLaunchKernelGGL(k_wino_active_tiles, dim3(1), dim3(256), 0, st, active, g.th * g.tw, (int)g.T, maps, maps + Tp, gflags);
    slot = maps; row_src = maps + Tp;
    p.group_active = gflags; p.rows_per_group = 64;
  }
  run_input<S>(dy, V, g, d->K, st, d->ldy, row_src);
  launch_gemm<MODE_DGRAD>(tile, p, PL, 1, st);
  run_output<S, MODE_DGRAD>(Mb, dx, g, d->C, nullptr, residual, mask_ref, epi, st, 0, slot);
}

template <typename S>
void wgrad(const mtlssl_conv_desc* d, int tile, const float* x, const float* dy, const float* out_scale,
           float* dw, float beta, void* workspace, hipStream_t st, const float* V_pre = nullptr,
           const uint8_t* active = nullptr) {
  constexpr int PL = S::P * S::P;
  WinoGeom g = geom<S>(d);
  const int64_t CK = (int64_t)d->C * d->K;
  float* V = (float*)workspace;
  float* dM = (float*)((char*)V + align_up((int64_t)PL * g.T * d->C * 4, 256));
  float* dU = (float*)((char*)dM + align_up((int64_t)PL * g.T * d->K * 4, 256));
  int ns, pps;
  wgrad_split(g.T, PL, d->C, d->K, tile, &ns, &pps);
  const bool split = fp32_engine() >= 1 && (tile == 0 || tile == 3) && split_wgrad_plan(g.T, d->C, d->K, PL, &ns, &pps);
  ConvArgs p = gemm_args(g.T, d->C, d->K);
  const int* row_src = nullptr;
  if (active && !split && ns <= KSTEP_HDR) {
    int* maps = (int*)((char*)workspace + workspace_bytes<S>(d, MODE_WGRAD) - index_bytes(g.T));
    int* list = maps + align_up(g.T, 64);
    hipLaunchKernelGGL(k_wino_active_pairs, dim3(ns), dim3(256), 0, st, active, g.th * g.tw, (int)g.T, pps,
                       tile >= NCFG ? 1 : 0, pps / BK, maps, list);
    row_src = maps;
    p.k_steps = list; p.k_stride = pps / BK;
  }
  if (V_pre && row_src)
    hipLaunchKernelGGL(k_wino_gather_rows, dim3(cdiv(g.T * d->C / 4, 256), PL), dim3(256), 0, st, V_pre, V, row_src, g.T, d->C);
  else if (V_pre) V = const_cast<float*>(V_pre);
  else run_input<S>(x, V, g, d->C, st, 0, row_src);
  run_dy<S>(dy, dM, g, d->K, st, d->ldy, row_src);
  p.a = V; p.b = dM; p.out = dU;
  p.M = d->C; p.NG = d->K; p.nsplit = ns; p.pix_per_split = pps;
  p.a_bytes = (unsigned)(g.T * d->C * 4); p.b_bytes = (unsigned)(g.T * d->K * 4);
  p.a_bs = g.T * d->C; p.b_bs = g.T * d->K;
  if (split) launch_split<MODE_WGRAD, true>(p, dim3(1, PL, ns), st);
  else launch_gemm<MODE_WGRAD>(tile, p, PL, ns, st);
  run_wgrad_out<S>(dU, ns, CK, d->K, out_scale, dw, beta, st);
}

}

bool wino_eligible(const mtlssl_conv_desc* d, int variant) {
  return variant == WINO_M7 ? eligible<M7>(d) : eligible<F43>(d);
}
double wino_time_us(const mtlssl_conv_desc* d, int variant, int mode, int* tile) {
  return variant == WINO_M7 ? time_us<M7>(d, mode, tile) : time_us<F43>(d, mode, tile);
}
int64_t wino_workspace_bytes(const mtlssl_conv_desc* d, int variant, int mode) {
  return variant == WINO_M7 ? workspace_bytes<M7>(d, mode) : workspace_bytes<F43>(d, mode);
}
void wino_fwd(const mtlssl_conv_desc* d, int variant, int tile, const float* x, const float* w, const float* bias,
              const float* residual, float* y, int epi, void* workspace, hipStream_t st, const float* filter_xf,
              float* input_xf_keep) {
  if (variant == WINO_M7) fwd<M7>(d, tile, x, w, bias, residual, y, epi, workspace, st, filter_xf, input_xf_keep);
  else fwd<F43>(d, tile, x, w, bias, residual, y, epi, workspace, st, filter_xf, input_xf_keep);
}
int64_t wino_input_bytes(const mtlssl_conv_desc* d, int variant) {
  if (variant == WINO_M7) { WinoGeom g = geom<M7>(d); return align_up((int64_t)M7::P * M7::P * g.T * d->C * 4, 256); }
  WinoGeom g = geom<F43>(d);
  return align_up((int64_t)F43::P * F43::P * g.T * d->C * 4, 256);
}
void wino_dgrad(const mtlssl_conv_desc* d, int variant, int tile, const float* dy, const float* w,
                const float* residual, const float* mask_ref, float* dx, int epi, void* workspace, hipStream_t st,
                const float* filter_xf, const uint8_t* batch_active) {
  if (variant == WINO_M7) dgrad<M7>(d, tile, dy, w, residual, mask_ref, dx, epi, workspace, st, filter_xf, batch_active);
  else dgrad<F43>(d, tile, dy, w, residual, mask_ref, dx, epi, workspace, st, filter_xf, batch_active);
}
int64_t wino_filter_bytes(const mtlssl_conv_desc* d, int variant) {
  const int64_t pl = variant == WINO_M7 ? M7::P * M7::P : F43::P * F43::P;
  return align_up(pl * (int64_t)d->C * d->K * 4, 256);
}
void wino_filters_batched(int variant, int n, const void* w_ptrs, const void* u_ptrs, const int64_t* ck,
                          const int32_t* flip, int64_t max_ck, hipStream_t st) {
  dim3 grid((unsigned)cdiv(max_ck, 256), n);
  if (variant == WINO_M7)
    hipLaunchKernelGGL((k_wino_filter_batched<M7>), grid, dim3(256), 0, st, (const float* const*)w_ptrs,
                       (float* const*)u_ptrs, ck, flip);
  else
    hipLaunchKernelGGL((k_wino_filter_batched<F43>), grid, dim3(256), 0, st, (const float* const*)w_ptrs,
                       (float* const*)u_ptrs, ck, flip);
}
void wino_filter(const mtlssl_conv_desc* d, int variant, int flip, const float* w, float* U, hipStream_t st) {
  const int64_t CK = (int64_t)d->C * d->K;
  if (variant == WINO_M7) run_filter<M7>(w, U, CK, flip, st);
  else run_filter<F43>(w, U, CK, flip, st);
}
void wino_wgrad(const mtlssl_conv_desc* d, int variant, int tile, const float* x, const float* dy,
                const float* out_scale, float* dw, float beta, void* workspace, hipStream_t st, const float* input_xf,
                const uint8_t* batch_active) {
  if (variant == WINO_M7) wgrad<M7>(d, tile, x, dy, out_scale, dw, beta, workspace, st, input_xf, batch_active);
  else wgrad<F43>(d, tile, x, dy, out_scale, dw, beta, workspace, st, input_xf, batch_active);
}
void wino_wgrad_split(const mtlssl_conv_desc* d, int variant, int tile, int* ns, int* pps) {
  const int PL = variant == WINO_M7 ? M7::P * M7::P : F43::P * F43::P;
  const int64_t T = variant == WINO_M7 ? geom<M7>(d).T : geom<F43>(d).T;
  wgrad_split(T, PL, d->C, d->K, tile, ns, pps);
  if (fp32_engine() >= 1 && (tile == 0 || tile == 3)) split_wgrad_plan(T, d->C, d->K, PL, ns, pps);
}

}
```

Baseline: 41.37 images/sec.

## Pack active row groups in pointwise dgrad to compact skipped tiles

Adds a single-block kernel that builds a permutation placing active row groups (per the group_active flags) first, and new pointwise dgrad GEMM variants that read and write rows through that permutation. Inactive groups then cluster into whole tiles that skip their K loop, rather than partially active tiles that still do full work. Tile rows are also reassigned in an interleaved order across workgroups. Separately, Winograd M7 dgrad with active-group flags switches to a different tile config. The cost is one extra serial pack launch per conv, indirect row addressing and some extra workspace.

```diff
diff --git a/mtl_ssl_amd/csrc/conv.hip b/mtl_ssl_amd/csrc/conv.hip
--- a/mtl_ssl_amd/csrc/conv.hip
+++ b/mtl_ssl_amd/csrc/conv.hip
@@ -39,6 +39,44 @@
   }
   if (threadIdx.x == 0) out[z] = base;
 }
+__device__ __forceinline__ int pack_region(const uint8_t* __restrict__ flags, int lo, int hi, int* __restrict__ perm, int* wave_cnt) {
+  const int lane = threadIdx.x & 63, w = threadIdx.x >> 6;
+  int n = 0;
+  for (int g0 = lo; g0 < hi; g0 += 256) {
+    const int g = g0 + threadIdx.x;
+    n += __popcll(__ballot(g < hi && flags[g] != 0));
+  }
+  if (lane == 0) wave_cnt[w] = n;
+  __syncthreads();
+  const int nlive = wave_cnt[0] + wave_cnt[1] + wave_cnt[2] + wave_cnt[3];
+  __syncthreads();
+  int base = 0;
+  for (int g0 = lo; g0 < hi; g0 += 256) {
+    const int g = g0 + threadIdx.x;
+    const bool act = g < hi && flags[g] != 0;
+    const unsigned long long m = __ballot(act);
+    if (lane == 0) wave_cnt[w] = __popcll(m);
+    __syncthreads();
+    int before = base + __popcll(m & ((1ull << lane) - 1ull));
+    for (int i = 0; i < w; ++i) before += wave_cnt[i];
+    if (act) perm[lo + before] = g;
+    else if (g < hi) perm[lo + nlive + (g - lo) - before] = g;
+    base += wave_cnt[0] + wave_cnt[1] + wave_cnt[2] + wave_cnt[3];
+    __syncthreads();
+  }
+  return nlive;
+}
+__global__ void __launch_bounds__(256) k_row_pack(const uint8_t* __restrict__ flags, int G, int cut0, int cut1, int* __restrict__ out) {
+  __shared__ int wave_cnt[4];
+  int n = pack_region(flags, 0, cut0, out, wave_cnt);
+  n += pack_region(flags, cut1, G, out, wave_cnt);
+  if (threadIdx.x == 0) {
+    for (int g = cut0; g < cut1; ++g) { out[g] = g; n += flags[g] != 0; }
+    out[G] = n;
+  }
+}
+constexpr int64_t PACK_MAX_GROUPS = 65536;
+static inline int64_t row_pack_bytes(int64_t M) { return align_up(((M < PACK_MAX_GROUPS ? M : PACK_MAX_GROUPS) + 1) * 4, 256); }
 static inline int64_t kstep_list_bytes(int64_t P) { return align_up((KSTEP_HDR + 2 * cdiv(P, BK) + 128) * 4, 256); }
 static std::atomic<int>& row_skip_ref() { static std::atomic<int> v{1}; return v; }
 
@@ -827,6 +865,21 @@
       return;
     }
   }
+  if constexpr (MODE == MODE_DGRAD) {
+    if (pw && p.row_perm) {
+      switch (cfg) {
+        case 0: hipLaunchKernelGGL((k_conv_mfma_pw_pack<128, 128>), grid, dim3(256), 0, st, p); break;
+        case 1: hipLaunchKernelGGL((k_conv_mfma_pw_pack<128, 64>), grid, dim3(256), 0, st, p); break;
+        case 2: hipLaunchKernelGGL((k_conv_mfma_pw_pack<64, 64>), grid, dim3(256), 0, st, p); break;
+        case 3: hipLaunchKernelGGL((k_conv_mfma_pw_pack<256, 128>), grid, dim3(512), 0, st, p); break;
+        case 4: hipLaunchKernelGGL((k_conv_glds_pw_pack<128, 128, 16, GLDS_STAGES>), grid, dim3(256), 0, st, p); break;
+        case 5: hipLaunchKernelGGL((k_conv_glds_pw_pack<128, 64, 16, GLDS_STAGES>), grid, dim3(256), 0, st, p); break;
+        case 6: hipLaunchKernelGGL((k_conv_glds_pw_pack<64, 64, 16, GLDS_STAGES>), grid, dim3(256), 0, st, p); break;
+        default: hipLaunchKernelGGL((k_conv_glds_pw_pack<256, 128, 16, GLDS_STAGES>), grid, dim3(512), 0, st, p); break;
+      }
+      return;
+    }
+  }
   if (cfg < NCFG && pw) {
     switch (cfg) {
       case 0: hipLaunchKernelGGL((k_conv_mfma_pw<128, 128, MODE>), grid, dim3(256), 0, st, p); break;
@@ -865,6 +918,15 @@
     p.nsplit = 1; p.ks_per_split = 0; p.tile_m0 = 0; p.ws_m0 = 0;
     launch_split_direct<MODE>(p, dim3(1, 1, 1), st);
     return;
+  }
+  if constexpr (MODE == MODE_DGRAD) {
+    if (p.row_perm && conv_is_pointwise(p) && pointwise_ref().load() != 0) {
+      const int m_tail0 = pl.tail_rows > 0 ? ((int)cdiv(p.M, CFG_BM[pl.cfg]) - pl.tail_rows) * CFG_BM[pl.cfg] : 0;
+      hipLaunchKernelGGL(k_row_pack, dim3(1), dim3(256), 0, st, p.group_active, p.M / p.rows_per_group,
+                         m_tail0 / p.rows_per_group, (int)cdiv(m_tail0, p.rows_per_group), const_cast<int*>(p.row_perm));
+    } else {
+      p.row_perm = nullptr;
+    }
   }
   if (pl.tail_rows == 0) {
     p.nsplit = pl.nsplit; p.ks_per_split = pl.ks_per_split;
@@ -1035,6 +1097,8 @@
   Plan parity[4];
   int64_t front_a, front_bytes;
   int64_t bytes;
+  int64_t pack_bytes;
+  int flagged_tile;
 };
 static inline int64_t colsum_bytes(const mtlssl_conv_desc* d) { return align_up((int64_t)COLSUM_MAX_PARTS * d->K * 4, 256); }
 static int64_t wgrad_partial_bytes(const mtlssl_conv_desc* d, int ns, int* split_ns, int* split_pps) {
@@ -1091,6 +1155,7 @@
     if (ws && choose_wino(d, mode, t, &r.wc)) {
       r.family = FAM_WINO;
       r.bytes = wino_workspace_bytes(d, r.wc.variant, mode);
+      r.flagged_tile = (!fwd && r.wc.variant == WINO_M7) ? 2 + (r.wc.tile & 4) : r.wc.tile;
     } else if (ws && !fwd && parity_ok(d)) {
       r.family = FAM_PARITY;
       r.front_a = align_up((int64_t)d->R * d->S * d->C * d->K * 4, 256);
@@ -1107,7 +1172,8 @@
     } else {
       r.family = FAM_DIRECT;
       if (!ws && (r.plan.nsplit > 1 || r.plan.tail_rows > 0)) r.plan = Plan{pick_tile(M, NG, 1), 1, 0, 0, 1, 0};
-      r.bytes = split_bytes(r.plan, M, NG);
+      if (ws && !fwd && desc_is_pointwise(d)) r.pack_bytes = row_pack_bytes(M);
+      r.bytes = split_bytes(r.plan, M, NG) + r.pack_bytes;
     }
     return r;
   }
@@ -1460,7 +1526,8 @@
     case FAM_WINO:
       wino_dgrad(d, r.wc.variant, r.wc.tile, dy, w, residual, mask_ref, dx, epi, workspace, S(stream),
                  (filter_xf && xf_variant == r.wc.variant) ? filter_xf : nullptr,
-                 (group_active && row_skip_ref().load() != 0 && rows_per_group == d->H * d->W) ? group_active : nullptr);
+                 (group_active && row_skip_ref().load() != 0 && rows_per_group == d->H * d->W) ? group_active : nullptr,
+                 r.flagged_tile);
       break;
     case FAM_PARITY:
       parity_dgrad(r, d, dy, w, residual, mask_ref, dx, epi, workspace, S(stream));
@@ -1469,6 +1536,8 @@
       if (group_active && row_skip_ref().load() != 0 && desc_is_pointwise(d)) {
         p.group_active = group_active;
         p.rows_per_group = rows_per_group;
+        if (r.pack_bytes > 0 && p.M % rows_per_group == 0 && p.M / rows_per_group <= PACK_MAX_GROUPS)
+          p.row_perm = (const int*)((char*)workspace + r.bytes - r.pack_bytes);
       }
       launch_planned<MODE_DGRAD>(r.plan, p, (float*)workspace, S(stream));
       break;
diff --git a/mtl_ssl_amd/csrc/conv_mfma.h b/mtl_ssl_amd/csrc/conv_mfma.h
--- a/mtl_ssl_amd/csrc/conv_mfma.h
+++ b/mtl_ssl_amd/csrc/conv_mfma.h
@@ -48,6 +48,7 @@
   int rows_per_group;
   const int* k_steps;
   int k_stride;
+  const int* row_perm;
 };
 constexpr int KSTEP_HDR = 64;
 
@@ -58,6 +59,27 @@
   return any;
 }
 
+__device__ __forceinline__ int pack_src_row(const ConvArgs& p, int row) {
+  const int s = row / p.rows_per_group;
+  return p.row_perm[s] * p.rows_per_group + (row - s * p.rows_per_group);
+}
+template <int BM>
+__device__ __forceinline__ void pack_tile_rows(const ConvArgs& p, int m0, int* srow) {
+  if ((int)threadIdx.x < BM) srow[threadIdx.x] = m0 + (int)threadIdx.x < p.M ? pack_src_row(p, m0 + threadIdx.x) : 0;
+  __syncthreads();
+}
+__device__ __forceinline__ bool tile_slots_active(const ConvArgs& p, int m0, int bm) {
+  const int s1 = (min(m0 + bm, p.M) - 1) / p.rows_per_group;
+  bool any = false;
+  for (int s = m0 / p.rows_per_group; s <= s1; ++s) any |= p.group_active[p.row_perm[s]] != 0;
+  return any;
+}
+__device__ __forceinline__ int pack_tile_row(int v, int tiles_m) {
+  const int q = tiles_m / 8, r = tiles_m % 8, cut = r * (q + 1);
+  if (v < cut) return (v % (q + 1)) * 8 + v / (q + 1);
+  return ((v - cut) % q) * 8 + r + (v - cut) / q;
+}
+
 typedef unsigned uintx4 __attribute__((ext_vector_type(4)));
 __host__ __device__ __forceinline__ int args_ldy(const ConvArgs& p) { return p.ldy ? p.ldy : p.K; }
 
@@ -66,9 +88,9 @@
   return __builtin_bit_cast(floatx4, __builtin_amdgcn_raw_buffer_load_b128(rsrc, voffset, soffset, 0));
 }
 
-template <int BM, int BN, int MODE, int NW, bool PREFETCH_RES = false>
+template <int BM, int BN, int MODE, int NW, bool PREFETCH_RES = false, bool PACK = false>
 __device__ __forceinline__ void conv_epilogue(const ConvArgs& p, floatx16 (&acc)[BM / (16 * NW)][BN / 64], float* smem,
-                                              int m0, int n0) {
+                                              int m0, int n0, const int* srow = nullptr) {
   constexpr int WR = NW / 2, TM = BM / (32 * WR), TN = BN / 64, LDT = 36;
   const int tid = threadIdx.x, lane = tid & 63, wid = tid >> 6;
   const int wr = wid >> 1, wc = wid & 1;
@@ -104,7 +126,8 @@
       for (int k = 0; k < 4; ++k) {
         const int row = m0 + wr * (BM / WR) + i * 32 + r_in + 8 * k;
         dst[k] = floatx4{0.f, 0.f, 0.f, 0.f};
-        if (use_res && row < p.M && col < p.NG) dst[k] = *reinterpret_cast<const floatx4*>(p.residual + (int64_t)row * ldo + col);
+        if (use_res && row < p.M && col < p.NG)
+          dst[k] = *reinterpret_cast<const floatx4*>(p.residual + (int64_t)(PACK ? srow[row - m0] : row) * ldo + col);
       }
     };
     if constexpr (PREFETCH_RES) fetch_res(0, res_cur);
@@ -124,8 +147,9 @@
         for (int k = 0; k < 4; ++k) {
           const int rt = r_in + 8 * k;
           floatx4 v = *reinterpret_cast<const floatx4*>(tile + rt * LDT + c4);
-          const int row = m0 + wr * (BM / WR) + i * 32 + rt;
+          int row = m0 + wr * (BM / WR) + i * 32 + rt;
           if (row >= p.M || col >= p.NG) continue;
+          if constexpr (PACK) row = srow[row - m0];
           if (raw) {
             *reinterpret_cast<floatx4*>(outp + (int64_t)(row - p.ws_m0) * ldo + col) = v;
             continue;
@@ -171,8 +195,9 @@
         if ((p.epi & MTLSSL_EPI_BIAS) && col_ok) bv = p.bias[col];
 #pragma unroll
       for (int e = 0; e < 16; ++e) {
-        const int row = m0 + wr * (BM / WR) + i * 32 + (e & 3) + 8 * (e >> 2) + 4 * hi;
+        int row = m0 + wr * (BM / WR) + i * 32 + (e & 3) + 8 * (e >> 2) + 4 * hi;
         if (row >= p.M || !col_ok) continue;
+        if constexpr (PACK) row = srow[row - m0];
         const int64_t o = (int64_t)row * ldo + col;
         const int64_t of = MODE == MODE_FWD ? (int64_t)row * ldf + col : o;
         float v = acc[i][j][e];
@@ -198,9 +223,10 @@
 }
 
 struct SegArgs { mtlssl_conv_seg_entry e[MTLSSL_CONV_GROUP_MAX]; };
-template <int BM, int BN, int MODE, int BKT, bool BATCH, bool PW = false, bool CS = false, bool SEG = false>
+template <int BM, int BN, int MODE, int BKT, bool BATCH, bool PW = false, bool CS = false, bool SEG = false, bool PACK = false>
 __device__ __forceinline__ void conv_mfma_body(ConvArgs p, const SegArgs sg = SegArgs{}) {
   static_assert(!SEG || (PW && MODE == MODE_DGRAD && !BATCH), "segments: pointwise dgrad only");
+  static_assert(!PACK || (PW && MODE == MODE_DGRAD && !BATCH && !SEG), "packed rows: plain pointwise dgrad only");
   constexpr int NW = BM > 128 ? 8 : 4, NT = 64 * NW, WR = NW / 2;
   constexpr int LDA = BM + 4, LDB = BN + 4;
   constexpr int KQ = BKT / 4;
@@ -224,7 +250,7 @@
   }
   if constexpr (BATCH && MODE == MODE_DGRAD)
     if (p.group_active) bid = (int)((bid + (unsigned)blockIdx.y * ((nwg + 7) / 8)) % (unsigned)nwg);
-  const int tile_m = bid / p.tiles_n + p.tile_m0, tile_n = bid % p.tiles_n;
+  const int tile_m = (PACK ? pack_tile_row(bid / p.tiles_n, p.tiles_m) : bid / p.tiles_n) + p.tile_m0, tile_n = bid % p.tiles_n;
   const int m0 = tile_m * BM, n0 = tile_n * BN;
   const int tid = threadIdx.x, lane = tid & 63, wid = tid >> 6;
   const int wr = wid >> 1, wc = wid & 1;
@@ -276,7 +302,11 @@
       ksteps = min(ksteps, ks_begin + p.ks_per_split);
     }
   }
-  if constexpr (PW && MODE == MODE_DGRAD && !SEG)
+  __shared__ int srow[PACK ? BM : 1];
+  if constexpr (PACK) {
+    pack_tile_rows<BM>(p, m0, srow);
+    if (!tile_slots_active(p, m0, BM)) ksteps = ks_begin;
+  } else if constexpr (PW && MODE == MODE_DGRAD && !SEG)
     if (p.group_active && !tile_rows_active(p, m0, BM)) {
       if constexpr (BATCH) return;
       ksteps = ks_begin;
@@ -298,7 +328,8 @@
     for (int i = 0; i < A_LD; ++i) {
       const int m = m0 + (tid / KQ) + RP * i;
       const int ld = MODE == MODE_FWD ? p.C : ldy;
-      a_voff[i] = m < p.M ? (unsigned)(m * ld + kq4) * 4u : OOB;
+      if constexpr (PACK) a_voff[i] = m < p.M ? (unsigned)(srow[m - m0] * ld + kq4) * 4u : OOB;
+      else a_voff[i] = m < p.M ? (unsigned)(m * ld + kq4) * 4u : OOB;
     }
   } else if constexpr (A_KC) {
 #pragma unroll
@@ -630,12 +661,13 @@
       __syncthreads();
     }
   }
-  conv_epilogue<BM, BN, MODE, NW>(p, acc, smem, m0, n0);
-}
-
-
-template <int BM, int BN, int MODE, int BKT, int NSTAGE, bool BATCH, bool PWISE = false, bool CS = false>
+  conv_epilogue<BM, BN, MODE, NW, false, PACK>(p, acc, smem, m0, n0, srow);
+}
+
+
+template <int BM, int BN, int MODE, int BKT, int NSTAGE, bool BATCH, bool PWISE = false, bool CS = false, bool PACK = false>
 __device__ __forceinline__ void conv_glds_body(ConvArgs p) {
+  static_assert(!PACK || (PWISE && MODE == MODE_DGRAD && !BATCH), "packed rows: plain pointwise dgrad only");
   constexpr int NW = BM > 128 ? 8 : 4, WR = NW / 2;
   constexpr int TM = BM / (32 * WR), TN = BN / 64;
   constexpr bool A_KC = (MODE != MODE_WGRAD);
@@ -661,7 +693,7 @@
   }
   if constexpr (BATCH && MODE == MODE_DGRAD)
     if (p.group_active) bid = (int)((bid + (unsigned)blockIdx.y * ((nwg + 7) / 8)) % (unsigned)nwg);
-  const int tile_m = bid / p.tiles_n + p.tile_m0, tile_n = bid % p.tiles_n;
+  const int tile_m = (PACK ? pack_tile_row(bid / p.tiles_n, p.tiles_m) : bid / p.tiles_n) + p.tile_m0, tile_n = bid % p.tiles_n;
   const int m0 = tile_m * BM, n0 = tile_n * BN;
   const int tid = threadIdx.x, lane = tid & 63, wid = tid >> 6;
   const int wr = wid >> 1, wc = wid & 1;
@@ -699,7 +731,11 @@
       ksteps = min(ksteps, ks_begin + p.ks_per_split);
     }
   }
-  if constexpr (PWISE && MODE == MODE_DGRAD)
+  __shared__ int srow[PACK ? BM : 1];
+  if constexpr (PACK) {
+    pack_tile_rows<BM>(p, m0, srow);
+    if (!tile_slots_active(p, m0, BM)) ksteps = ks_begin;
+  } else if constexpr (PWISE && MODE == MODE_DGRAD)
     if (p.group_active && !tile_rows_active(p, m0, BM)) {
       if constexpr (BATCH) return;
       ksteps = ks_begin;
@@ -730,7 +766,8 @@
     for (int i = 0; i < PA; ++i) {
       const int row = kc_row(wid * PA + i);
       const int m = m0 + row;
-      a_voff[i] = m < p.M ? (unsigned)(m * (MODE == MODE_FWD ? p.C : ldy) + kc_quad4(row)) * 4u : OOB;
+      if constexpr (PACK) a_voff[i] = m < p.M ? (unsigned)(srow[row] * ldy + kc_quad4(row)) * 4u : OOB;
+      else a_voff[i] = m < p.M ? (unsigned)(m * (MODE == MODE_FWD ? p.C : ldy) + kc_quad4(row)) * 4u : OOB;
     }
   } else if constexpr (A_KC) {
 #pragma unroll
@@ -1000,7 +1037,7 @@
   }
   if constexpr (CS)
     if (do_cs && tid < BN && n0 + tid < p.NG) p.cs_part[(int64_t)blockIdx.z * p.NG + n0 + tid] = csum;
-  conv_epilogue<BM, BN, MODE, NW>(p, acc, smem, m0, n0);
+  conv_epilogue<BM, BN, MODE, NW, false, PACK>(p, acc, smem, m0, n0, srow);
 }
 
 template <int BM, int BN, int BKT, int NSTAGE>
@@ -1031,6 +1068,11 @@
 k_conv_glds_pw_cs(ConvArgs p) {
   conv_glds_body<BM, BN, MODE_WGRAD, BKT, NSTAGE, false, true, true>(p);
 }
+template <int BM, int BN, int BKT, int NSTAGE>
+__global__ void __launch_bounds__(BM > 128 ? 512 : 256, (glds_waves<BM, BN, BKT, NSTAGE>()))
+k_conv_glds_pw_pack(ConvArgs p) {
+  conv_glds_body<BM, BN, MODE_DGRAD, BKT, NSTAGE, false, true, false, true>(p);
+}
 template <int BM, int BN, int MODE, int BKT, int NSTAGE>
 __global__ void __launch_bounds__(BM > 128 ? 512 : 256, (glds_waves<BM, BN, BKT, NSTAGE>()))
 k_wino_glds(ConvArgs p) {
@@ -1046,6 +1088,11 @@
 __global__ void __launch_bounds__(BM > 128 ? 512 : 256, (BM > 128 ? 2 : BM * BN >= 128 * 128 ? 3 : 4))
 k_conv_mfma_pw(ConvArgs p) {
   conv_mfma_body<BM, BN, MODE, 16, false, true>(p);
+}
+template <int BM, int BN>
+__global__ void __launch_bounds__(BM > 128 ? 512 : 256, (BM > 128 ? 2 : BM * BN >= 128 * 128 ? 3 : 4))
+k_conv_mfma_pw_pack(ConvArgs p) {
+  conv_mfma_body<BM, BN, MODE_DGRAD, 16, false, true, false, false, true>(p);
 }
 template <int BM, int BN, int BKT>
 __global__ void __launch_bounds__(BM > 128 ? 512 : 256, (BM > 128 ? 2 : BM * BN >= 128 * 128 ? (BKT > 16 ? 2 : 3) : 4))
@@ -1115,7 +1162,7 @@
 int64_t wino_input_bytes(const mtlssl_conv_desc* d, int variant);
 void wino_dgrad(const mtlssl_conv_desc* d, int variant, int tile, const float* dy, const float* w,
                 const float* residual, const float* mask_ref, float* dx, int epi, void* workspace, hipStream_t st,
-                const float* filter_xf = nullptr, const uint8_t* batch_active = nullptr);
+                const float* filter_xf = nullptr, const uint8_t* batch_active = nullptr, int flagged_tile = -1);
 int64_t wino_filter_bytes(const mtlssl_conv_desc* d, int variant);
 void wino_filter(const mtlssl_conv_desc* d, int variant, int flip, const float* w, float* U, hipStream_t st);
 void wino_filters_batched(int variant, int n, const void* w_ptrs, const void* u_ptrs, const int64_t* ck,
diff --git a/mtl_ssl_amd/csrc/winograd.hip b/mtl_ssl_amd/csrc/winograd.hip
--- a/mtl_ssl_amd/csrc/winograd.hip
+++ b/mtl_ssl_amd/csrc/winograd.hip
@@ -616,7 +616,7 @@
 template <typename S>
 void dgrad(const mtlssl_conv_desc* d, int tile, const float* dy, const float* w, const float* residual,
            const float* mask_ref, float* dx, int epi, void* workspace, hipStream_t st, const float* U_pre = nullptr,
-           const uint8_t* active = nullptr) {
+           const uint8_t* active = nullptr, int flagged_tile = -1) {
   constexpr int PL = S::P * S::P;
   WinoGeom g = geom<S>(d);
   const int64_t CK = (int64_t)d->C * d->K;
@@ -639,6 +639,7 @@
     hipLaunchKernelGGL(k_wino_active_tiles, dim3(1), dim3(256), 0, st, active, g.th * g.tw, (int)g.T, maps, maps + Tp, gflags);
     slot = maps; row_src = maps + Tp;
     p.group_active = gflags; p.rows_per_group = 64;
+    if (flagged_tile >= 0) tile = flagged_tile;
   }
   run_input<S>(dy, V, g, d->K, st, d->ldy, row_src);
   launch_gemm<MODE_DGRAD>(tile, p, PL, 1, st);
@@ -706,9 +707,9 @@
 }
 void wino_dgrad(const mtlssl_conv_desc* d, int variant, int tile, const float* dy, const float* w,
                 const float* residual, const float* mask_ref, float* dx, int epi, void* workspace, hipStream_t st,
-                const float* filter_xf, const uint8_t* batch_active) {
-  if (variant == WINO_M7) dgrad<M7>(d, tile, dy, w, residual, mask_ref, dx, epi, workspace, st, filter_xf, batch_active);
-  else dgrad<F43>(d, tile, dy, w, residual, mask_ref, dx, epi, workspace, st, filter_xf, batch_active);
+                const float* filter_xf, const uint8_t* batch_active, int flagged_tile) {
+  if (variant == WINO_M7) dgrad<M7>(d, tile, dy, w, residual, mask_ref, dx, epi, workspace, st, filter_xf, batch_active, flagged_tile);
+  else dgrad<F43>(d, tile, dy, w, residual, mask_ref, dx, epi, workspace, st, filter_xf, batch_active, flagged_tile);
 }
 int64_t wino_filter_bytes(const mtlssl_conv_desc* d, int variant) {
   const int64_t pl = variant == WINO_M7 ? M7::P * M7::P : F43::P * F43::P;
```

After: 41.61 images/sec, median of 6. No clear change (+0.6%).
